# dcy0577/Enhancing-3D-Point-Cloud-Segmentation-Using-Multi-Modal-Fusion-with-2D-Images

Measured on AMD Instinct MI355X. Metric: input points/s through MV-KPConv KPFCNN forward+backward (pyramid + fusion + fwd + bwd + SGD), higher is better.
Workload: dtype f32; 1 GPU; early_fusion_kpfcnn5_sphere19k_x1_per_gpu; views=3, parallelism=dp1, execution=hipGraph[net|chain|enc2d(x2 every 2nd step)+fa], ranks=1, input_lookahead_batches=2, capacity_overflow=False

## Files before the change

### enhancing-3d-point-cloud-segmentation-using-multi-modal-fusion-with-2d-images_amd/_lib.py

```python
import ctypes as C
import os
import re

_HERE = os.path.dirname(os.path.abspath(__file__))
LIB_PATH = os.path.join(_HERE, "libmvkpconv.so")
HEADER_PATH = os.path.join(_HERE, "..", "include", "mvkpconv.h")
SCENE_HEADER_PATH = os.path.join(_HERE, "..", "include", "mvkpconv_scene.h")
TRAIN_HEADER_PATH = os.path.join(_HERE, "..", "include", "mvkpconv_train.h")
SPHERE_HEADER_PATH = os.path.join(_HERE, "..", "include", "mvkpconv_sphere.h")

CTYPES = {"int": C.c_int, "int32_t": C.c_int32, "int64_t": C.c_int64, "float": C.c_float, "double": C.c_double,
          "const char*": C.c_char_p}
_SCALARS = frozenset(t for t in CTYPES if not t.endswith("*"))
_POINTEES = _SCALARS | {"void", "char", "uint8_t", "uint16_t"}
_INTEGER = r"-?(?:0[xX][0-9a-fA-F]+|0|[1-9][0-9]*)"
_DIRECTIVE = re.compile(r"\s*#\s*(?:include\s*<[\w./]+>|ifdef\s+__cplusplus|ifndef\s+\w+_H|endif"
                        r"|define\s+(\w+)(?:\s+(%s))?)\s*" % _INTEGER)
_STRUCT = re.compile(r"typedef\s+struct(?:\s+\w+)?\s*\{([^{}]*)\}\s*(mvk_\w+)\s*;")
_FUNCTION = re.compile(r"([\w\s*]+?)\b(mvk_\w+)\s*\(([^(){};]*)\)\s*;")


def parse_header(text):
    functions, structs, constants = {}, {}, {}

    def fail(pos, what):
        pos += len(text[pos:]) - len(text[pos:].lstrip())
        raise ValueError("mvkpconv.h line %d: %s" % (text.count("\n", 0, pos) + 1, what))

    def canonical(pos, spelling):
        tokens = re.findall(r"\w+|\S", spelling)
        const = tokens[:1] == ["const"]
        base, stars = "".join(tokens[const:const + 1]), tokens[const + 1:]
        if not (stars == [] and not const and base in _SCALARS
                or stars == ["*"] and (base in _POINTEES or base in structs)):
            fail(pos, "unsupported type %r" % " ".join(tokens))
        return "const " * const + base + "*" * len(stars)

    def declarator(pos, spelling):
        m = re.fullmatch(r"(.*[\s*])([A-Za-z_]\w*)\s*", spelling, re.S)
        if not m or m.group(2) == "const" or m.group(2) in _POINTEES:
            fail(pos, "expected '<type> <name>', found %r" % spelling.strip())
        return canonical(pos, m.group(1)), m.group(2)

    text = re.sub(r"/\*.*?\*/|//[^\n]*", lambda m: " " + "\n" * m.group().count("\n"), text, flags=re.S)
    lines = text.split("\n")
    for i, line in enumerate(lines):
        if line.lstrip().startswith("#"):
            m = _DIRECTIVE.fullmatch(line)
            name, value = m.groups() if m else (None, None)
            if not m or (name is not None and (name.startswith("MVK_") != (value is not None) or name in constants)):
                raise ValueError("mvkpconv.h line %d: unsupported preprocessor line %r" % (i + 1, line.strip()))
            if value is not None:
                constants[name] = int(value, 0)
            lines[i] = ""
    text = "\n".join(lines)

    block = re.fullmatch(r'\s*extern\s+"C"\s*\{(.*)\}\s*', text, re.S)
    if not block:
        fail(0, 'expected one extern "C" { ... } block around all declarations')
    pos, end = block.start(1), block.end(1)
    while True:
        pos = re.compile(r"\s*").match(text, pos, end).end()
        if pos == end:
            return functions, structs, constants
        s = _STRUCT.match(text, pos, end)
        f = None if s else _FUNCTION.match(text, pos, end)
        if (s or f) and (s or f).group(2) in functions.keys() | structs.keys():
            fail(pos, "%s is declared twice" % (s or f).group(2))
        if s:
            fields, at = [], s.start(1)
            *statements, tail = s.group(1).split(";")
            if tail.strip() or not statements:
                fail(s.end(1) - len(tail), "struct %s: expected 'type name;' fields" % s.group(2))
            for statement in statements:
                first, *more = statement.split(",")
                ctype, name = declarator(at, first)
                if more and (ctype.endswith("*") or not all(re.fullmatch(r"\s*[A-Za-z_]\w*\s*", n) for n in more)):
                    fail(at, "only scalar fields share a declaration, found %r" % statement.strip())
                fields += [(ctype, n.strip()) for n in [name] + more]
                at += len(statement) + 1
            structs[s.group(2)] = tuple(fields)
        elif f:
            params, at = [], f.start(3)
            for spelling in f.group(3).split(",") if f.group(3).strip() != "void" else ():
                params.append(declarator(at, spelling))
                at += len(spelling) + 1
            functions[f.group(2)] = (canonical(pos, f.group(1)), tuple(params))
        else:
            fail(pos, "neither a function declaration nor a struct typedef: %r" % text[pos:end].split("\n")[0].strip())
        pos = (s or f).end()


def _bind(functions, structs):
    classes = {}

    def ctype(t):
        if t in CTYPES:
            return CTYPES[t]
        assert t.endswith("*"), t
        pointee = t[6 * t.startswith("const "):-1]
        return C.POINTER(classes[pointee]) if pointee in classes else C.c_void_p

    for name, fields in structs.items():
        classes[name] = type("".join(w.capitalize() for w in name.split("_")[1:]), (C.Structure,),
                             {"_fields_": [(n, ctype(t)) for t, n in fields], "__doc__": name + " (include/mvkpconv.h)"})
    return classes, {name: (ctype(ret), [ctype(t) for t, _ in params]) for name, (ret, params) in functions.items()}


def _read_header(path=None, name="mvkpconv.h"):
    path = HEADER_PATH if path is None else path
    if not os.path.exists(path):
        raise RuntimeError(
            "include/%s is not there (%s). The binding reads every prototype of libmvkpconv.so from it -- "
            "run the package from a checkout of the repository; there is no second copy of the C ABI." % (name, path))
    with open(path) as f:
        return f.read()


FUNCTIONS, STRUCTS, CONSTANTS = parse_header(_read_header())
_CLASSES, _PROTOTYPES = _bind(FUNCTIONS, STRUCTS)
EXPORTS = tuple(FUNCTIONS)
ABI_VERSION = CONSTANTS["MVK_ABI_VERSION"]

SCENE_FUNCTIONS, _scene_structs, SCENE_CONSTANTS = parse_header(_read_header(SCENE_HEADER_PATH, "mvkpconv_scene.h"))
if _scene_structs or SCENE_FUNCTIONS.keys() & FUNCTIONS.keys() or SCENE_CONSTANTS.keys() & CONSTANTS.keys():
    raise ValueError("mvkpconv_scene.h: it may declare neither a struct nor a name of mvkpconv.h")
_SCENE_PROTOTYPES = _bind(SCENE_FUNCTIONS, {})[1]

TRAIN_FUNCTIONS, _train_structs, TRAIN_CONSTANTS = parse_header(_read_header(TRAIN_HEADER_PATH, "mvkpconv_train.h"))
if (_train_structs or TRAIN_FUNCTIONS.keys() & (FUNCTIONS.keys() | SCENE_FUNCTIONS.keys())
        or TRAIN_CONSTANTS.keys() & (CONSTANTS.keys() | SCENE_CONSTANTS.keys())):
    raise ValueError("mvkpconv_train.h: it may declare neither a struct nor a name of the other two headers")
_TRAIN_PROTOTYPES = _bind(TRAIN_FUNCTIONS, {})[1]

SPHERE_FUNCTIONS, _sphere_structs, SPHERE_CONSTANTS = parse_header(_read_header(SPHERE_HEADER_PATH, "mvkpconv_sphere.h"))
if (_sphere_structs
        or SPHERE_FUNCTIONS.keys() & (FUNCTIONS.keys() | SCENE_FUNCTIONS.keys() | TRAIN_FUNCTIONS.keys())
        or SPHERE_CONSTANTS.keys() & (CONSTANTS.keys() | SCENE_CONSTANTS.keys() | TRAIN_CONSTANTS.keys())):
    raise ValueError("mvkpconv_sphere.h: it may declare neither a struct nor a name of the other three headers")
_SPHERE_PROTOTYPES = _bind(SPHERE_FUNCTIONS, {})[1]
BnFwdProblem, BnBwdProblem = _CLASSES["mvk_bn_fwd_problem"], _CLASSES["mvk_bn_bwd_problem"]
BnFinish, ATransform = _CLASSES["mvk_bn_finish"], _CLASSES["mvk_a_transform"]
RevList, RegLayer = _CLASSES["mvk_rev_list"], _CLASSES["mvk_reg_layer"]

_lib = None
_owner_pid = None

FORK_MESSAGE = ("the MV-KPConv HIP library was initialised in process %d and is being called from its forked child %d: "
                "a HIP context does not survive fork(). Start DataLoader workers with multiprocessing_context='spawn', "
                "or let the workers emit only stacked points / lengths and build the pyramid "
                "(datasets.common.segmentation_inputs_sphere) in the main process -- see INTEGRATION.md")


def _check_process():
    pid = os.getpid()
    if _owner_pid is not None and pid != _owner_pid:
        raise RuntimeError(FORK_MESSAGE % (_owner_pid, pid))
    try:
        import torch
        if torch.cuda._is_in_bad_fork():
            raise RuntimeError(FORK_MESSAGE % (os.getppid(), pid))
    except (ImportError, AttributeError):
        pass


def lib():
    global _lib, _owner_pid
    _check_process()
    if _lib is None:
        if not os.path.exists(LIB_PATH):
            raise RuntimeError(
                "libmvkpconv.so is not built (%s). Run `python __graft_entry__.py build` -- there is "
                "no CPU fallback for the MV-KPConv hot path." % LIB_PATH)
        l = C.CDLL(LIB_PATH)
        for name, (res, args) in list(_PROTOTYPES.items()) + list(_SCENE_PROTOTYPES.items()) + list(_TRAIN_PROTOTYPES.items()) \
                + list(_SPHERE_PROTOTYPES.items()):
            fn = getattr(l, name)
            fn.restype = res
            fn.argtypes = args
        if l.mvk_abi_version() != ABI_VERSION:
            raise RuntimeError("libmvkpconv.so ABI %d != expected %d; rebuild" % (l.mvk_abi_version(), ABI_VERSION))
        _lib = l
        _owner_pid = os.getpid()
    return _lib


def check(rc):
    if rc != 0:
        raise RuntimeError(lib().mvk_last_error().decode("utf-8", "replace"))
```

### enhancing-3d-point-cloud-segmentation-using-multi-modal-fusion-with-2d-images_amd/build.py

```python
import os
import subprocess
import sys

HERE = os.path.dirname(os.path.abspath(__file__))
CSRC = os.path.join(HERE, "csrc")
OUT = os.path.join(HERE, "libmvkpconv.so")
ARCH = "gfx950"

SOURCES = [
    ("error.cpp", []),
    ("kpconv.hip", []),
    ("gemm.hip", []),
    ("gemm32s.hip", []),
    ("pool.hip", []),
    ("bn.hip", []),
    ("optim.hip", []),
    ("deform.hip", []),
    ("loss.hip", []),
    ("batchpad.hip", []),
    ("revlist.hip", []),
    ("subsample.hip", ["-ffp-contract=off"]),
    ("neighbors.hip", ["-ffp-contract=off"]),
    ("fusion.hip", ["-ffp-contract=off"]),
    ("vote.hip", ["-ffp-contract=off"]),
    ("pn2.hip", ["-ffp-contract=off"]),
    ("chunk.hip", ["-ffp-contract=off"]),
    ("pn2_ordered.hip", ["-ffp-contract=off"]),
    ("pn2_mlp.hip", ["-ffp-contract=off"]),
    ("pn2_rows.hip", ["-ffp-contract=off"]),
    ("scene_inputs.hip", ["-ffp-contract=off"]),
    ("train_inputs.hip", ["-ffp-contract=off"]),
    ("sphere_inputs.hip", ["-ffp-contract=off"]),
]


def _hipcc():
    for c in (os.environ.get("HIPCC"), "/opt/rocm/bin/hipcc", "hipcc"):
        if c and (os.path.isabs(c) and os.path.exists(c) or not os.path.isabs(c)):
            return c
    return "hipcc"


def _stale(target, deps):
    if not os.path.exists(target):
        return True
    t = os.path.getmtime(target)
    return any(os.path.getmtime(d) > t for d in deps if os.path.exists(d))


def build_library(force=False, verbose=False):
    hipcc = _hipcc()
    common = [os.path.join(CSRC, "common.h"), os.path.join(CSRC, "blockscan.h"), os.path.join(CSRC, "compact.h"),
              os.path.join(CSRC, "pn2_rows.h"), os.path.join(CSRC, "unproject.h"), os.path.join(CSRC, "select_frames.h"),
              os.path.join(CSRC, "knn_core.h"), os.path.join(HERE, "..", "include", "mvkpconv_sphere.h"),
              os.path.join(HERE, "..", "include", "mvkpconv.h"), os.path.join(HERE, "..", "include", "mvkpconv_scene.h"),
              os.path.join(HERE, "..", "include", "mvkpconv_train.h"),
              os.path.join(HERE, "..", "include", "mvk_prime_list.h"), os.path.abspath(__file__)]
    objs, jobs = [], []
    for src, extra in SOURCES:
        sp = os.path.join(CSRC, src)
        if not os.path.exists(sp):
            raise FileNotFoundError(sp)
        obj = os.path.join(CSRC, os.path.splitext(src)[0] + ".o")
        if force or _stale(obj, [sp] + common):
            cmd = [hipcc, "--offload-arch=" + ARCH, "-O3", "-std=c++17", "-fPIC", "-c", sp, "-o", obj] + extra
            if src.endswith(".cpp"):
                cmd = [hipcc, "-O2", "-std=c++17", "-fPIC", "-c", sp, "-o", obj]
            jobs.append(cmd)
        objs.append(obj)
    if jobs:
        from concurrent.futures import ThreadPoolExecutor
        n = max(1, min(int(os.environ.get("MVK_BUILD_JOBS", "6")), os.cpu_count() or 1, len(jobs)))

        def run(cmd):
            if verbose:
                print(" ".join(cmd), flush=True)
            subprocess.check_call(cmd)
        with ThreadPoolExecutor(n) as pool:
            list(pool.map(run, jobs))
    if force or _stale(OUT, objs):
        cmd = [hipcc, "--offload-arch=" + ARCH, "-shared", "-fPIC", "-o", OUT] + objs
        if verbose:
            print(" ".join(cmd))
        subprocess.check_call(cmd)
    return OUT


if __name__ == "__main__":
    print(build_library(force="--force" in sys.argv, verbose=True))
```

### enhancing-3d-point-cloud-segmentation-using-multi-modal-fusion-with-2d-images_amd/csrc/gemm.hip

```cpp
#include <stdlib.h>

#include <mutex>
#include <type_traits>

#include "common.h"

namespace {

typedef float f32x4 __attribute__((ext_vector_type(4)));

constexpr int BK = 32;

template <bool CONTIG_K, int ROWS>
struct Tile {
  static constexpr int LD = CONTIG_K ? 40 : ROWS + 4;
  static constexpr int FLOATS = CONTIG_K ? ROWS * 40 : BK * (ROWS + 4);
  static constexpr int NF4 = ROWS * BK / 4;
  static constexpr int NV = (NF4 + 255) / 256;
  static constexpr int IPT = ROWS / 4;
  float4 v[NV];

  __device__ __forceinline__ void transform(const float* __restrict__ xs, int64_t k0, int64_t kbase0, int64_t i0, int64_t imax,
                                            int64_t kmax, int64_t nvalid, float slope, float* __restrict__ out, int64_t ld,
                                            int tid) {
    static_assert(CONTIG_K, "the transform is written for k-contiguous A tiles");
#pragma unroll
    for (int u = 0; u < NV; ++u) {
      const int f = tid + 256 * u;
      if (NF4 % 256 == 0 || f < NF4) {
        const int i = f >> 3, kq = (f & 7) * 4;
        const int64_t gi = i0 + i, gk = k0 + kq;
        const float* t = xs + (gk - kbase0) * 4;
        float e[4] = {v[u].x, v[u].y, v[u].z, v[u].w};
#pragma unroll
        for (int c = 0; c < 4; ++c) {
          const float4 q = *reinterpret_cast<const float4*>(t + 4 * c);
          float z = (e[c] - q.x) * q.y + q.z;
          z = z > 0.f ? z : z * slope;
          e[c] = gi < nvalid ? z : 0.f;
        }
        v[u] = make_float4(e[0], e[1], e[2], e[3]);
        if (out && gi < imax) {
          float* o = out + gi * ld + gk;
          if (gk + 3 < kmax && (ld & 3) == 0)
            *reinterpret_cast<float4*>(o) = v[u];
          else {
#pragma unroll
            for (int c = 0; c < 4; ++c)
              if (gk + c < kmax) o[c] = e[c];
          }
        }
      }
    }
  }

  __device__ __forceinline__ void load(const float* __restrict__ src, int64_t ld, int64_t i0, int64_t imax,
                                       int64_t k0, int64_t kmax, int vec, int tid) {
#pragma unroll
    for (int u = 0; u < NV; ++u) {
      float t[4] = {0.f, 0.f, 0.f, 0.f};
      const int f = tid + 256 * u;
      if (NF4 % 256 == 0 || f < NF4) {
        if (CONTIG_K) {
          const int i = f >> 3, kq = (f & 7) * 4;
          const int64_t gi = i0 + i, gk = k0 + kq;
          if (gi < imax) {
            const float* p = src + gi * ld + gk;
            if (vec == 4 && gk + 3 < kmax) {
              const float4 q = *reinterpret_cast<const float4*>(p);
              t[0] = q.x; t[1] = q.y; t[2] = q.z; t[3] = q.w;
            } else if (vec == 2 && gk + 3 < kmax) {
              const float2 q0 = *reinterpret_cast<const float2*>(p), q1 = *reinterpret_cast<const float2*>(p + 2);
              t[0] = q0.x; t[1] = q0.y; t[2] = q1.x; t[3] = q1.y;
            } else {
#pragma unroll
              for (int e = 0; e < 4; ++e)
                if (gk + e < kmax) t[e] = p[e];
            }
          }
        } else {
          const int k = f / IPT, iq = (f % IPT) * 4;
          const int64_t gk = k0 + k, gi = i0 + iq;
          if (gk < kmax) {
            const float* p = src + gk * ld + gi;
            if (vec == 4 && gi + 3 < imax) {
              const float4 q = *reinterpret_cast<const float4*>(p);
              t[0] = q.x; t[1] = q.y; t[2] = q.z; t[3] = q.w;
            } else if (vec == 2 && gi + 3 < imax) {
              const float2 q0 = *reinterpret_cast<const float2*>(p), q1 = *reinterpret_cast<const float2*>(p + 2);
              t[0] = q0.x; t[1] = q0.y; t[2] = q1.x; t[3] = q1.y;
            } else {
#pragma unroll
              for (int e = 0; e < 4; ++e)
                if (gi + e < imax) t[e] = p[e];
            }
          }
        }
      }
      v[u] = make_float4(t[0], t[1], t[2], t[3]);
    }
  }

  template <int VEC>
  __device__ __forceinline__ void load_fast(const float* __restrict__ src, int64_t ld, int64_t i0, int64_t imax,
                                            int64_t k0, int tid) {
#pragma unroll
    for (int u = 0; u < NV; ++u) {
      int f = tid + 256 * u;
      if (NF4 % 256 != 0) f = f < NF4 ? f : NF4 - 1;
      const float* p;
      if (CONTIG_K) {
        const int i = f >> 3, kq = (f & 7) * 4;
        int64_t gi = i0 + i;
        gi = gi < imax ? gi : imax - 1;
        p = src + gi * ld + (k0 + kq);
      } else {
        const int k = f / IPT, iq = (f % IPT) * 4;
        int64_t gi = i0 + iq;
        gi = gi + 3 < imax ? gi : imax - 4;
        p = src + (k0 + k) * ld + gi;
      }
      if (VEC == 4) {
        const f32x4 q = *reinterpret_cast<const f32x4*>(p);
        v[u] = make_float4(q[0], q[1], q[2], q[3]);
      } else {
        const float2 q0 = *reinterpret_cast<const float2*>(p), q1 = *reinterpret_cast<const float2*>(p + 2);
        v[u] = make_float4(q0.x, q0.y, q1.x, q1.y);
      }
    }
  }

  static __device__ __forceinline__ bool fast_ok(int64_t imax, int vec) {
    return CONTIG_K ? (vec >= 2 && imax >= 1) : (vec == 4 && imax >= 4 && (imax & 3) == 0);
  }

  template <int VEC>
  __device__ __forceinline__ void fetch(const float* __restrict__ src, int64_t ld, int64_t i0, int64_t imax, int64_t k0,
                                        int64_t kmax, int vec, int tid) {
    if (VEC == 0)
      load(src, ld, i0, imax, k0, kmax, vec, tid);
    else
      load_fast<VEC>(src, ld, i0, imax, k0, tid);
  }

  __device__ __forceinline__ void store(float* __restrict__ T, int tid) const {
#pragma unroll
    for (int u = 0; u < NV; ++u) {
      const int f = tid + 256 * u;
      if (NF4 % 256 == 0 || f < NF4) {
        const f32x4 q = {v[u].x, v[u].y, v[u].z, v[u].w};
        if (CONTIG_K) {
          const int i = f >> 3, kq = (f & 7) * 4;
          *reinterpret_cast<f32x4*>(&T[i * LD + kq]) = q;
        } else {
          const int k = f / IPT, iq = (f % IPT) * 4;
          *reinterpret_cast<f32x4*>(&T[k * LD + iq]) = q;
        }
      }
    }
  }

  static __device__ __forceinline__ f32x4 frag(const float* __restrict__ T, int r0, int j, int lane) {
    const int i = lane & 15, g = lane >> 4;
    if (CONTIG_K) {
      return *reinterpret_cast<const f32x4*>(&T[(r0 + i) * LD + 16 * j + 4 * g]);
    } else {
      f32x4 r;
      const float* p = &T[(16 * j + 4 * g) * LD + r0 + i];
      r[0] = p[0];
      r[1] = p[LD];
      r[2] = p[2 * LD];
      r[3] = p[3 * LD];
      return r;
    }
  }
};

struct GemmArgs {
  const float* A;
  const float* B;
  float* C;
  int64_t M, N, Kd, lda, ldb, k_per_split;
  int atomic_out, accumulate, vecA, vecB;
  float* bn_part;
  const int32_t* n_valid;
  const float* bias;
  float act_slope;
  const float* A2;
  const float* B2;
  int64_t Kd2, lda2, ldb2;
  int vecA2, vecB2;
  const void* sc_idx;
  int sc_idx64, sc_c1;
  int64_t sc_stride, sc_ns;
  float* sc_dst;
  float* sc_rest;
  float* det_ws;
  int* det_cnt;
  int det_gx, det_nsplit;
  int seg_shift;
  int64_t seg_extra;
  int* fin_cnt;
  int fin_gy;
  float fin_eps, fin_momentum;
  float* fin_mean;
  float* fin_invstd;
  float* fin_rmean;
  float* fin_rvar;
  long long* fin_nbt;
  const float* ax_mean;
  const float* ax_invstd;
  const float* ax_gamma;
  const float* ax_beta;
  float ax_slope;
  const int32_t* ax_nvalid;
  float* ax_out;
};

constexpr int XF_KMAX = 512;

template <bool TA, bool TB, int PM, int QN, int WM, int WN, bool DUAL = false, bool XF = false>
__device__ __forceinline__ void gemm_body(const GemmArgs& a, const int bx, const int by, const int bz) {
  static_assert(WM * WN == 4, "four waves per workgroup");
  constexpr int TM = 16 * PM * WM, TN = 16 * QN * WN;
  typedef Tile<!TA, TM> TileA;
  typedef Tile<TB, TN> TileB;
  __shared__ __attribute__((aligned(16))) float lds[2 * (TileA::FLOATS + TileB::FLOATS)];
  __shared__ __attribute__((aligned(16))) float xs[XF ? 4 * (XF_KMAX + BK) : 4];
  float* const As = lds;
  float* const Bs = lds + 2 * TileA::FLOATS;
  const int tid = threadIdx.x, lane = tid & 63, wave = tid >> 6;
  const int wm = wave / WN, wn = wave % WN;
  const int64_t m0 = (int64_t)by * TM, n0 = (int64_t)bx * TN;
  const int64_t ktot = DUAL ? a.Kd + a.Kd2 : a.Kd;
  const int64_t kbeg_all = (int64_t)bz * a.k_per_split;
  const int64_t kend_all = kbeg_all + a.k_per_split < ktot ? kbeg_all + a.k_per_split : ktot;

  f32x4 acc[PM][QN];
#pragma unroll
  for (int p = 0; p < PM; ++p)
#pragma unroll
    for (int q = 0; q < QN; ++q) acc[p][q] = (f32x4){0.f, 0.f, 0.f, 0.f};

  int64_t x_nvalid = 0;
  if (XF) {
    for (int k = tid; k < XF_KMAX + BK; k += 256) {
      const int64_t gk = kbeg_all + k;
      float4 q = make_float4(0.f, 0.f, 0.f, 0.f);
      if (gk < a.Kd && k < a.k_per_split + BK) q = make_float4(a.ax_mean[gk], a.ax_invstd[gk] * a.ax_gamma[gk], a.ax_beta[gk], 0.f);
      *reinterpret_cast<float4*>(&xs[4 * k]) = q;
    }
    x_nvalid = a.ax_nvalid ? (int64_t)*a.ax_nvalid : a.M;
    __syncthreads();
  }
  float* const x_out = (XF && bx == 0) ? a.ax_out : nullptr;

  TileA la0, la1;
  TileB lb0, lb1;
  const int ra = wm * 16 * PM, rb = wn * 16 * QN;
  auto compute = [&](const float* __restrict__ Ta, const float* __restrict__ Tb) {
#pragma unroll
    for (int j = 0; j < 2; ++j) {
      f32x4 fa[PM], fb[QN];
#pragma unroll
      for (int p = 0; p < PM; ++p) fa[p] = TileA::frag(Ta, ra + 16 * p, j, lane);
#pragma unroll
      for (int q = 0; q < QN; ++q) fb[q] = TileB::frag(Tb, rb + 16 * q, j, lane);
#pragma unroll
      for (int s = 0; s < 4; ++s)
#pragma unroll
        for (int p = 0; p < PM; ++p)
#pragma unroll
          for (int q = 0; q < QN; ++q)
            acc[p][q] = __builtin_amdgcn_mfma_f32_16x16x4f32(fa[p][s], fb[q][s], acc[p][q], 0, 0, 0);
    }
  };
  float* const A0 = As;
  float* const A1 = As + TileA::FLOATS;
  float* const B0 = Bs;
  float* const B1 = Bs + TileB::FLOATS;
  auto run_range = [&](const float* __restrict__ pA, const int64_t lda, const int vecA, const float* __restrict__ pB,
                       const int64_t ldb, const int vecB, int64_t kbeg, const int64_t kend) {
  auto Bat = [&](const int64_t k) -> const float* {
    return (TB && !DUAL && a.seg_shift >= 0) ? pB + (k >> a.seg_shift) * a.seg_extra : pB;
  };
  auto putA = [&](TileA& la, float* __restrict__ T, const int64_t kt) {
    if constexpr (XF) la.transform(xs, kt, kbeg_all, m0, a.M, a.Kd, x_nvalid, a.ax_slope, x_out, lda, tid);
    la.store(T, tid);
  };
  auto pipeline = [&](auto va, auto vb, const int64_t klim) {
    constexpr int VA = decltype(va)::value, VB = decltype(vb)::value;
    if (kbeg >= klim) return;
    la0.template fetch<VA>(pA, lda, m0, a.M, kbeg, klim, vecA, tid);
    lb0.template fetch<VB>(Bat(kbeg), ldb, n0, a.N, kbeg, klim, vecB, tid);
    if (kbeg + BK < klim) {
      la1.template fetch<VA>(pA, lda, m0, a.M, kbeg + BK, klim, vecA, tid);
      lb1.template fetch<VB>(Bat(kbeg + BK), ldb, n0, a.N, kbeg + BK, klim, vecB, tid);
    }
    putA(la0, A0, kbeg);
    lb0.store(B0, tid);
    __syncthreads();
    for (int64_t k0 = kbeg; k0 < klim; k0 += 2 * BK) {
      if (k0 + 2 * BK < klim) {
        la0.template fetch<VA>(pA, lda, m0, a.M, k0 + 2 * BK, klim, vecA, tid);
        lb0.template fetch<VB>(Bat(k0 + 2 * BK), ldb, n0, a.N, k0 + 2 * BK, klim, vecB, tid);
      }
      compute(A0, B0);
      if (k0 + BK >= klim) break;
      putA(la1, A1, k0 + BK);
      lb1.store(B1, tid);
      __syncthreads();
      if (k0 + 3 * BK < klim) {
        la1.template fetch<VA>(pA, lda, m0, a.M, k0 + 3 * BK, klim, vecA, tid);
        lb1.template fetch<VB>(Bat(k0 + 3 * BK), ldb, n0, a.N, k0 + 3 * BK, klim, vecB, tid);
      }
      compute(A1, B1);
      if (k0 + 2 * BK >= klim) break;
      putA(la0, A0, k0 + 2 * BK);
      lb0.store(B0, tid);
      __syncthreads();
    }
  };
  const bool fastA = TileA::fast_ok(a.M, vecA), fastB = TileB::fast_ok(a.N, vecB);
  const int64_t kfull = kbeg + (kend - kbeg) / BK * BK;
  typedef std::integral_constant<int, 4> I4;
  typedef std::integral_constant<int, 2> I2;
  typedef std::integral_constant<int, 0> I0;
  if (fastA && fastB && vecA == 4 && vecB == 4) {
    pipeline(I4(), I4(), kfull);
  } else if (fastA && fastB && vecA == 2 && vecB == 4) {
    pipeline(I2(), I4(), kfull);
  } else {
    pipeline(I0(), I0(), kend);
    kbeg = kend;
  }
  if (kfull < kend && kbeg < kend) {
    __syncthreads();
    la0.load(pA, lda, m0, a.M, kfull, kend, vecA, tid);
    lb0.load(Bat(kfull), ldb, n0, a.N, kfull, kend, vecB, tid);
    putA(la0, A0, kfull);
    lb0.store(B0, tid);
    __syncthreads();
    compute(A0, B0);
  }
  };
  if (!DUAL) {
    run_range(a.A, a.lda, a.vecA, a.B, a.ldb, a.vecB, kbeg_all, kend_all);
  } else {
    if (kbeg_all < a.Kd) run_range(a.A, a.lda, a.vecA, a.B, a.ldb, a.vecB, kbeg_all, kend_all < a.Kd ? kend_all : a.Kd);
    if (kend_all > a.Kd) {
      if (kbeg_all < a.Kd) __syncthreads();
      run_range(a.A2, a.lda2, a.vecA2, a.B2, a.ldb2, a.vecB2, kbeg_all > a.Kd ? kbeg_all - a.Kd : 0, kend_all - a.Kd);
    }
  }

  if (a.det_ws) {
    constexpr int NB = PM * QN, SLOT = NB * 4 * 256;
    const int64_t tile = (int64_t)by * a.det_gx + bx;
    const __amdgpu_buffer_rsrc_t slots = park_rsrc(a.det_ws + tile * a.det_nsplit * SLOT);
    const uint32_t lane_off = (uint32_t)tid * 16u;
#pragma unroll
    for (int p = 0; p < PM; ++p)
#pragma unroll
      for (int q = 0; q < QN; ++q)
        park_store4(slots, (uint32_t)bz * (SLOT * 4u) + (uint32_t)(p * QN + q) * 4096u + lane_off, acc[p][q]);
    park_wait();
    __syncthreads();
    int* const flag = reinterpret_cast<int*>(lds);
    if (tid == 0) {
      const int old = __hip_atomic_fetch_add(a.det_cnt + tile, 1, __ATOMIC_RELAXED, __HIP_MEMORY_SCOPE_AGENT);
      const int last = old == a.det_nsplit - 1;
      if (last) __hip_atomic_store(a.det_cnt + tile, 0, __ATOMIC_RELAXED, __HIP_MEMORY_SCOPE_AGENT);
      *flag = last;
    }
    __syncthreads();
    const int last = *flag;
    __syncthreads();
    if (!last) return;
#pragma unroll
    for (int p = 0; p < PM; ++p)
#pragma unroll
      for (int q = 0; q < QN; ++q) acc[p][q] = (f32x4){0.f, 0.f, 0.f, 0.f};
    constexpr int ZC = NB >= 8 ? 2 : 4;
    for (int z0 = 0; z0 < a.det_nsplit; z0 += ZC) {
      f32x4 t[ZC][NB];
#pragma unroll
      for (int zz = 0; zz < ZC; ++zz) {
        const int z = z0 + zz < a.det_nsplit ? z0 + zz : a.det_nsplit - 1;
#pragma unroll
        for (int b = 0; b < NB; ++b) t[zz][b] = park_load4(slots, (uint32_t)z * (SLOT * 4u) + (uint32_t)b * 4096u + lane_off);
      }
#pragma unroll
      for (int zz = 0; zz < ZC; ++zz)
        if (z0 + zz < a.det_nsplit) {
#pragma unroll
          for (int p = 0; p < PM; ++p)
#pragma unroll
            for (int q = 0; q < QN; ++q) acc[p][q] += t[zz][p * QN + q];
        }
    }
  }

  const int ci = lane & 15, g4 = (lane >> 4) * 4;
#pragma unroll
  for (int q = 0; q < QN; ++q) {
    const int64_t col = n0 + rb + 16 * q + ci;
    if (col < a.N) {
      const float bq = a.bias ? a.bias[col] : 0.f;
#pragma unroll
      for (int p = 0; p < PM; ++p)
#pragma unroll
        for (int r = 0; r < 4; ++r) {
          const int64_t row = m0 + ra + 16 * p + g4 + r;
          if (row < a.M) {
            if (a.sc_idx) {
              const float v = acc[p][q][r];
              if (col < a.sc_c1) {
                const int j = a.sc_idx64 ? load_idx<true>(a.sc_idx, row * a.sc_stride, a.sc_ns)
                                         : load_idx<false>(a.sc_idx, row * a.sc_stride, a.sc_ns);
                if (j >= 0) atomicAdd(a.sc_dst + (int64_t)j * a.sc_c1 + col, v);
              } else {
                float* c2 = a.sc_rest + row * (a.N - a.sc_c1) + (col - a.sc_c1);
                if (a.atomic_out) atomicAdd(c2, v);
                else *c2 = v;
              }
              continue;
            }
            float* c = a.C + row * a.N + col;
            if (a.atomic_out)
              atomicAdd(c, acc[p][q][r]);
            else if (a.accumulate)
              *c += acc[p][q][r];
            else if (a.bias) {
              const float v = acc[p][q][r] + bq;
              *c = v > 0.f ? v : v * a.act_slope;
            } else
              *c = acc[p][q][r];
          }
        }
    }
  }

  if (a.bn_part) {
    int64_t nv = a.n_valid ? (int64_t)*a.n_valid : a.M;
    nv = nv < a.M ? nv : a.M;
    const int64_t wcnt = nv - (m0 + ra) < 0 ? 0 : (nv - (m0 + ra) > 16 * PM ? 16 * PM : nv - (m0 + ra));
    const int64_t bcnt = nv - m0 < 0 ? 0 : (nv - m0 > TM ? TM : nv - m0);
    const int64_t blk = m0 / TM;
    float* red = lds;
    const __amdgpu_buffer_rsrc_t part_rs = park_rsrc(a.bn_part);
    auto put_part = [&](const int64_t col, const float sum, const float m2) {
      if (a.fin_cnt) {
        park_store1(part_rs, (uint32_t)(((blk * 2) * a.N + col) * 4), sum);
        park_store1(part_rs, (uint32_t)(((blk * 2 + 1) * a.N + col) * 4), m2);
      } else {
        a.bn_part[(blk * 2) * a.N + col] = sum;
        a.bn_part[(blk * 2 + 1) * a.N + col] = m2;
      }
    };
    if (WM > 1) __syncthreads();
    float s[QN], mu[QN];
#pragma unroll
    for (int q = 0; q < QN; ++q) {
      s[q] = 0.f;
#pragma unroll
      for (int p = 0; p < PM; ++p)
#pragma unroll
        for (int r = 0; r < 4; ++r)
          if (16 * p + g4 + r < wcnt) s[q] += acc[p][q][r];
      s[q] += __shfl_xor(s[q], 16);
      s[q] += __shfl_xor(s[q], 32);
      if (WM > 1 && lane < 16) red[wm * TN + rb + 16 * q + ci] = s[q];
    }
    if (WM > 1) {
      __syncthreads();
#pragma unroll
      for (int q = 0; q < QN; ++q) {
        s[q] = 0.f;
#pragma unroll
        for (int w = 0; w < WM; ++w) s[q] += red[w * TN + rb + 16 * q + ci];
      }
    }
#pragma unroll
    for (int q = 0; q < QN; ++q) {
      mu[q] = bcnt > 0 ? s[q] / (float)bcnt : 0.f;
      float m2 = 0.f;
#pragma unroll
      for (int p = 0; p < PM; ++p)
#pragma unroll
        for (int r = 0; r < 4; ++r)
          if (16 * p + g4 + r < wcnt) {
            const float d = acc[p][q][r] - mu[q];
            m2 += d * d;
          }
      m2 += __shfl_xor(m2, 16);
      m2 += __shfl_xor(m2, 32);
      if (WM > 1) {
        if (lane < 16) red[(WM + wm) * TN + rb + 16 * q + ci] = m2;
      } else {
        const int64_t col = n0 + rb + 16 * q + ci;
        if (lane < 16 && col < a.N && m0 < a.M) put_part(col, s[q], m2);
      }
    }
    if (WM > 1) {
      __syncthreads();
      if (wm == 0 && lane < 16) {
#pragma unroll
        for (int q = 0; q < QN; ++q) {
          float m2 = 0.f;
#pragma unroll
          for (int w = 0; w < WM; ++w) m2 += red[(WM + w) * TN + rb + 16 * q + ci];
          const int64_t col = n0 + rb + 16 * q + ci;
          if (col < a.N && m0 < a.M) put_part(col, s[q], m2);
        }
      }
    }
    if (a.fin_cnt) {
      park_wait();
      __syncthreads();
      int* const flag = reinterpret_cast<int*>(lds);
      if (tid == 0) {
        const int old = __hip_atomic_fetch_add(a.fin_cnt + bx, 1, __ATOMIC_RELAXED, __HIP_MEMORY_SCOPE_AGENT);
        const int last = old == a.fin_gy - 1;
        if (last) __hip_atomic_store(a.fin_cnt + bx, 0, __ATOMIC_RELAXED, __HIP_MEMORY_SCOPE_AGENT);
        *flag = last;
      }
      __syncthreads();
      const int last = *flag;
      __syncthreads();
      if (!last) return;
      constexpr int C4 = TN / 4, BL = 256 / C4;
      const int c4 = tid % C4, bl = tid / C4;
      const int64_t col0 = n0 + 4 * c4;
      const int nb = nv > 0 ? (int)((nv + TM - 1) / TM) : 0;
      f32x4 X = {0.f, 0.f, 0.f, 0.f}, Y = {0.f, 0.f, 0.f, 0.f}, ref = {0.f, 0.f, 0.f, 0.f};
      if (col0 < a.N && nb > 0) {
        const float n0f = (float)(nv < TM ? nv : TM);
        ref = park_load4(part_rs, (uint32_t)(col0 * 4));
        ref = ref * (1.f / n0f);
        constexpr int FP = 4;
        for (int i0 = bl; i0 < nb; i0 += FP * BL) {
          f32x4 u[FP], w[FP];
#pragma unroll
          for (int t = 0; t < FP; ++t) {
            const int i = i0 + t * BL < nb ? i0 + t * BL : nb - 1;
            u[t] = park_load4(part_rs, (uint32_t)((((int64_t)i * 2) * a.N + col0) * 4));
            w[t] = park_load4(part_rs, (uint32_t)((((int64_t)i * 2 + 1) * a.N + col0) * 4));
          }
#pragma unroll
          for (int t = 0; t < FP; ++t)
            if (i0 + t * BL < nb) {
              const int64_t left = nv - (int64_t)(i0 + t * BL) * TM;
              const float ni = (float)(left < TM ? left : TM);
              const f32x4 d = u[t] * (1.f / ni) - ref;
              X += u[t];
              Y += w[t] + ni * d * d;
            }
        }
      }
      float* const q1 = lds;
      float* const q2 = lds + 256 * 4;
      *reinterpret_cast<f32x4*>(&q1[bl * TN + 4 * c4]) = X;
      *reinterpret_cast<f32x4*>(&q2[bl * TN + 4 * c4]) = Y;
      float* const qr = lds + 2 * 256 * 4;
      if (bl == 0) *reinterpret_cast<f32x4*>(&qr[4 * c4]) = ref;
      __syncthreads();
      const int64_t col = n0 + tid;
      if (tid < TN && col < a.N) {
        float x = 0.f, y = 0.f;
#pragma unroll 4
        for (int l = 0; l < BL; ++l) {
          x += q1[l * TN + tid];
          y += q2[l * TN + tid];
        }
        float mu = 0.f, var = 0.f, is = 0.f;
        if (nv > 0) {
          mu = x / (float)nv;
          const float dm = mu - qr[tid];
          float M2 = y - (float)nv * dm * dm;
          M2 = M2 > 0.f ? M2 : 0.f;
          var = M2 / (float)nv;
          is = rsqrtf(var + a.fin_eps);
        }
        a.fin_mean[col] = mu;
        a.fin_invstd[col] = is;
        if (a.fin_rmean && nv > 0) {
          const float unbiased = nv > 1 ? var * ((float)nv / (float)(nv - 1)) : var;
          a.fin_rmean[col] = (1.f - a.fin_momentum) * a.fin_rmean[col] + a.fin_momentum * mu;
          a.fin_rvar[col] = (1.f - a.fin_momentum) * a.fin_rvar[col] + a.fin_momentum * unbiased;
        }
      }
      if (a.fin_nbt && bx == 0 && tid == 0) *a.fin_nbt += 1;
    }
  }
}

template <bool TA, bool TB, int PM, int QN, int WM, int WN>
__global__ __launch_bounds__(256) void gemm_f32_mfma(const GemmArgs a) {
  gemm_body<TA, TB, PM, QN, WM, WN>(a, blockIdx.x, blockIdx.y, blockIdx.z);
}

template <bool TB, int PM>
__global__ __launch_bounds__(256) void gemm_f32_mfma_xf(const GemmArgs a) {
  gemm_body<false, TB, PM, 1, 1, 4, false, true>(a, blockIdx.x, blockIdx.y, blockIdx.z);
}

template <bool TA, bool TB, int PM, int QN, int WM, int WN>
__global__ __launch_bounds__(256) void gemm_f32_mfma_pair(const GemmArgs a0, const GemmArgs a1, int gx0, int gz0, int gz1) {
  if ((int)blockIdx.x < gx0) {
    if ((int)blockIdx.z >= gz0) return;
    gemm_body<TA, TB, PM, QN, WM, WN>(a0, blockIdx.x, blockIdx.y, blockIdx.z);
  } else {
    if ((int)blockIdx.z >= gz1) return;
    gemm_body<TA, TB, PM, QN, WM, WN>(a1, blockIdx.x - gx0, blockIdx.y, blockIdx.z);
  }
}

template <bool TA, bool TB, int PM, int QN, int WM, int WN>
__global__ __launch_bounds__(256) void gemm_f32_mfma_dual(const GemmArgs a) {
  gemm_body<TA, TB, PM, QN, WM, WN, true>(a, blockIdx.x, blockIdx.y, blockIdx.z);
}

struct GroupEntry {
  GemmArgs args;
  int gx, gy, gz;
  int wg_begin;
};

template <bool TA, bool TB, int PM, int QN, int WM, int WN>
__global__ __launch_bounds__(256) void gemm_f32_mfma_grouped(const GroupEntry* __restrict__ tab, int n_prob) {
  const int b = blockIdx.x;
  int lo = 0, hi = n_prob - 1;
  while (lo < hi) {
    const int mid = (lo + hi + 1) >> 1;
    if (tab[mid].wg_begin <= b)
      lo = mid;
    else
      hi = mid - 1;
  }
  const GroupEntry& e = tab[lo];
  const int local = b - e.wg_begin;
  const int bx = local % e.gx, by = (local / e.gx) % e.gy, bz = local / (e.gx * e.gy);
  GemmArgs a = e.args;
  a.A = load_global_ptr(&e.args.A);
  a.B = load_global_ptr(&e.args.B);
  a.C = load_global_ptr(&e.args.C);
  a.bn_part = load_global_ptr(&e.args.bn_part);
  a.n_valid = load_global_ptr(&e.args.n_valid);
  a.det_ws = load_global_ptr(&e.args.det_ws);
  a.det_cnt = load_global_ptr(&e.args.det_cnt);
  gemm_body<TA, TB, PM, QN, WM, WN>(a, bx, by, bz);
}


struct Plan {
  int pm, qn, narrow, split;
  int64_t tm() const { return narrow ? 64 * pm : 16 * pm; }
  int64_t tn() const { return narrow ? 16 * qn : 64 * qn; }
};

struct SplitArena {
  float* ws = nullptr;
  int* cnt = nullptr;
  int64_t ws_floats = 0, n_cnt = 0;
  int64_t ws_off = 0, cnt_off = 0;
  int64_t ws_top = 0, cnt_top = 0;
};
SplitArena g_arena;
std::mutex g_arena_mu;

bool ordered_splits() { return g_arena.ws != nullptr; }

int arena_take(hipStream_t st, int64_t tiles, int split, int64_t slot, float** ws, int** cnt) {
  const int64_t need = (tiles * split * slot + 63) / 64 * 64;
  std::lock_guard<std::mutex> lock(g_arena_mu);
  if (need > g_arena.ws_floats || tiles > g_arena.n_cnt) return 1;
  hipStreamCaptureStatus cap = hipStreamCaptureStatusNone;
  if (hipStreamIsCapturing(st, &cap) != hipSuccess) {
    (void)hipGetLastError();
    cap = hipStreamCaptureStatusNone;
  }
  if (cap != hipStreamCaptureStatusNone) {
    if (g_arena.ws_top - need < g_arena.ws_off || g_arena.cnt_top - tiles < g_arena.cnt_off) return 2;
    g_arena.ws_top -= need;
    g_arena.cnt_top -= tiles;
    *ws = g_arena.ws + g_arena.ws_top;
    *cnt = g_arena.cnt + g_arena.cnt_top;
    return 0;
  }
  const int64_t ws_cap = g_arena.ws_top < g_arena.ws_floats / 4 ? g_arena.ws_top : (need > g_arena.ws_floats / 4 ? need : g_arena.ws_floats / 4);
  const int64_t cnt_cap = g_arena.cnt_top < g_arena.n_cnt / 4 ? g_arena.cnt_top : (tiles > g_arena.n_cnt / 4 ? tiles : g_arena.n_cnt / 4);
  if (g_arena.ws_off + need > ws_cap || g_arena.cnt_off + tiles > cnt_cap) {
    if (need > g_arena.ws_top || tiles > g_arena.cnt_top) return 2;
    if (hipDeviceSynchronize() != hipSuccess) return -2;
    g_arena.ws_off = 0;
    g_arena.cnt_off = 0;
  }
  *ws = g_arena.ws + g_arena.ws_off;
  *cnt = g_arena.cnt + g_arena.cnt_off;
  g_arena.ws_off += need;
  g_arena.cnt_off += tiles;
  return 0;
}

const char* arena_error(int rc) {
  return rc == 1 ? "the split-reduction arena is smaller than one product's parking space (MVK_GEMM_ARENA_MB)"
         : rc == 2 ? "the split-reduction arena is used up by the slices captured graphs hold for good: too small for the "
                     "captured steps of this process (MVK_GEMM_ARENA_MB)"
                   : "hipDeviceSynchronize failed while recycling the split-reduction arena";
}

int make_ordered(hipStream_t st, GemmArgs& a, int split, int gx, int64_t gy, int64_t tm, int64_t tn) {
  a.det_ws = nullptr; a.det_cnt = nullptr; a.det_gx = gx; a.det_nsplit = split;
  if (split <= 1 || !ordered_splits()) return 0;
  const int rc = arena_take(st, (int64_t)gx * gy, split, tm * tn, &a.det_ws, &a.det_cnt);
  if (rc != 0) return rc;
  a.atomic_out = 0;
  return 0;
}

#define MVK_ORDERED(call)                                      \
  do {                                                         \
    const int _rc = (call);                                    \
    MVK_REQUIRE(_rc == 0, "gemm: %s", arena_error(_rc));       \
  } while (0)

Plan plan_gemm(int64_t M, int64_t N, int64_t Kd, int split_req, bool want_stats) {
  const int narrow = N <= 32 ? 1 : 0;
  const int pm = narrow ? 1 : (want_stats ? 4 : 2), qn = narrow ? (N <= 16 ? 1 : 2) : 1;
  Plan best{pm, qn, narrow, 1};
  const int64_t tiles = cdiv64(M, best.tm()) * cdiv64(N, best.tn()), ksteps = cdiv64(Kd, BK);
  double best_t = 1e300, t1 = 1e300;
  for (int split = 1; split <= 64; ++split) {
    if (split_req > 0 && split != split_req) continue;
    if (split > 1 && ksteps / split < 4) break;
    const int64_t kt = cdiv64(ksteps, split), wgs = tiles * split;
    double t = (double)cdiv64(wgs, 1280) * (kt * 1500.0 + 3000.0) + (double)wgs * kt * 256.0 * pm * qn / 256.0;
    if (split > 1) t += (double)M * N * split * 4.0 / 2160.0 + 500.0 * split;
    if (split == 1) t1 = t;
    if (t < best_t) {
      best_t = t;
      best.split = split;
    }
  }
  static double bonus = -1.0;
  if (bonus < 0.0) {
    const char* eb = getenv("MVK_GEMM_STATS_BONUS");
    bonus = eb ? atof(eb) : 14000.0;
  }
  if (want_stats && !ordered_splits() && t1 <= best_t + bonus) best.split = 1;
  const char* e = getenv("MVK_GEMM_FORCE");
  if (e) {
    int pm = 0, qn = 0, sp = 0;
    if (sscanf(e, "%d,%d,%d", &pm, &qn, &sp) == 3) {
      if (pm > 0) best.pm = pm;
      if (qn > 0 && !best.narrow) best.qn = qn;
      if (sp > 0 && split_req <= 0) best.split = sp;
    }
  }
  return best;
}

template <bool TA, bool TB, int PM, int QN, int WM, int WN>
void launch_one(dim3 grid, hipStream_t st, const GemmArgs& a) {
  hipLaunchKernelGGL((gemm_f32_mfma<TA, TB, PM, QN, WM, WN>), grid, dim3(256), 0, st, a);
}

template <bool TA, bool TB>
bool launch_cfg(const Plan& p, dim3 grid, hipStream_t st, const GemmArgs& a) {
  if (p.narrow) {
#define NARROW(PMv, QNv) \
  if (p.pm == PMv && p.qn == QNv) return launch_one<TA, TB, PMv, QNv, 4, 1>(grid, st, a), true
    NARROW(1, 1); NARROW(2, 1); NARROW(1, 2); NARROW(2, 2);
#undef NARROW
    return false;
  }
#define WIDE(PMv, QNv) \
  if (p.pm == PMv && p.qn == QNv) return launch_one<TA, TB, PMv, QNv, 1, 4>(grid, st, a), true
  WIDE(1, 1); WIDE(2, 1); WIDE(4, 1); WIDE(5, 1);
  WIDE(1, 2); WIDE(2, 2); WIDE(4, 2);
#undef WIDE
  return false;
}

template <bool TA, bool TB, int PM>
void launch_pair_one(dim3 grid, hipStream_t st, const GemmArgs& a0, const GemmArgs& a1, int gx0, int gz0, int gz1) {
  hipLaunchKernelGGL((gemm_f32_mfma_pair<TA, TB, PM, 1, 1, 4>), grid, dim3(256), 0, st, a0, a1, gx0, gz0, gz1);
}

template <bool TA, bool TB>
bool launch_pair_cfg(const Plan& p, dim3 grid, hipStream_t st, const GemmArgs& a0, const GemmArgs& a1, int gx0, int gz0, int gz1) {
  if (p.qn != 1) return false;
  if (p.pm == 2) return launch_pair_one<TA, TB, 2>(grid, st, a0, a1, gx0, gz0, gz1), true;
  if (p.pm == 4) return launch_pair_one<TA, TB, 4>(grid, st, a0, a1, gx0, gz0, gz1), true;
  return false;
}

void pair_widen(Plan& a, const Plan& b, int64_t Kd) {
  if (a.narrow && !b.narrow && Kd <= 512) {
    a.narrow = 0;
    a.pm = b.pm;
    a.qn = 1;
    a.split = 1;
  }
}

int vec_width(const void* p, int64_t ld) {
  return ((ld % 4 == 0) && ((uintptr_t)p % 16 == 0)) ? 4 : ((ld % 2 == 0) && ((uintptr_t)p % 8 == 0)) ? 2 : 1;
}

struct KSplit { int n; int64_t k_per_split; };
KSplit clamp_split(int64_t Kd, int split) {
  const int64_t ksteps = cdiv64(Kd, BK);
  if (split > ksteps) split = (int)ksteps;
  const int64_t k_per_split = cdiv64(ksteps, split) * BK;
  return {(int)cdiv64(Kd, k_per_split), k_per_split};
}

GemmArgs make_args(const float* A, const float* B, float* C, int64_t M, int64_t N, int64_t Kd, int64_t lda, int64_t ldb,
                   KSplit ks) {
  GemmArgs a{};
  a.A = A; a.B = B; a.C = C; a.M = M; a.N = N; a.Kd = Kd;
  a.lda = lda; a.ldb = ldb; a.vecA = vec_width(A, lda); a.vecB = vec_width(B, ldb);
  a.k_per_split = ks.k_per_split; a.atomic_out = ks.n > 1; a.det_nsplit = ks.n;
  a.act_slope = 1.f; a.ax_slope = 1.f; a.vecA2 = 1; a.vecB2 = 1; a.seg_shift = -1;
  return a;
}

int set_finish(GemmArgs& a, const mvk_bn_finish* fin, int64_t gy) {
  if (!fin) return 0;
  MVK_REQUIRE(a.bn_part != nullptr, "gemm: finished BatchNorm statistics need the statistics epilogue (plan: stat rows 0)");
  MVK_REQUIRE(fin->counters && fin->mean && fin->invstd && a.N % 4 == 0 && (uintptr_t)a.bn_part % 16 == 0,
              "gemm: finished statistics need counters, mean, invstd and a channel count that is a multiple of 4");
  MVK_REQUIRE((fin->running_mean == nullptr) == (fin->running_var == nullptr), "gemm: running_mean and running_var go together");
  a.fin_cnt = fin->counters; a.fin_gy = (int)gy; a.fin_eps = fin->eps; a.fin_momentum = fin->momentum;
  a.fin_mean = fin->mean; a.fin_invstd = fin->invstd; a.fin_rmean = fin->running_mean; a.fin_rvar = fin->running_var;
  a.fin_nbt = (long long*)fin->num_batches_tracked;
  return 0;
}

struct ScatterOut {
  const void* idx;
  int idx64, c1;
  int64_t stride, ns;
  float* dst;
  float* rest;
};

struct GemmOpts {
  int accumulate = 0, split_k = 0;
  float* bn_part = nullptr;
  const int32_t* n_valid = nullptr;
  const float* bias = nullptr;
  float act_slope = 1.f;
  const ScatterOut* scatter = nullptr;
  int seg_shift = -1;
  int64_t seg_extra = 0, ldb = 0, lda = 0;
  const mvk_bn_finish* fin = nullptr;
  const mvk_a_transform* ax = nullptr;
};

int gemm_run(const float* A, const float* B, float* C, int64_t M, int64_t N, int64_t Kd, int transA, int transB,
             const GemmOpts& o, void* stream) {
  MVK_REQUIRE(M >= 0 && N >= 0 && Kd >= 0, "gemm: negative size");
  if (M == 0 || N == 0) return 0;
  hipStream_t st = (hipStream_t)stream;
  MVK_REQUIRE(!(o.bn_part && (o.accumulate || Kd == 0)), "gemm: BatchNorm statistics need a plain store of a non-empty product");
  if (Kd == 0) {
    if (!o.accumulate && o.split_k <= 1) MVK_CHECK_HIP(hipMemsetAsync(C, 0, sizeof(float) * M * N, st));
    return 0;
  }
  MVK_REQUIRE(!(o.bn_part && o.split_k > 1 && !ordered_splits()), "gemm: BatchNorm statistics need an unsplit (or ordered) reduction");
  const Plan p = plan_gemm(M, N, Kd, (o.bn_part && !ordered_splits()) ? 1 : (o.split_k > 0 ? o.split_k : 0), o.bn_part != nullptr);
  const KSplit ks = clamp_split(Kd, p.split);
  const int64_t lda = o.lda > 0 ? o.lda : (transA ? M : Kd);
  if (cdiv64(M, p.tm()) >= 65536) {
    MVK_REQUIRE(!o.bn_part && !o.fin && !o.ax && !o.scatter && o.seg_shift < 0 && ks.n < 65536, "gemm: grid too large");
    constexpr int64_t CHUNK = 15 * 65536;
    GemmOpts oc = o;
    oc.split_k = ks.n;
    oc.lda = lda;
    for (int64_t m0 = 0; m0 < M; m0 += CHUNK) {
      const int64_t mc = M - m0 < CHUNK ? M - m0 : CHUNK;
      if (int e = gemm_run(A + (transA ? m0 : m0 * lda), B, C + m0 * N, mc, N, Kd, transA, transB, oc, stream)) return e;
    }
    return 0;
  }
  GemmArgs a = make_args(A, B, C, M, N, Kd, lda, o.ldb > 0 ? o.ldb : (transB ? Kd : N), ks);
  if (o.seg_shift >= 0) {
    a.ldb = (int64_t)1 << o.seg_shift;
    a.vecB = ((uintptr_t)B % 16 == 0 && o.seg_extra % 4 == 0) ? 4 : 1;
  }
  a.accumulate = o.accumulate; a.bn_part = o.bn_part; a.n_valid = o.n_valid; a.bias = o.bias; a.act_slope = o.act_slope;
  a.seg_shift = o.seg_shift; a.seg_extra = o.seg_extra;
  if (o.scatter) {
    a.sc_idx = o.scatter->idx; a.sc_idx64 = o.scatter->idx64; a.sc_c1 = o.scatter->c1; a.sc_stride = o.scatter->stride;
    a.sc_ns = o.scatter->ns; a.sc_dst = o.scatter->dst; a.sc_rest = o.scatter->rest;
  }
  MVK_REQUIRE(cdiv64(M, p.tm()) < 65536 && ks.n < 65536, "gemm: grid too large");
  dim3 grid((unsigned)cdiv64(N, p.tn()), (unsigned)cdiv64(M, p.tm()), (unsigned)ks.n);
  MVK_ORDERED(make_ordered(st, a, ks.n, (int)grid.x, grid.y, p.tm(), p.tn()));
  MVK_REQUIRE(!(o.bn_part && ks.n > 1 && !a.det_ws), "gemm: BatchNorm statistics of a split product need the ordered reduction");
  if (int e = set_finish(a, o.fin, grid.y)) return e;
  if (const mvk_a_transform* ax = o.ax) {
    MVK_REQUIRE(!transA && transB && !p.narrow && p.qn == 1 && (p.pm == 2 || p.pm == 4) && ks.k_per_split <= XF_KMAX && !o.scatter &&
                    o.seg_shift < 0 && ax->mean && ax->invstd && ax->gamma && ax->beta && ax->slope > 0.f,
                "gemm: the operand transform needs an NT product of more than 32 columns with k-ranges <= %d", XF_KMAX);
    a.ax_mean = ax->mean; a.ax_invstd = ax->invstd; a.ax_gamma = ax->gamma; a.ax_beta = ax->beta; a.ax_slope = ax->slope;
    a.ax_nvalid = ax->n_valid; a.ax_out = ax->out;
    if (p.pm == 2) hipLaunchKernelGGL((gemm_f32_mfma_xf<true, 2>), grid, dim3(256), 0, st, a);
    else hipLaunchKernelGGL((gemm_f32_mfma_xf<true, 4>), grid, dim3(256), 0, st, a);
    MVK_CHECK_HIP(hipGetLastError());
    return 0;
  }
  bool ok;
  if (!transA && !transB) ok = launch_cfg<false, false>(p, grid, st, a);
  else if (!transA && transB) ok = launch_cfg<false, true>(p, grid, st, a);
  else if (transA && !transB) ok = launch_cfg<true, false>(p, grid, st, a);
  else ok = launch_cfg<true, true>(p, grid, st, a);
  MVK_REQUIRE(ok, "gemm: no kernel for plan pm=%d qn=%d narrow=%d", p.pm, p.qn, p.narrow);
  MVK_CHECK_HIP(hipGetLastError());
  return 0;
}

int gemm_pair_run(const float* A, const float* B0, const float* B1, float* C0, float* C1, int64_t M, int64_t N0, int64_t N1,
                  int64_t Kd, int transB, int want_stats, float* bn_part0, float* bn_part1, const int32_t* n_valid,
                  const mvk_bn_finish* fin0, const mvk_bn_finish* fin1, void* stream) {
  MVK_REQUIRE(M > 0 && N0 > 0 && N1 > 0 && Kd > 0, "gemm pair: empty product");
  Plan p0 = plan_gemm(M, N0, Kd, 0, want_stats != 0), p1 = plan_gemm(M, N1, Kd, 0, want_stats != 0);
  pair_widen(p0, p1, Kd);
  MVK_REQUIRE(!p0.narrow && !p1.narrow && p0.pm == p1.pm && p0.qn == 1 && p1.qn == 1 && (p0.pm == 2 || p0.pm == 4),
              "gemm pair: the two products do not share a tile shape (ask mvk_gemm_f32_pair_plan first)");
  hipStream_t st = (hipStream_t)stream;
  const bool ord = ordered_splits();
  const KSplit s0 = clamp_split(Kd, p0.split), s1 = clamp_split(Kd, p1.split);
  GemmArgs a0 = make_args(A, B0, C0, M, N0, Kd, Kd, transB ? Kd : N0, s0);
  GemmArgs a1 = make_args(A, B1, C1, M, N1, Kd, Kd, transB ? Kd : N1, s1);
  a0.bn_part = (want_stats && (p0.split == 1 || ord)) ? bn_part0 : nullptr;
  a1.bn_part = (want_stats && (p1.split == 1 || ord)) ? bn_part1 : nullptr;
  a0.n_valid = a1.n_valid = n_valid;
  const int64_t tm = p0.tm(), tn = p0.tn(), gy = cdiv64(M, tm);
  MVK_REQUIRE(gy < 65536 && s0.n < 65536 && s1.n < 65536, "gemm: grid too large");
  const int gx0 = (int)cdiv64(N0, tn), gx1 = (int)cdiv64(N1, tn);
  MVK_ORDERED(make_ordered(st, a0, s0.n, gx0, gy, tm, tn));
  MVK_ORDERED(make_ordered(st, a1, s1.n, gx1, gy, tm, tn));
  MVK_REQUIRE(ord || ((s0.n == 1 || !a0.bn_part) && (s1.n == 1 || !a1.bn_part)), "gemm pair: statistics of a split product");
  if (int e = set_finish(a0, fin0, gy)) return e;
  if (int e = set_finish(a1, fin1, gy)) return e;
  dim3 grid((unsigned)(gx0 + gx1), (unsigned)gy, (unsigned)(s0.n > s1.n ? s0.n : s1.n));
  const bool ok = transB ? launch_pair_cfg<false, true>(p0, grid, st, a0, a1, gx0, s0.n, s1.n)
                         : launch_pair_cfg<false, false>(p0, grid, st, a0, a1, gx0, s0.n, s1.n);
  MVK_REQUIRE(ok, "gemm pair: no kernel for plan pm=%d", p0.pm);
  MVK_CHECK_HIP(hipGetLastError());
  return 0;
}

}

bool mvk_internal_arena_take(void* stream, int64_t floats, int64_t counters, float** ws, int** cnt) {
  if (!ordered_splits() || floats < 0 || counters < 0) return false;
  return arena_take((hipStream_t)stream, counters > 0 ? counters : 1, 1, cdiv64(floats, counters > 0 ? counters : 1), ws, cnt) == 0;
}

extern "C" int mvk_gemm_split_arena(void* ws, int64_t ws_bytes, void* counters, int64_t n_counters) {
  MVK_REQUIRE((ws == nullptr) == (counters == nullptr) && ws_bytes >= 0 && n_counters >= 0, "gemm arena: bad arguments");
  MVK_REQUIRE(ws == nullptr || (ws_bytes >= (1 << 20) && n_counters >= 4096 && (uintptr_t)ws % 256 == 0),
              "gemm arena: at least 1 MB of 256-byte aligned slots and 4096 counters");
  std::lock_guard<std::mutex> lock(g_arena_mu);
  g_arena.ws = (float*)ws;
  g_arena.cnt = (int*)counters;
  g_arena.ws_floats = ws ? ws_bytes / 4 : 0;
  g_arena.n_cnt = ws ? n_counters : 0;
  g_arena.ws_off = 0;
  g_arena.cnt_off = 0;
  g_arena.ws_top = g_arena.ws_floats;
  g_arena.cnt_top = g_arena.n_cnt;
  return 0;
}

extern "C" int mvk_gemm_split_ordered(void) { return ordered_splits() ? 1 : 0; }

extern "C" int mvk_gemm_f32_dual_plan(int64_t M, int64_t N, int64_t Kd, int64_t Kd2, int* out_split) {
  MVK_REQUIRE(M >= 0 && N >= 0 && Kd >= 0 && Kd2 >= 0 && out_split, "gemm dual plan: bad arguments");
  *out_split = 0;
  if (M == 0 || N == 0 || Kd == 0 || Kd2 == 0 || Kd % BK != 0) return 0;
  const Plan p = plan_gemm(M, N, Kd + Kd2, 0, false);
  if (p.narrow || p.qn != 1 || p.pm != 2) return 0;
  *out_split = clamp_split(Kd + Kd2, p.split).n;
  return 0;
}

extern "C" int mvk_gemm_f32_dual(const float* A, const float* B, const float* A2, const float* B2, float* C, int64_t M,
                                 int64_t N, int64_t Kd, int64_t Kd2, void* stream) {
  MVK_REQUIRE(M > 0 && N > 0 && Kd > 0 && Kd2 > 0 && Kd % BK == 0, "gemm dual: unsupported shape (ask mvk_gemm_f32_dual_plan)");
  const Plan p = plan_gemm(M, N, Kd + Kd2, 0, false);
  MVK_REQUIRE(!p.narrow && p.qn == 1 && p.pm == 2, "gemm dual: unsupported shape (ask mvk_gemm_f32_dual_plan)");
  hipStream_t st = (hipStream_t)stream;
  const KSplit ks = clamp_split(Kd + Kd2, p.split);
  GemmArgs a = make_args(A, B, C, M, N, Kd, Kd, N, ks);
  a.A2 = A2; a.B2 = B2; a.Kd2 = Kd2; a.lda2 = Kd2; a.ldb2 = N;
  a.vecA2 = vec_width(A2, a.lda2);
  a.vecB2 = vec_width(B2, a.ldb2);
  MVK_REQUIRE(cdiv64(M, 32) < 65536 && ks.n < 65536, "gemm: grid too large");
  dim3 grid((unsigned)cdiv64(N, 64), (unsigned)cdiv64(M, 32), (unsigned)ks.n);
  MVK_ORDERED(make_ordered(st, a, ks.n, (int)grid.x, grid.y, 32, 64));
  hipLaunchKernelGGL((gemm_f32_mfma_dual<false, false, 2, 1, 1, 4>), grid, dim3(256), 0, st, a);
  MVK_CHECK_HIP(hipGetLastError());
  return 0;
}

extern "C" int mvk_gemm_f32_pair_plan(int64_t M, int64_t N0, int64_t N1, int64_t Kd, int want_stats, int* out ) {
  MVK_REQUIRE(M >= 0 && N0 >= 0 && N1 >= 0 && Kd >= 0 && out, "gemm pair plan: bad arguments");
  for (int i = 0; i < 5; ++i) out[i] = 0;
  if (M == 0 || N0 == 0 || N1 == 0 || Kd == 0) return 0;
  Plan p0 = plan_gemm(M, N0, Kd, 0, want_stats != 0), p1 = plan_gemm(M, N1, Kd, 0, want_stats != 0);
  pair_widen(p0, p1, Kd);
  if (p0.narrow || p1.narrow || p0.pm != p1.pm || p0.qn != 1 || p1.qn != 1 || (p0.pm != 2 && p0.pm != 4)) return 0;
  out[0] = 1;
  out[1] = p0.split;
  out[2] = p1.split;
  out[3] = (want_stats && (p0.split == 1 || ordered_splits())) ? (int)p0.tm() : 0;
  out[4] = (want_stats && (p1.split == 1 || ordered_splits())) ? (int)p1.tm() : 0;
  return 0;
}

extern "C" int mvk_gemm_f32_pair(const float* A, const float* B0, const float* B1, float* C0, float* C1, int64_t M,
                                 int64_t N0, int64_t N1, int64_t Kd, int transB, int want_stats, float* bn_part0,
                                 float* bn_part1, const int32_t* n_valid, void* stream) {
  return gemm_pair_run(A, B0, B1, C0, C1, M, N0, N1, Kd, transB, want_stats, bn_part0, bn_part1, n_valid, nullptr, nullptr, stream);
}
extern "C" int mvk_gemm_f32_pair_bn(const float* A, const float* B0, const float* B1, float* C0, float* C1, int64_t M,
                                    int64_t N0, int64_t N1, int64_t Kd, int transB, float* bn_part0, float* bn_part1,
                                    const int32_t* n_valid, const mvk_bn_finish* fin0, const mvk_bn_finish* fin1, void* stream) {
  return gemm_pair_run(A, B0, B1, C0, C1, M, N0, N1, Kd, transB, 1, bn_part0, bn_part1, n_valid, fin0, fin1, stream);
}

extern "C" int mvk_gemm_f32_plan(int64_t M, int64_t N, int64_t Kd, int split_k, int want_stats, int* out_split,
                                 int* out_stat_rows) {
  MVK_REQUIRE(M >= 0 && N >= 0 && Kd >= 0 && out_split && out_stat_rows, "gemm plan: bad arguments");
  if (M == 0 || N == 0 || Kd == 0) {
    *out_split = 1;
    *out_stat_rows = 0;
    return 0;
  }
  const Plan p = plan_gemm(M, N, Kd, split_k > 0 ? split_k : 0, want_stats != 0);
  *out_split = p.split;
  *out_stat_rows = (want_stats && (p.split == 1 || ordered_splits())) ? (int)p.tm() : 0;
  return 0;
}

extern "C" int mvk_gemm_f32_ex(const float* A, const float* B, float* C, int64_t M, int64_t N, int64_t Kd,
                               int transA, int transB, int accumulate, int split_k, float* bn_part,
                               const int32_t* n_valid, void* stream) {
  GemmOpts o; o.accumulate = accumulate; o.split_k = split_k; o.bn_part = bn_part; o.n_valid = n_valid;
  return gemm_run(A, B, C, M, N, Kd, transA, transB, o, stream);
}

extern "C" int mvk_gemm_f32_bn(const float* A, const float* B, float* C, int64_t M, int64_t N, int64_t Kd, int transB,
                               float* bn_part, const int32_t* n_valid, const mvk_bn_finish* fin, const mvk_a_transform* ax,
                               void* stream) {
  MVK_REQUIRE(M > 0 && N > 0 && Kd > 0, "gemm bn: empty product");
  GemmOpts o; o.bn_part = bn_part; o.n_valid = n_valid; o.fin = fin; o.ax = ax;
  return gemm_run(A, B, C, M, N, Kd, 0, transB, o, stream);
}

extern "C" int mvk_gemm_f32_bias_act(const float* A, const float* B, float* C, int64_t M, int64_t N, int64_t Kd, int transB,
                                     const float* bias, float slope, void* stream) {
  MVK_REQUIRE(bias != nullptr && slope > 0.f && Kd > 0, "gemm bias_act: bias, a positive slope and a non-empty product");
  GemmOpts o; o.split_k = 1; o.bias = bias; o.act_slope = slope;
  return gemm_run(A, B, C, M, N, Kd, 0, transB, o, stream);
}

extern "C" int mvk_gemm_f32_kp_transposed(const float* A, const float* W, float* dx, int64_t M, int K, int Cin, int Cout,
                                          void* stream) {
  MVK_REQUIRE(K >= 1 && Cin >= 1 && Cout >= BK && (Cout & (Cout - 1)) == 0, "gemm kp_transposed: Cout must be a power of two >= 32");
  int shift = 0;
  while ((1 << shift) < Cout) ++shift;
  GemmOpts o; o.seg_shift = shift; o.seg_extra = (int64_t)Cin * Cout - Cout;
  return gemm_run(A, W, dx, M, Cin, (int64_t)K * Cout, 0, 1, o, stream);
}

extern "C" int mvk_gemm_f32_ldb(const float* A, const float* B, float* C, int64_t M, int64_t N, int64_t Kd, int64_t ldb,
                                void* stream) {
  MVK_REQUIRE(ldb >= N, "gemm ldb: ldb < N");
  GemmOpts o; o.ldb = ldb;
  return gemm_run(A, B, C, M, N, Kd, 0, 0, o, stream);
}

extern "C" int mvk_gemm_f32_scatter_cat(const float* A, const float* B, int64_t M, int64_t N, int64_t Kd, const void* idx,
                                        int idx64, int64_t idx_stride, int64_t Ns, int c1, float* d_x, float* d_skip,
                                        void* stream) {
  MVK_REQUIRE(idx && d_x && d_skip && c1 > 0 && c1 < N && Kd > 0 && Ns >= 0 && idx_stride >= 1, "gemm scatter_cat: bad arguments");
  const ScatterOut sc{idx, idx64, c1, idx_stride, Ns, d_x, d_skip};
  GemmOpts o; o.scatter = &sc;
  return gemm_run(A, B, d_skip , M, N, Kd, 0, 0, o, stream);
}

struct MvkGemmProblem {
  const float* A;
  const float* B;
  float* C;
  int64_t M, N, Kd;
};

extern "C" int64_t mvk_gemm_group_entry_bytes(void) { return (int64_t)sizeof(GroupEntry); }

constexpr int GROUP_KTILES_MIN = 16, GROUP_KTILES_MAX = 96;

int group_wide_pm() {
  static const int v = getenv("MVK_DW_WIDE_PM") ? atoi(getenv("MVK_DW_WIDE_PM")) : 4;
  return v == 2 || v == 8 ? v : 4;
}

int group_ktiles_env() {
  static const int v = getenv("MVK_DW_GROUP_KTILES") ? atoi(getenv("MVK_DW_GROUP_KTILES")) : -1;
  return v;
}

int grouped_split_at(int64_t M, int64_t N, int64_t Kd, int ktiles) {
  if (ktiles <= 0) return plan_gemm(M, N, Kd, 0, false).split;
  int64_t split = cdiv64(cdiv64(Kd, BK), ktiles);
  return (int)(split > 64 ? 64 : (split < 1 ? 1 : split));
}

extern "C" int mvk_gemm_f32_tn_grouped_split(int64_t M, int64_t N, int64_t Kd) {
  const int e = group_ktiles_env();
  return grouped_split_at(M, N, Kd, e >= 0 ? e : GROUP_KTILES_MIN);
}

extern "C" int mvk_gemm_f32_tn_grouped_plan(const void* problems, int n, void* table_host, int* n_narrow,
                                            int64_t* wgs_narrow, int64_t* wgs_wide, int32_t* splits ,
                                            void* stream ) {
  MVK_REQUIRE(n >= 0 && problems && table_host && n_narrow && wgs_narrow && wgs_wide && splits, "grouped gemm: bad arguments");
  const MvkGemmProblem* pr = (const MvkGemmProblem*)problems;
  GroupEntry* tab = (GroupEntry*)table_host;
  int nn = 0;
  for (int i = 0; i < n; ++i) nn += pr[i].N <= 32 ? 1 : 0;
  int64_t wn = 0, ww = 0;
  int in = 0, iw = nn;
  int ktiles = group_ktiles_env();
  if (ktiles < 0) {
    double units = 0.0;
    for (int i = 0; i < n; ++i)
      units += (double)cdiv64(pr[i].M, pr[i].N <= 32 ? 64 : 16 * group_wide_pm()) * cdiv64(pr[i].N, pr[i].N <= 32 ? 32 : 64) * cdiv64(pr[i].Kd, BK);
    const double t = units / 8000.0;
    ktiles = t < GROUP_KTILES_MIN ? GROUP_KTILES_MIN : (t > GROUP_KTILES_MAX ? GROUP_KTILES_MAX : (int)t);
  }
  for (int i = 0; i < n; ++i) {
    const MvkGemmProblem& q = pr[i];
    MVK_REQUIRE(q.M > 0 && q.N > 0 && q.Kd > 0 && q.A && q.B && q.C, "grouped gemm: empty problem %d", i);
    const bool narrow = q.N <= 32;
    MVK_REQUIRE(!narrow || q.N > 16, "grouped gemm: outputs of <= 16 columns are not grouped");
    const KSplit ks = clamp_split(q.Kd, grouped_split_at(q.M, q.N, q.Kd, ktiles));
    const int split = ks.n;
    GroupEntry e{};
    e.args = make_args(q.A, q.B, q.C, q.M, q.N, q.Kd, q.M, q.N, ks);
    const int64_t tm = narrow ? 64 : 16 * group_wide_pm(), tn = narrow ? 32 : 64;
    e.gx = (int)cdiv64(q.N, tn);
    e.gy = (int)cdiv64(q.M, tm);
    e.gz = split;
    MVK_ORDERED(make_ordered((hipStream_t)stream, e.args, split, e.gx, e.gy, tm, tn));
    const int64_t wgs = (int64_t)e.gx * e.gy * e.gz;
    if (narrow) {
      e.wg_begin = (int)wn;
      wn += wgs;
      tab[in++] = e;
    } else {
      e.wg_begin = (int)ww;
      ww += wgs;
      tab[iw++] = e;
    }
    splits[i] = split;
  }
  MVK_REQUIRE(wn < (1ll << 31) && ww < (1ll << 31), "grouped gemm: grid too large");
  *n_narrow = nn;
  *wgs_narrow = wn;
  *wgs_wide = ww;
  return 0;
}

extern "C" int mvk_gemm_f32_tn_grouped(const void* table_dev, int n, int n_narrow, int64_t wgs_narrow, int64_t wgs_wide,
                                       void* stream) {
  MVK_REQUIRE(n >= 0 && n_narrow >= 0 && n_narrow <= n, "grouped gemm: bad counts");
  hipStream_t st = (hipStream_t)stream;
  const GroupEntry* tab = (const GroupEntry*)table_dev;
  if (n_narrow > 0 && wgs_narrow > 0)
    hipLaunchKernelGGL((gemm_f32_mfma_grouped<true, false, 1, 2, 4, 1>), dim3((unsigned)wgs_narrow), dim3(256), 0, st, tab,
                       n_narrow);
  if (n - n_narrow > 0 && wgs_wide > 0) {
    if (group_wide_pm() == 4)
      hipLaunchKernelGGL((gemm_f32_mfma_grouped<true, false, 4, 1, 1, 4>), dim3((unsigned)wgs_wide), dim3(256), 0, st,
                         tab + n_narrow, n - n_narrow);
    else if (group_wide_pm() == 8)
      hipLaunchKernelGGL((gemm_f32_mfma_grouped<true, false, 8, 1, 1, 4>), dim3((unsigned)wgs_wide), dim3(256), 0, st,
                         tab + n_narrow, n - n_narrow);
    else
      hipLaunchKernelGGL((gemm_f32_mfma_grouped<true, false, 2, 1, 1, 4>), dim3((unsigned)wgs_wide), dim3(256), 0, st,
                         tab + n_narrow, n - n_narrow);
  }
  MVK_CHECK_HIP(hipGetLastError());
  return 0;
}

extern "C" int mvk_gemm_f32(const float* A, const float* B, float* C, int64_t M, int64_t N, int64_t Kd, int transA,
                            int transB, int accumulate, int split_k, void* stream) {
  return mvk_gemm_f32_ex(A, B, C, M, N, Kd, transA, transB, accumulate, split_k, nullptr, nullptr, stream);
}
```

### enhancing-3d-point-cloud-segmentation-using-multi-modal-fusion-with-2d-images_amd/ops.py

```python
import collections
import os
import ctypes as C

import weakref

import torch

from ._lib import lib, check, CONSTANTS, SCENE_CONSTANTS, TRAIN_CONSTANTS, SPHERE_CONSTANTS

INFLUENCE = {k[len("MVK_INFL_"):].lower(): v for k, v in CONSTANTS.items() if k.startswith("MVK_INFL_")}
AGGREGATION = {k[len("MVK_AGG_"):].lower(): v for k, v in CONSTANTS.items() if k.startswith("MVK_AGG_")}


def _p(t):
    return C.c_void_p(t.data_ptr()) if t is not None else None


def _stream():
    return C.c_void_p(torch.cuda.current_stream().cuda_stream)


def _dev(*ts):
    for t in ts:
        if t is not None and not t.is_cuda:
# ... 138 lines not shown
    e = getattr(t, "_mvk_bn_stats", None)
    return e if e is None or isinstance(e, BnStats) else BnStats(*e)


def bn_finished(t):
    return getattr(bn_stats_of(t), "finished", None) is not None


def _finishable(bn):
    return BN_FOLD and bn is not None and bn.training and _SYNC_BN["group"] is None and bn.num_features % 4 == 0


def _fin_counters(bn, device):
    c = getattr(bn, "_mvk_fin_counters", None)
    if c is None or c.device != device:
        if torch.cuda.is_current_stream_capturing():
            raise RuntimeError("ops: the finish counters of a BatchNorm do not exist yet and cannot be created inside a "
                               "graph capture; run one eager step first")
        c = torch.zeros(128, dtype=torch.int32, device=device)
        torch.cuda.current_stream(device).synchronize()
        bn._mvk_fin_counters = c
    return c


def _fin_struct(bn, N, device):
    from ._lib import BnFinish
    if bn.num_features != N:
        raise RuntimeError("ops: the BatchNorm handed to a product has %d channels, the product %d columns" % (bn.num_features, N))
    mean = torch.empty(N, device=device, dtype=torch.float32)
    invstd = torch.empty(N, device=device, dtype=torch.float32)
    track = bn.track_running_stats and bn.running_mean is not None
    fin = BnFinish(_p(_fin_counters(bn, device)), float(bn.eps), float(bn.momentum if bn.momentum is not None else 0.0),
                   _p(mean), _p(invstd), _p(bn.running_mean) if track else None, _p(bn.running_var) if track else None,
                   _p(bn.num_batches_tracked) if track else None)
    return fin, (mean, invstd)


def gemm(A, B, transA=False, transB=False, out=None, accumulate=False, split_k=None, keep=False, stats_n_valid=None):
    out, st = _product(A, B, transA=transA, transB=transB, out=out, accumulate=accumulate, split_k=split_k, keep=keep,
                       stats_n_valid=stats_n_valid)
    if stats_n_valid is None:
        return out
    return out, (st[:2] if st is not None else None)


def _product(A, B, *, transA=False, transB=False, out=None, accumulate=False, split_k=None, keep=False,
             stats_n_valid=None, finish=None, a_transform=None):
    _dev(A, B)
    A, B = _f32c(A), _f32c(B)
    M, Kd = (A.shape[1], A.shape[0]) if transA else (A.shape[0], A.shape[1])
    N = B.shape[0] if transB else B.shape[1]
    assert (B.shape[1] if transB else B.shape[0]) == Kd, "gemm: inner dimensions differ"
    ax = a_transform
    if ax is not None and (ax["lazy"].data_ptr() != A.data_ptr() or transA or not transB or out is not None or accumulate
                           or M == 0):
        raise RuntimeError("ops: a product with an operand transform takes the lazy tensor as A, W as transposed B and "
                           "an output of its own")
    if M == 0 or N == 0 or Kd == 0:
        return (out.zero_() if out is not None else torch.zeros((M, N), device=A.device, dtype=torch.float32)), None
    split_arena_prepare(A.device)
    stats_ok = stats_n_valid is not None and out is None and not accumulate and M <= _STATS_EPILOGUE_ROWS
    if finish is None and ax is None:
        stats_ok = stats_ok and M > bn_single_launch_rows(N)
    split, rows = gemm_plan(M, N, Kd, split_k, stats_ok)
    if out is None:
        out = _split_out((M, N), A.device, split, keep)
    elif split > 1 and not accumulate and A.device.index not in _SPLIT_ARENA:
        out.zero_()
    part =torch.empty(((M + rows - 1) // rows, 2, N), device=A.device, dtype=torch.float32) if rows > 0 else None
    fin = done = None
    if finish is not None and part is not None and not transA and split_k is None:
        fin, done = _fin_struct(finish, N, A.device)
    if fin is not None or ax is not None:
        xf = None
        if ax is not None:
            from ._lib import ATransform
            xf = ATransform(_p(ax["mean"]), _p(ax["invstd"]), _p(ax["gamma"]), _p(ax["beta"]), float(ax["slope"]),
                            _p(ax["n_valid"]), _p(ax["lazy"]))
            A = ax["raw"]
        check(lib().mvk_gemm_f32_bn(_p(A), _p(B), _p(out), M, N, Kd, int(transB), _p(part),
                                    _p(stats_n_valid) if part is not None else None,
                                    C.byref(fin) if fin is not None else None, C.byref(xf) if xf is not None else None,
                                    _stream()))
    else:
        check(lib().mvk_gemm_f32_ex(_p(A), _p(B), _p(out), M, N, Kd, int(transA), int(transB), int(accumulate),
                                    int(split), _p(part), _p(stats_n_valid) if part is not None else None, _stream()))
    return out, (BnStats(part, rows, done) if part is not None else None)


def gemm_f32_stream_plan(M, N, Kd):
    out = (C.c_int64 * 4)()
    check(lib().mvk_gemm_f32_stream_plan(int(M), int(N), int(Kd), out))
    return bool(out[0]), int(out[1]), int(out[2]), int(out[3])


def _slack_floats(t):
    return t.untyped_storage().nbytes() // 4 - t.storage_offset() - t.numel()


def gemm_f32_stream(A, B, stats_n_valid=None):
    _dev(A, B, stats_n_valid)
    A, B = _f32c(A), _f32c(B)
    M, Kd = A.shape
    N = B.shape[1]
    ok, tiles, wgs, need = gemm_f32_stream_plan(M, N, Kd)
    if not ok or B.shape[0] != Kd:
        raise RuntimeError("gemm_f32_stream: unsupported shape %d x %d x %d" % (M, N, Kd))
    y = torch.empty((M, N), device=A.device, dtype=torch.float32)
    part = torch.empty((wgs, 2, N), device=A.device, dtype=torch.float32) if stats_n_valid is not None else None
    check(lib().mvk_gemm_f32_stream(_p(A), _slack_floats(A), _p(B), _p(y), M, N, Kd, _p(stats_n_valid), _p(part), _stream()))
    return y, ((part, 16 * tiles) if part is not None else None)


_PROF = {"on": False, "rec": [], "gemm": []}


def profile_reset(enabled):
    _PROF["on"] = bool(enabled)
    _PROF["rec"] = []
    _PROF["gemm"] = []
    _PROF["h_eff"] = {}


def _timing_events():
    torch.cuda._sleep(200000)
    e0, e1 = torch.cuda.Event(enable_timing=True), torch.cuda.Event(enable_timing=True)
    e0.record()
    return e0, e1


def profile_collect_contraction():
    torch.cuda.synchronize()
    out = {}
    for key, e0, e1 in _PROF["gemm"]:
        r = out.setdefault(key, {"launches": 0, "total_ms": 0.0, "flops_per_launch": 2.0 * key[0] * key[1] * key[2]})
        r["launches"] += 1
        r["total_ms"] += e0.elapsed_time(e1)
    return out


def _gather_kernel_label(Nq, Ns, H, Cin, deform, fast=True):
    p = kpconv_gather_plan(Nq, Ns, H, Cin, 4, deform)
    if fast and p["mfma"]:
        return "kpconv_gather_mfma<T=%d>(1 point per wave)" % p["rows_per_batch"]
    return "kpconv_lane_channel<fwd,deform>" if deform else "kpconv_lane_channel<fwd>"


def profile_collect(h_eff=None):
    torch.cuda.synchronize()
    out = {}
    for key, e0, e1 in _PROF["rec"]:
        r = out.setdefault(key, {"launches": 0, "total_ms": 0.0, "each_ms": []})
        r["launches"] += 1
        t = e0.elapsed_time(e1)
        r["total_ms"] += t
        r["each_ms"].append(t)
    for key, r in out.items():
        name, Nq, Ns, H, Cin, K = key
        he = _PROF.get("h_eff", {}).get((Nq, Ns, H)) if name.endswith("[dx]") else None
        if he is None:
            he = (h_eff or {}).get((Nq, Ns, H), H)
        sx = 4
        r["bytes_per_launch"] = Nq * he * (Cin * sx + 12 + 4) + Nq * 12 + Nq * K * Cin * sx
        r["kernel"] = name
        r["shape"] = {"Nq": Nq, "Ns": Ns, "H": H, "H_eff": he, "Cin": Cin, "K": K}
    return out


def kpconv_gather(q, s, idx, x, kp, extent, influence="linear", aggregation="sum", offsets=None,
                  want_min_d2=False, order=None, tag=None):
    _dev(q, s, idx, x, kp, offsets, order)
    if order is not None and (order.dtype != torch.int32 or order.shape != (q.shape[0],) or not order.is_contiguous()):
        raise RuntimeError("kpconv_gather: order must be a contiguous int32 tensor of Nq entries")
    q, s, x, kp = _f32c(q), _f32c(s), _f32c(x), _f32c(kp)
    idx, i64 = _idx(idx)
    Nq, Ns, H, Cin, K = q.shape[0], s.shape[0], idx.shape[1] if idx.dim() == 2 else 0, x.shape[1], kp.shape[0]
    if x.shape[0] != Ns:
        raise RuntimeError("kpconv: features and support points differ in length")
    A = torch.empty(Nq * K * Cin + 64, device=q.device, dtype=torch.float32)[:Nq * K * Cin].view(Nq, K, Cin)
    min_d2 = min_arg = None
    if offsets is not None:
        offsets = _f32c(offsets)
        if want_min_d2:
            min_d2 = torch.empty((Nq, K), device=q.device, dtype=torch.float32)
            min_arg = torch.empty((Nq, K), device=q.device, dtype=torch.int32)
    if _PROF["on"]:
        e0, e1 = _timing_events()
    check(lib().mvk_kpconv_gather_fwd_ordered(_p(q), Nq, _p(s), Ns, _p(idx), i64, H, _p(x), Cin, _p(kp), K,
                                              float(extent), INFLUENCE[influence], AGGREGATION[aggregation],
                                              _p(offsets), _p(min_d2), _p(min_arg), _p(A), _p(order), _stream()))
    if _PROF["on"]:
        e1.record()
        name = _gather_kernel_label(Nq, Ns, H, Cin, offsets is not None, (influence, aggregation) == ("linear", "sum"))
        if tag:
            name += tag
            _PROF.setdefault("h_eff", {})[(Nq, Ns, H)] = float((idx < Ns).sum().item()) / max(Nq, 1)
        _PROF["rec"].append(((name, Nq, Ns, H, Cin, K), e0, e1))
    if min_d2 is not None:
        min_d2._mvk_min_arg = min_arg
    return A, min_d2


def kpconv_scatter(q, s, idx, dA, kp, extent, influence="linear", aggregation="sum", x=None,
                   offsets=None, g_min_d2=None, min_arg=None):
    _dev(q, s, idx, dA, kp)
    q, s, dA, kp = _f32c(q), _f32c(s), _f32c(dA), _f32c(kp)
    idx, i64 = _idx(idx)
    Nq, Ns, H, K, Cin = q.shape[0], s.shape[0], idx.shape[1], kp.shape[0], dA.shape[2]
    dx = _zeros((Ns, Cin), q.device)
    d_off = None
    if offsets is not None:
        offsets, x = _f32c(offsets), _f32c(x)
        d_off = (torch.zeros if (Nq == 0 or H == 0) else torch.empty)((Nq, K, 3), device=q.device, dtype=torch.float32)
        if g_min_d2 is not None:
            g_min_d2 = _f32c(g_min_d2)
            if min_arg is None:
                raise RuntimeError("kpconv_scatter: the min_d2 gradient needs the forward's arg-min columns")
    check(lib().mvk_kpconv_scatter_bwd(_p(q), Nq, _p(s), Ns, _p(idx), i64, H, Cin, _p(kp), K, float(extent),
                                       INFLUENCE[influence], AGGREGATION[aggregation], _p(dA), _p(dx),
                                       _p(x), _p(offsets), _p(g_min_d2), _p(min_arg), _p(d_off), _stream()))
    return dx, d_off


def kpconv_deform_doff(q, s, idx, x, kp, extent, offsets, dA, g_min_d2=None, min_arg=None):
    _dev(q, s, idx, x, kp, offsets, dA, g_min_d2, min_arg)
    q, s, x, kp, offsets, dA = _f32c(q), _f32c(s), _f32c(x), _f32c(kp), _f32c(offsets), _f32c(dA)
    idx, i64 = _idx(idx)
    Nq, Ns, H, K, Cin = q.shape[0], s.shape[0], idx.shape[1], kp.shape[0], dA.shape[2]
    if Nq == 0 or H == 0:
        return torch.zeros((Nq, K, 3), device=q.device, dtype=torch.float32)
    d_off = torch.empty((Nq, K, 3), device=q.device, dtype=torch.float32)
    if g_min_d2 is not None:
        g_min_d2 = _f32c(g_min_d2)
        if min_arg is None:
            raise RuntimeError("kpconv_deform_doff: the min_d2 gradient needs the forward's arg-min columns")
    check(lib().mvk_kpconv_deform_doff(_p(q), Nq, _p(s), Ns, _p(idx), i64, H, _p(x), Cin, _p(kp), K, float(extent),
                                       INFLUENCE["linear"], _p(offsets), _p(dA), _p(g_min_d2), _p(min_arg), _p(d_off),
                                       _stream()))
    return d_off


def kpconv_gather_rev_deform(s, q, rev, g, kp, extent, offsets, modulations=None, order=None):
    _dev(s, q, rev, g, kp, offsets, modulations, order)
    s, q, g, kp, offsets = _f32c(s), _f32c(q), _f32c(g), _f32c(kp), _f32c(offsets)
    if modulations is not None:
        modulations = _f32c(modulations)
    rev, r64 = _idx(rev)
    Ns, Nq, Hr, Cc, K = s.shape[0], q.shape[0], rev.shape[1], g.shape[1], kp.shape[0]
    if rev.shape[0] != Ns or g.shape[0] != Nq or offsets.shape != (Nq, K, 3):
        raise RuntimeError("kpconv_gather_rev_deform: rev [Ns,Hr], g [Nq,C] and offsets [Nq,K,3] expected")
    A2 = torch.empty(Ns * K * Cc + 64, device=s.device, dtype=torch.float32)[:Ns * K * Cc].view(Ns, K, Cc)
    check(lib().mvk_kpconv_gather_rev_deform(_p(s), Ns, _p(q), Nq, _p(rev), r64, Hr, _p(g), Cc, _p(kp), K, float(extent),
                                             _p(offsets), _p(modulations), _p(A2), _p(order), _stream()))
    return A2


_DEFER = {"on": False, "items": [], "leaves": set(), "slots": None, "eager": 0}
_DW_MAX = 512


def _defer_slots(device):
    if _DEFER["slots"] is None:
        nb = _DW_MAX * int(lib().mvk_gemm_group_entry_bytes())
        _DEFER["slots"] = [{"host": torch.empty(nb, dtype=torch.uint8).pin_memory(),
                            "dev": torch.empty(nb, dtype=torch.uint8, device=device), "event": None} for _ in range(34)]
    return _DEFER["slots"]


def capture_table_slots_left(device):
    return max(0, len(_defer_slots(device)) - 2)


class defer_weight_grads:

    def __init__(self, flush=True):
        self.flush = bool(flush)
        self.items = []

    def __enter__(self):
        _DEFER.update(on=True, items=[], leaves=set())
        return self

    def __exit__(self, *exc):
        try:
            if exc[0] is None:
                if self.flush:
                    _flush_deferred()
                else:
                    self.items = _DEFER["items"]
        finally:
            _DEFER.update(on=False, items=[], leaves=set())
        return False

    def take(self):
        items, self.items = self.items, []
        return items


def flush_deferred(items, stream=None):
    if not items:
        return
    if stream is None or stream == torch.cuda.current_stream():
        return _flush_deferred(items)
    for (A, B, _, _, _) in items:
        A.record_stream(stream)
        B.record_stream(stream)
    with torch.cuda.stream(stream):
        _flush_deferred(items)


_HAS_USE_COUNT = hasattr(torch._C, "_storage_Use_Count")


def _storage_use_count(storage):
    return torch._C._storage_Use_Count(storage._cdata)


def _flush_deferred(items=None):
    if items is None:
        items = _DEFER["items"]
    if not items:
        return
    import numpy as np
    dev = items[0][0].device
    n = len(items)
    prob = np.zeros(n, dtype=np.dtype([("A", "<u8"), ("B", "<u8"), ("C", "<u8"), ("M", "<i8"), ("N", "<i8"), ("Kd", "<i8")]))
    for i, (A, B, out_ptr, _, storage) in enumerate(items):
        if _storage_use_count(storage) < 2:
            raise RuntimeError("defer_weight_grads: a deferred weight-gradient result (%d x %d) was consumed before the "
                               "grouped launch computed it; was the backward run on parameters that already hold a "
                               ".grad, or with hooks that copy gradients? Run it without the scope (MVK_DEFER_DW=0)"
                               % (A.shape[1], B.shape[1]))
        prob[i] = (A.data_ptr(), B.data_ptr(), out_ptr, A.shape[1], B.shape[1], A.shape[0])
    slots = _defer_slots(dev)
    if torch.cuda.is_current_stream_capturing():
        if len(slots) <= 2:
            raise RuntimeError("defer_weight_grads: out of pre-pinned table slots for graph captures")
        slot = slots.pop()
        _DEFER.setdefault("captured", []).append(slot)
    else:
        slot = slots[_DEFER["eager"] % 2]
        _DEFER["eager"] += 1
        if slot["event"] is not None:
            slot["event"].synchronize()
    nn, wn, ww = C.c_int(0), C.c_int64(0), C.c_int64(0)
    splits = np.zeros(n, np.int32)
    check(lib().mvk_gemm_f32_tn_grouped_plan(prob.ctypes.data_as(C.c_void_p), n, C.c_void_p(slot["host"].data_ptr()),
                                             C.byref(nn), C.byref(wn), C.byref(ww), splits.ctypes.data_as(C.c_void_p),
                                             _stream()))
    for i, item in enumerate(items):
        if splits[i] > 1 and not item[3] and not lib().mvk_gemm_split_ordered():
            raise RuntimeError("defer_weight_grads: the grouped plan splits a product whose output was not zero-initialised")
    nb = n * int(lib().mvk_gemm_group_entry_bytes())
    slot["dev"][:nb].copy_(slot["host"][:nb], non_blocking=True)
    check(lib().mvk_gemm_f32_tn_grouped(C.c_void_p(slot["dev"].data_ptr()), n, nn.value, wn.value, ww.value, _stream()))
    if not torch.cuda.is_current_stream_capturing():
        ev = torch.cuda.Event()
        ev.record()
        slot["event"] = ev


def _accumulate_in_place_ok(t):
    if _DEFER["on"] and _DEFER["items"]:
        st = t.untyped_storage().data_ptr()
        for it in _DEFER["items"]:
            if it[0].untyped_storage().data_ptr() == st or it[1].untyped_storage().data_ptr() == st:
                return False
    return True


def _dw_gemm(A, B, transB=False, target=None):
    leaf = target if (target is not None and target.is_leaf) else None
    if _DEFER["on"] and leaf is not None:
        if id(leaf) in _DEFER["leaves"]:
            raise RuntimeError("defer_weight_grads: the same parameter receives two weight gradients inside one scope "
                               "(shared weights): run this backward without the scope (MVK_DEFER_DW=0)")
        if leaf.grad is not None:
            return gemm(A, B, transA=True, transB=transB)
    if _DEFER["on"] and _HAS_USE_COUNT and not transB and A.is_cuda and B.shape[1] > 16 and len(_DEFER["items"]) < _DW_MAX \
            and A.shape[0] > 0 and A.shape[1] > 0:
        A, B = _f32c(A), _f32c(B)
        split_arena_prepare(A.device)
        zeroed = lib().mvk_gemm_f32_tn_grouped_split(A.shape[1], B.shape[1], A.shape[0]) > 1 \
            and not lib().mvk_gemm_split_ordered()
        out = (_zeros((A.shape[1], B.shape[1]), A.device) if zeroed
               else torch.empty((A.shape[1], B.shape[1]), device=A.device, dtype=torch.float32))
        _DEFER["items"].append((A, B, out.data_ptr(), zeroed, out.untyped_storage()))
        if leaf is not None:
            _DEFER["leaves"].add(id(leaf))
        return out
    return gemm(A, B, transA=True, transB=transB)



class _KPConvFn(torch.autograd.Function):

    @staticmethod
    def forward(ctx, q, s, idx, x, kp, W, offsets, modulations, extent, influence, aggregation, stats_n_valid=None,
                order=None, rev=None, rev_order=None, finish=None):
        K, Cin, Cout = W.shape
        deform = offsets is not None
        A, min_d2 = kpconv_gather(q, s, idx, x, kp, extent, influence, aggregation, offsets, want_min_d2=deform,
                                  order=order)
        ctx.rev = (rev, rev_order)
        Am = A * modulations.unsqueeze(2) if modulations is not None else A
        if _PROF["on"]:
            e0, e1 = _timing_events()
        st = None
        if _contraction_streams(Am, q.shape[0], K * Cin, Cout):
            y, st = gemm_f32_stream(Am.view(-1, K * Cin), W.reshape(K * Cin, Cout), stats_n_valid)
            st = BnStats(*st) if st is not None else None
        else:
            y, st = _product(Am.view(-1, K * Cin), W.reshape(K * Cin, Cout), stats_n_valid=stats_n_valid, finish=finish)
        if _PROF["on"]:
            e1.record()
            _PROF["gemm"].append(((q.shape[0], K * Cin, Cout), e0, e1))
        ctx.save_for_backward(q, s, idx, x, kp, W, A, offsets, modulations)
        ctx.min_arg = getattr(min_d2, "_mvk_min_arg", None)
        ctx.cfg = (extent, influence, aggregation)
        if st is not None:
            ctx.mark_non_differentiable(st.partials)
        ctx.set_materialize_grads(False)
        return y, min_d2, st

    @staticmethod
    def backward(ctx, gy, g_min_d2, g_st=None):
        q, s, idx, x, kp, W, A, offsets, modulations = ctx.saved_tensors
        extent, influence, aggregation = ctx.cfg
        K, Cin, Cout = W.shape
        Nq = q.shape[0]
        if gy is None:
            gy = torch.zeros((Nq, Cout), device=q.device, dtype=torch.float32)
        gy = _f32c(gy)
        Am = A * modulations.unsqueeze(2) if modulations is not None else A
        dW = dx = d_off = d_mod = None
        if ctx.needs_input_grad[5]:
            dW = _dw_gemm(Am.view(Nq, K * Cin), gy, target=W).view(K, Cin, Cout)
        need_dA = ctx.needs_input_grad[3] or (offsets is not None)
        rev, rev_order = ctx.rev
        gather_form = (need_dA and rev is not None and REVERSE_DX and rev.shape[0] >= s.shape[0] and Cout >= 5
                       and influence == "linear" and aggregation == "sum")
        if gather_form and rev.shape[0] != s.shape[0]:
            rev = rev[:s.shape[0]]
        if gather_form and offsets is None and modulations is None:
            A2, _ = kpconv_gather(s, q, rev, gy, _neg_kernel_points(kp), extent, influence, aggregation, order=rev_order,
                                  tag="[dx]")
            dx = kp_transposed_contraction(A2, W)
        elif need_dA:
            dAm = gemm(gy, W.reshape(K * Cin, Cout), transB=True).view(Nq, K, Cin)
            if modulations is not None:
                if ctx.needs_input_grad[7]:
                    d_mod = (dAm * A).sum(dim=2)
                dA = dAm * modulations.unsqueeze(2)
            else:
                dA = dAm
            if gather_form and offsets is not None:
                d_off = kpconv_deform_doff(q, s, idx, x, kp, extent, offsets, dA, g_min_d2, ctx.min_arg)
                if ctx.needs_input_grad[3]:
                    A2 = kpconv_gather_rev_deform(s, q, rev, gy, kp, extent, offsets, modulations, order=rev_order)
                    dx = kp_transposed_contraction(A2, W)
            else:
                dx, d_off = kpconv_scatter(q, s, idx, dA, kp, extent, influence, aggregation, x=x,
                                           offsets=offsets,
                                           g_min_d2=g_min_d2 if offsets is not None else None, min_arg=ctx.min_arg)
        return None, None, None, dx, None, dW, d_off, d_mod, None, None, None, None, None, None, None, None


def _contraction_streams(A, M, Kd, N):
    if M <= 0:
        return False
    ok, _, _, need = gemm_f32_stream_plan(M, N, Kd)
    return ok and A.is_contiguous() and _slack_floats(A) >= need


def kpconv(q, s, idx, x, kp, W, extent, influence="linear", aggregation="sum", offsets=None, modulations=None,
           stats_n_valid=None, order=None, rev=None, rev_order=None, bn=None):
    if rev is not None and (rev.dtype != torch.int32 or rev.dim() != 2 or not rev.is_contiguous()):
        raise RuntimeError("kpconv: rev must be a contiguous int32 [Ns, Hr] matrix (ops.reverse_neighbors)")
    if influence not in INFLUENCE:
        raise ValueError("Unknown influence function type (config.KP_influence)")
    if aggregation not in AGGREGATION:
        raise ValueError("Unknown convolution mode. Should be 'closest' or 'sum'")
    y, min_d2, st = _KPConvFn.apply(q, s, idx, x, kp, W, offsets, modulations, float(extent), influence, aggregation,
                                    stats_n_valid, order, rev, rev_order,
                                    bn if stats_n_valid is not None and _finishable(bn) else None)
    if st is not None:
        y._mvk_bn_stats = st
    return y, min_d2



class _DeformRegFn(torch.autograd.Function):

    @staticmethod
    def forward(ctx, min_d2, deformed_kp, n_valid, extent, repulse_extent, power):
        _dev(min_d2, deformed_kp, n_valid)
        min_d2, dkp = _f32c(min_d2), _f32c(deformed_kp)
        N, K = min_d2.shape
        loss = _zeros((1,), min_d2.device)
        d_min = torch.empty_like(min_d2)
        d_dkp = torch.empty_like(dkp)
        check(lib().mvk_deform_regularizer(_p(min_d2), _p(dkp), _p(n_valid), N, K, float(extent), float(repulse_extent),
                                           float(power), _p(loss), _p(d_min), _p(d_dkp), _stream()))
        ctx.save_for_backward(d_min, d_dkp)
        return loss.reshape(())

    @staticmethod
    def backward(ctx, g):
        d_min, d_dkp = ctx.saved_tensors
        return d_min * g, d_dkp * g, None, None, None, None


class _DeformOperandsFn(torch.autograd.Function):

    @staticmethod
    def forward(ctx, raw, bias, kernel_points, extent, modulated):
        _dev(raw, bias, kernel_points)
        raw, bias, kp = _f32c(raw), _f32c(bias), _f32c(kernel_points)
        N, D = raw.shape
        K = kp.shape[0]
        if D != (4 if modulated else 3) * K or bias.numel() != D:
            raise RuntimeError("deform operands: the inner convolution must deliver %d columns" % ((4 if modulated else 3) * K))
        feat = torch.empty_like(raw)
        offsets = torch.empty((N, K, 3), device=raw.device, dtype=torch.float32)
        dkp = torch.empty_like(offsets)
        mod = torch.empty((N, K), device=raw.device, dtype=torch.float32) if modulated else None
        check(lib().mvk_deform_operands_fwd(_p(raw), _p(bias), _p(kp), N, K, int(bool(modulated)), float(extent), _p(feat),
                                            _p(offsets), _p(dkp), _p(mod), _stream()))
        ctx.save_for_backward(mod)
        ctx.cfg = (N, K, D, float(extent), bool(modulated))
        ctx.set_materialize_grads(False)
        return feat, offsets, dkp, mod

    @staticmethod
    def backward(ctx, g_feat, g_off, g_dkp, g_mod):
        (mod,) = ctx.saved_tensors
        N, K, D, extent, modulated = ctx.cfg
        dev = (mod if mod is not None else next(g for g in (g_feat, g_off, g_dkp, g_mod) if g is not None)).device
        gs = [None if g is None else _f32c(g) for g in (g_off, g_dkp, g_mod, g_feat)]
        d_raw = torch.empty((N, D), device=dev, dtype=torch.float32)
        d_bias = _zeros((D,), dev)
        check(lib().mvk_deform_operands_bwd(_p(gs[0]), _p(gs[1]), _p(gs[2]), _p(mod), _p(gs[3]), N, K, int(modulated), extent,
                                            _p(d_raw), _p(d_bias), _stream()))
        return d_raw, d_bias, None, None, None


def deform_operands(raw, bias, kernel_points, extent, modulated=False):
    return _DeformOperandsFn.apply(raw, bias, kernel_points, extent, modulated)


def _reg_many(cfgs, ts, grads, loss, gscale):
    from ._lib import RegLayer
    by_k = {}
    for i, (extent, repulse, power, nv) in enumerate(cfgs):
        m, d = ts[2 * i], ts[2 * i + 1]
        L = RegLayer(_p(m), _p(d), _p(nv), _p(grads[2 * i]) if grads else None, _p(grads[2 * i + 1]) if grads else None,
                     m.shape[0], float(extent), float(repulse), float(power))
        by_k.setdefault(int(m.shape[1]), []).append(L)
    for K, layers in by_k.items():
        for b in range(0, len(layers), REG_MANY):
            part = layers[b:b + REG_MANY]
            arr = (RegLayer * len(part))(*part)
            check(lib().mvk_deform_regularizer_many(arr, len(part), K, _p(loss), _p(gscale), _stream()))


class _DeformRegAllFn(torch.autograd.Function):

    @staticmethod
    def forward(ctx, cfgs, *tensors):
        ts = [_f32c(t) for t in tensors]
        _dev(*ts)
        loss = _zeros((1,), ts[0].device)
        _reg_many(cfgs, ts, None, loss, None)
        ctx.save_for_backward(*ts)
        ctx.cfgs = cfgs
        return loss.reshape(())

    @staticmethod
    def backward(ctx, g):
        ts = ctx.saved_tensors
        g = _f32c(g).reshape(1)
        grads = [torch.empty_like(t) for t in ts]
        _reg_many(ctx.cfgs, ts, grads, None, g)
        return (None, *grads)


def deform_regularizer_all(layers):
    layers = [l for l in layers if l[0].shape[0] > 0]
    if not layers:
        return None
    cfgs = [(l[2], l[3], l[4], l[5]) for l in layers]
    flat = []
    for l in layers:
        flat += [l[0], l[1]]
    return _DeformRegAllFn.apply(cfgs, *flat)


def deform_regularizer(min_d2, deformed_kp, extent, repulse_extent, power=1.0, n_valid=None):
    return _DeformRegFn.apply(min_d2, deformed_kp, n_valid, extent, repulse_extent, power)



_ROW_COUNTS = {}


def set_row_counts(mapping):
    _ROW_COUNTS.clear()
    if mapping:
        _ROW_COUNTS.update(mapping)


def row_count_for(rows):
    return _ROW_COUNTS.get(int(rows))


_COUNT_TABLE = {}
_COUNT_TABLE_ROWS = 1 << 22
_BIG_COUNTS = {}


def full_count(rows, device):
    rows = int(rows)
    t = _COUNT_TABLE.get(device.index)
    if t is None:
        if torch.cuda.is_current_stream_capturing():
            raise RuntimeError("ops.full_count: the constant row-count table does not exist yet and cannot be created "
                               "inside a graph capture; run one eager step first or call ops.full_count_prepare(device)")
        t = torch.arange(_COUNT_TABLE_ROWS, dtype=torch.int32, device=device)
        torch.cuda.current_stream(device).synchronize()
        _COUNT_TABLE[device.index] = t
    if 0 <= rows < _COUNT_TABLE_ROWS:
        return t[rows:rows + 1]
    key = (rows, device.index)
    w = _BIG_COUNTS.get(key)
    if w is None:
        if torch.cuda.is_current_stream_capturing():
            raise RuntimeError("ops.full_count: %d rows lie beyond the constant table; request this count once outside "
                               "the capture" % rows)
        w = torch.full((1,), rows, dtype=torch.int32, device=device)
        torch.cuda.current_stream(device).synchronize()
        _BIG_COUNTS[key] = w
    return w


def full_count_prepare(device):
    full_count(0, torch.device(device))


def _bn_fwd_problem(who, x, n_valid, gamma, beta, running_mean, running_var, cfg, nbt, addend, ext):
    R, D = x.shape
    y = torch.empty_like(x)
    ext_part, ext_rows, fin = ext if ext is not None else (None, 0, None)
    if ext_part is not None and (ext_part.shape[2] != D or ext_part.shape[0] != (R + ext_rows - 1) // ext_rows):
        raise RuntimeError("%s: the statistics partials do not belong to this tensor" % who)
    scratch = None
    if fin is not None:
        mean, invstd = fin
        running_mean = running_var = nbt = ext_part = None
        ext_rows = -1
    else:
        mean = torch.empty(D, device=x.device, dtype=torch.float32)
        invstd = torch.empty(D, device=x.device, dtype=torch.float32)
        if ext_part is None:
            scratch = torch.empty(((R + 63) // 64) * 2 * D, device=x.device, dtype=torch.float32)
    eps, momentum, slope = cfg
    args = (_p(x), _p(n_valid), R, D, _p(gamma), _p(beta), float(eps), float(momentum), float(slope), _p(running_mean),
            _p(running_var), _p(mean), _p(invstd), _p(scratch), _p(y), _p(nbt), _p(addend), _p(ext_part), int(ext_rows))
    return args, y, mean, invstd, scratch


def _bn_bwd_problem(x, g, n_valid, gamma, beta, mean, invstd, slope, yout):
    g = _f32c(g)
    R, D = x.shape
    dgb = torch.empty(2 * D, device=x.device, dtype=torch.float32)
    scratch = torch.empty(((R + 63) // 64) * 2 * D, device=x.device, dtype=torch.float32)
    dx = torch.empty_like(x)
    d_add = torch.empty_like(x) if yout is not None else None
    args = (_p(x), _p(g), _p(n_valid), R, D, _p(gamma), _p(beta), _p(mean), _p(invstd), float(slope), _p(scratch), _p(dgb),
            _p(dx), _p(yout), _p(d_add))
    return args, dgb, dx, d_add, (g, scratch)


class _BNLReLUFn(torch.autograd.Function):
    @staticmethod
    def forward(ctx, x, n_valid, gamma, beta, running_mean, running_var, eps, momentum, slope, training, nbt=None,
                addend=None, ext=None):
        _dev(x, n_valid, gamma, beta, addend)
        x = _f32c(x)
        if addend is not None:
            addend = _f32c(addend)
            if addend.shape != x.shape:
                raise RuntimeError("bn_lrelu: the residual addend must have the shape of the input")
        if not training:
            raise RuntimeError("masked BatchNorm is a training-mode op; use nn.BatchNorm1d in eval mode")
# ... 56 lines not shown
    nbt = bn.num_batches_tracked if (bn.training and bn.track_running_stats) else None
    return _BNLReLUFn.apply(x, n_valid, bn.weight, bn.bias, bn.running_mean, bn.running_var, bn.eps,
                            bn.momentum if bn.momentum is not None else 0.0, slope, bn.training, nbt, addend,
                            bn_stats_of(x))


class _BNLazyFn(torch.autograd.Function):

    @staticmethod
    def forward(ctx, x, n_valid, gamma, beta, mean, invstd, slope):
        y = torch.empty_like(x)
        ctx.save_for_backward(x, n_valid, gamma, beta, mean, invstd)
        ctx.slope = float(slope)
        return y

    @staticmethod
    def backward(ctx, g):
        x, n_valid, gamma, beta, mean, invstd = ctx.saved_tensors
        args, dgb, dx, _, _keep = _bn_bwd_problem(x, g, n_valid, gamma, beta, mean, invstd, ctx.slope, None)
        check(lib().mvk_bn_lrelu_bwd(*args, _stream()))
        D = x.shape[1]
        return dx, None, dgb[D:], dgb[:D], None, None, None


XF_KMAX = 512


def bn_lrelu_linear(x, n_valid, bn, slope, W, stats_n_valid=None, bn_out=None):
    fin = getattr(bn_stats_of(x), "finished", None)
    R, Kd = x.shape
    if (fin is None or not BN_FOLD or _SYNC_BN["group"] is not None or not x.is_cuda or x.dtype != torch.float32
            or not x.is_contiguous() or W.dtype != torch.float32 or not W.is_contiguous() or W.shape[1] != Kd
            or W.shape[0] <= 32 or Kd > XF_KMAX or Kd % 4 != 0 or R == 0 or not slope > 0):
        return None
    mean, invstd = fin
    lazy = _BNLazyFn.apply(x, n_valid, bn.weight, bn.bias, mean, invstd, float(slope))
    xf = {"raw": x.detach(), "mean": mean, "invstd": invstd, "gamma": bn.weight.detach(), "beta": bn.bias.detach(),
          "slope": float(slope), "n_valid": n_valid, "lazy": lazy}
    return linear(lazy, W, stats_n_valid=stats_n_valid, bn=bn_out, _a_transform=xf), lazy


class _BNLReLUPairFn(torch.autograd.Function):

    @staticmethod
    def forward(ctx, xa, xb, n_valid, ga, ba, rma, rva, gb, bb, rmb, rvb, cfg_a, cfg_b, nbt_a, nbt_b, ext_a, ext_b):
        from ._lib import BnFwdProblem
        _dev(xa, xb, n_valid, ga, ba, gb, bb)
        xa, xb = _f32c(xa), _f32c(xb)
        if xa.shape[0] != xb.shape[0]:
            raise RuntimeError("bn_lrelu_pair: the two inputs differ in rows")
        (args_a, ya, mean_a, is_a, _ka), (args_b, yb, mean_b, is_b, _kb) = [
            _bn_fwd_problem("bn_lrelu_pair", x, n_valid, g, b, rm, rv, cfg, nbt, None, ext)
            for x, g, b, rm, rv, cfg, nbt, ext in ((xa, ga, ba, rma, rva, cfg_a, nbt_a, ext_a),
                                                   (xb, gb, bb, rmb, rvb, cfg_b, nbt_b, ext_b))]
        check(lib().mvk_bn_lrelu_fwd_pair(C.byref(BnFwdProblem(*args_a)), C.byref(BnFwdProblem(*args_b)), _stream()))
        ctx.save_for_backward(xa, xb, n_valid, ga, ba, gb, bb, mean_a, is_a, mean_b, is_b)
        ctx.slopes = (float(cfg_a[2]), float(cfg_b[2]))
        ctx.set_materialize_grads(False)
        return ya, yb

    @staticmethod
    def backward(ctx, g_a, g_b):
        from ._lib import BnBwdProblem
        xa, xb, n_valid, ga, ba, gb, bb, mean_a, is_a, mean_b, is_b = ctx.saved_tensors
        (args_a, dgb_a, dx_a, _, _ka), (args_b, dgb_b, dx_b, _, _kb) = [
            _bn_bwd_problem(x, g if g is not None else torch.zeros_like(x), n_valid, gam, bet, mean, istd, slope, None)
            for x, g, gam, bet, mean, istd, slope in ((xa, g_a, ga, ba, mean_a, is_a, ctx.slopes[0]),
                                                      (xb, g_b, gb, bb, mean_b, is_b, ctx.slopes[1]))]
        check(lib().mvk_bn_lrelu_bwd_pair(C.byref(BnBwdProblem(*args_a)), C.byref(BnBwdProblem(*args_b)), _stream()))
        Da, Db = xa.shape[1], xb.shape[1]
        return (dx_a, dx_b, None, dgb_a[Da:], dgb_a[:Da], None, None, dgb_b[Db:], dgb_b[:Db], None, None, None, None, None,
                None, None, None)


def bn_lrelu_pair(xa, bn_a, slope_a, xb, bn_b, slope_b, n_valid):
    def unpack(bn):
        nbt = bn.num_batches_tracked if (bn.training and bn.track_running_stats) else None
        return nbt, (bn.eps, bn.momentum if bn.momentum is not None else 0.0)
    if not (bn_a.training and bn_b.training):
        raise RuntimeError("masked BatchNorm is a training-mode op; use nn.BatchNorm1d in eval mode")
    if _SYNC_BN["group"] is not None:
        return _sync_bn_lrelu(xa, n_valid, bn_a, slope_a, None), _sync_bn_lrelu(xb, n_valid, bn_b, slope_b, None)
    nbt_a, (eps_a, mom_a) = unpack(bn_a)
    nbt_b, (eps_b, mom_b) = unpack(bn_b)
    return _BNLReLUPairFn.apply(xa, xb, n_valid, bn_a.weight, bn_a.bias, bn_a.running_mean, bn_a.running_var,
                                bn_b.weight, bn_b.bias, bn_b.running_mean, bn_b.running_var,
                                (eps_a, mom_a, slope_a), (eps_b, mom_b, slope_b), nbt_a, nbt_b,
                                bn_stats_of(xa), bn_stats_of(xb))


class _AddLReLUFn(torch.autograd.Function):
    @staticmethod
    def forward(ctx, a, b, slope):
        _dev(a, b)
        a, b = _f32c(a), _f32c(b)
        y = torch.empty_like(a)
        check(lib().mvk_add_lrelu_fwd(_p(a), _p(b), a.numel(), float(slope), _p(y), _stream()))
        ctx.save_for_backward(y)
        ctx.slope = float(slope)
        return y

    @staticmethod
    def backward(ctx, g):
        (y,) = ctx.saved_tensors
        g = _f32c(g)
        d = torch.empty_like(y)
        check(lib().mvk_add_lrelu_bwd(_p(y), _p(g), y.numel(), ctx.slope, _p(d), _stream()))
        return d, d.clone(), None


def _bias_grad(y):
    split_arena_prepare(y.device)
    if lib().mvk_gemm_split_ordered():
        return torch.empty((y.shape[1],), device=y.device, dtype=torch.float32)
    return torch.zeros((y.shape[1],), device=y.device, dtype=torch.float32)


class _BiasLReLUFn(torch.autograd.Function):
    @staticmethod
    def forward(ctx, x, bias, slope):
        _dev(x, bias)
        x, bias = _f32c(x), _f32c(bias)
        y = torch.empty_like(x)
        check(lib().mvk_bias_lrelu_fwd(_p(x), _p(bias), x.shape[0], x.shape[1], float(slope), _p(y), _stream()))
        ctx.save_for_backward(y)
        ctx.slope = float(slope)
        return y

    @staticmethod
    def backward(ctx, g):
        (y,) = ctx.saved_tensors
        g = _f32c(g)
        dx = torch.empty_like(y)
        db = _bias_grad(y)
        check(lib().mvk_bias_lrelu_bwd(_p(y), _p(g), y.shape[0], y.shape[1], ctx.slope, _p(dx), _p(db), _stream()))
        return dx, db, None


def bias_lrelu(x, bias, slope=0.1):
    if x.dim() != 2 or bias.dim() != 1 or bias.shape[0] != x.shape[1]:
        raise RuntimeError("bias_lrelu: x [R,C] and bias [C] expected")
    if not slope > 0:
        raise ValueError("bias_lrelu: slope must be positive")
    return _BiasLReLUFn.apply(x, bias, slope)


class _LinearBiasActFn(torch.autograd.Function):

    @staticmethod
    def forward(ctx, x, W, bias, slope):
        _dev(x, W, bias)
        x, W, bias = _f32c(x), _f32c(W), _f32c(bias)
        y = torch.empty((x.shape[0], W.shape[0]), device=x.device, dtype=torch.float32)
        if x.shape[0] > 0:
            check(lib().mvk_gemm_f32_bias_act(_p(x), _p(W), _p(y), x.shape[0], W.shape[0], x.shape[1], 1, _p(bias),
                                              float(slope), _stream()))
        ctx.save_for_backward(x, W, y)
        ctx.slope = float(slope)
        return y

    @staticmethod
    def backward(ctx, g):
        x, W, y = ctx.saved_tensors
        g = _f32c(g)
        d = torch.empty_like(y)
        db = _bias_grad(y)
        check(lib().mvk_bias_lrelu_bwd(_p(y), _p(g), y.shape[0], y.shape[1], ctx.slope, _p(d), _p(db), _stream()))
        dx = gemm(d, W) if ctx.needs_input_grad[0] else None
        dW = _dw_gemm(d, x, target=W) if ctx.needs_input_grad[1] else None
        return dx, dW, db, None


def linear_bias_lrelu(x, W, bias, slope=0.1):
    if x.dim() != 2 or bias.dim() != 1 or bias.shape[0] != W.shape[0] or W.shape[1] != x.shape[1]:
        raise RuntimeError("linear_bias_lrelu: x [R,K], W [C,K] and bias [C] expected")
    if not slope > 0:
        raise ValueError("linear_bias_lrelu: slope must be positive")
    return _LinearBiasActFn.apply(x, W, bias, slope)


def add_lrelu(a, b, slope=0.1):
    if a.shape != b.shape:
        raise RuntimeError("add_lrelu: shapes differ")
    return _AddLReLUFn.apply(a, b, slope)



class _MaxPoolFn(torch.autograd.Function):

    @staticmethod
    def forward(ctx, x, inds, passthrough=False):
        _dev(x, inds)
        x = _f32c(x)
        ctx.rev = reverse_for(inds) if is_deterministic() else None
        inds, i64 = _idx(inds)
        Nq, H = inds.shape
        out = torch.empty((Nq, x.shape[1]), device=x.device, dtype=torch.float32)
        arg = torch.empty((Nq, x.shape[1]), device=x.device, dtype=torch.int32)
        check(lib().mvk_max_pool_fwd(_p(x), x.shape[0], x.shape[1], _p(inds), i64, Nq, H, _p(out), _p(arg), _stream()))
        ctx.save_for_backward(inds, arg)
        ctx.ns, ctx.c = x.shape[0], x.shape[1]
        ctx.set_materialize_grads(False)
        return out, (x.view_as(x) if passthrough else None)

    @staticmethod
    def backward(ctx, g, g_alias=None):
        inds, arg = ctx.saved_tensors
        if g is None:
            return g_alias, None, None
        g = _f32c(g)
        if is_deterministic():
            rev = ctx.rev
            if rev is not None and rev.shape[0] >= ctx.ns:
                base = g_alias if (g_alias is not None and g_alias.shape == (ctx.ns, ctx.c)) else None
                dx = torch.empty((ctx.ns, ctx.c), device=g.device, dtype=torch.float32)
                check(lib().mvk_max_pool_bwd_gather(_p(g), _p(arg), _p(inds), int(inds.dtype == torch.int64), inds.shape[1],
                                                    inds.shape[0], _p(rev), rev.shape[1], ctx.ns, ctx.c,
                                                    _p(_f32c(base)) if base is not None else None, _p(dx), _stream()))
                if g_alias is not None and base is None:
                    dx = dx + g_alias
                return dx, None, None
            _no_reverse_list("a max_pool matrix")
        if (g_alias is not None and g_alias.dtype == torch.float32 and g_alias.is_contiguous()
                and g_alias.shape == (ctx.ns, ctx.c) and _accumulate_in_place_ok(g_alias)):
            dx = g_alias
        else:
            dx = _zeros((ctx.ns, ctx.c), g.device)
        check(lib().mvk_max_pool_bwd(_p(g), _p(arg), _p(inds), int(inds.dtype == torch.int64), inds.shape[0],
                                     inds.shape[1], ctx.ns, g.shape[1], _p(dx), _stream()))
        if g_alias is not None and dx is not g_alias:
            dx = dx + g_alias
        return dx, None, None


class _GatherRowsFn(torch.autograd.Function):
    @staticmethod
    def forward(ctx, x, inds2d):
        _dev(x, inds2d)
        x = _f32c(x)
        ctx.rev = reverse_for(inds2d, first_column=True) if is_deterministic() else None
        inds2d, i64 = _idx(inds2d)
        Nq = inds2d.shape[0]
        stride = inds2d.shape[1] if inds2d.dim() == 2 else 1
        out = torch.empty((Nq, x.shape[1]), device=x.device, dtype=torch.float32)
        check(lib().mvk_gather_rows_fwd(_p(x), x.shape[0], x.shape[1], _p(inds2d), i64, Nq, stride, _p(out), _stream()))
        ctx.save_for_backward(inds2d)
        ctx.ns, ctx.stride = x.shape[0], stride
        return out

    @staticmethod
    def backward(ctx, g):
        (inds2d,) = ctx.saved_tensors
        if not (g.dtype == torch.float32 and g.dim() == 2 and g.stride(1) == 1 and g.stride(0) >= g.shape[1]):
            g = _f32c(g)
        if is_deterministic():
            rev = ctx.rev
            if rev is not None and rev.shape[0] >= ctx.ns:
                return gather_sum_rows(g, rev[:ctx.ns]), None
            _no_reverse_list("a closest_pool / upsampling matrix")
        dx = _zeros((ctx.ns, g.shape[1]), g.device)
        check(lib().mvk_gather_rows_bwd_ld(_p(g), g.stride(0), _p(inds2d), int(inds2d.dtype == torch.int64),
                                           inds2d.shape[0], ctx.stride, ctx.ns, g.shape[1], _p(dx), _stream()))
        return dx, None


class _UpsampleCatFn(torch.autograd.Function):

    @staticmethod
    def forward(ctx, x, inds2d, skip):
        _dev(x, inds2d, skip)
        x, skip = _f32c(x), _f32c(skip)
        ctx.rev = reverse_for(inds2d, first_column=True) if is_deterministic() else None
        inds2d, i64 = _idx(inds2d)
        Nq = inds2d.shape[0]
        if skip.shape[0] != Nq:
            raise RuntimeError("upsample_cat: the skip features and the upsampling indices differ in length")
        stride = inds2d.shape[1] if inds2d.dim() == 2 else 1
        C1, C2 = x.shape[1], skip.shape[1]
        out = torch.empty((Nq, C1 + C2), device=x.device, dtype=torch.float32)
        check(lib().mvk_gather_rows_cat_fwd(_p(x), x.shape[0], C1, _p(inds2d), i64, Nq, stride, _p(skip), C2, _p(out),
                                            _stream()))
        ctx.save_for_backward(inds2d)
        ctx.ns, ctx.stride, ctx.c1 = x.shape[0], stride, C1
        return out

    @staticmethod
    def backward(ctx, g):
        (inds2d,) = ctx.saved_tensors
        g = _f32c(g)
        c2 = g.shape[1] - ctx.c1
        if is_deterministic():
            rev = ctx.rev
            if rev is not None and rev.shape[0] >= ctx.ns:
                dx = gather_sum_rows(g[:, :ctx.c1], rev[:ctx.ns]) if ctx.needs_input_grad[0] else None
                return dx, None, (g[:, ctx.c1:].contiguous() if ctx.needs_input_grad[2] else None)
            _no_reverse_list("a closest_pool / upsampling matrix")
        dx = _zeros((ctx.ns, ctx.c1), g.device) if ctx.needs_input_grad[0] else None
        d_skip = torch.empty((g.shape[0], c2), device=g.device, dtype=torch.float32) if ctx.needs_input_grad[2] else None
        check(lib().mvk_gather_rows_cat_bwd(_p(g), _p(inds2d), int(inds2d.dtype == torch.int64), inds2d.shape[0],
                                            ctx.stride, ctx.ns, ctx.c1, c2, _p(dx), _p(d_skip), _stream()))
        return dx, None, d_skip


class _UpsampleCatLinearFn(torch.autograd.Function):

    @staticmethod
    def forward(ctx, x, inds2d, skip, W, stats_n_valid, finish=None):
        _dev(x, inds2d, skip, W)
        x, skip = _f32c(x), _f32c(skip)
        ctx.rev = reverse_for(inds2d, first_column=True) if is_deterministic() else None
        inds2d, i64 = _idx(inds2d)
        Nq = inds2d.shape[0]
        if skip.shape[0] != Nq:
            raise RuntimeError("upsample_cat_linear: the skip features and the upsampling indices differ in length")
        stride = inds2d.shape[1] if inds2d.dim() == 2 else 1
        C1, C2 = x.shape[1], skip.shape[1]
        cat = torch.empty((Nq, C1 + C2), device=x.device, dtype=torch.float32)
        check(lib().mvk_gather_rows_cat_fwd(_p(x), x.shape[0], C1, _p(inds2d), i64, Nq, stride, _p(skip), C2, _p(cat),
                                            _stream()))
        ctx.set_materialize_grads(False)
        ctx.save_for_backward(cat, W, inds2d)
        ctx.dims = (x.shape[0], C1, C2, stride, i64)
        y, st = _product(cat, W, transB=True, stats_n_valid=stats_n_valid, finish=finish)
        if st is not None:
            ctx.mark_non_differentiable(st.partials)
        return y, st

    @staticmethod
    def backward(ctx, g, g_st=None):
        cat, W, inds2d = ctx.saved_tensors
        ns, C1, C2, stride, i64 = ctx.dims
        g = _f32c(g)
        M, N, Kd = cat.shape[0], C1 + C2, W.shape[0]
        split_arena_prepare(g.device)
        if is_deterministic() and M > 0:
            rev = ctx.rev
            if rev is not None and rev.shape[0] >= ns:
                dx = gemm_ldb(gather_sum_rows(g, rev[:ns]), W, 0, C1, N) if ctx.needs_input_grad[0] else None
                d_skip = gemm_ldb(g, W, C1, C2, N) if ctx.needs_input_grad[2] else None
                dW = _dw_gemm(g, cat, target=W) if ctx.needs_input_grad[3] else None
                return dx, None, d_skip, dW, None, None
            _no_reverse_list("a closest_pool / upsampling matrix")
        dx = _zeros((ns, C1), g.device)
        split = gemm_plan(M, N, Kd, None, False)[0] if M > 0 else 1
        d_skip = _split_out((M, C2), g.device, split)
        if M > 0:
            check(lib().mvk_gemm_f32_scatter_cat(_p(g), _p(W), M, N, Kd, _p(inds2d), i64, stride, ns, C1, _p(dx),
                                                 _p(d_skip), _stream()))
        dW = _dw_gemm(g, cat, target=W) if ctx.needs_input_grad[3] else None
        return (dx if ctx.needs_input_grad[0] else None), None, (d_skip if ctx.needs_input_grad[2] else None), dW, None, None


def upsample_cat_linear(x, inds, skip, W, stats_n_valid=None, bn=None):
    y, st = _UpsampleCatLinearFn.apply(x, inds, skip, W, stats_n_valid,
                                       bn if stats_n_valid is not None and _finishable(bn) else None)
    if st is not None:
        y._mvk_bn_stats = st
    return y


def upsample_cat(x, inds, skip):
    return _UpsampleCatFn.apply(x, inds, skip)


def max_pool(x, inds, passthrough=False):
    out, alias = _MaxPoolFn.apply(x, inds, passthrough)
    return (out, alias) if passthrough else out


def closest_pool(x, inds):
    return _GatherRowsFn.apply(x, inds)



import numpy as _np

_WS = {}


def _workspace(tag, nbytes, device):
    key = (tag, device.index)
    buf = _WS.get(key)
    if buf is None or buf.numel() < nbytes:
        buf = torch.empty(int(nbytes * 1.25) + 1024, dtype=torch.uint8, device=device)
        _WS[key] = buf
    return buf


def _lens_host(lens):
    if isinstance(lens, torch.Tensor):
        lens = lens.detach().cpu().numpy()
    return _np.ascontiguousarray(lens, dtype=_np.int32)


def grid_subsample_batch(points, lens, features=None, labels=None, dl=0.1, max_p=0, rotations=None):
    _dev(points, features, labels)
    points = _f32c(points)
    lens_h = _lens_host(lens)
    N, B = points.shape[0], int(lens_h.shape[0])
    fdim = ldim = 0
    if features is not None:
        features = _f32c(features)
        fdim = features.shape[1]
    if labels is not None:
        labels = labels.to(torch.int32).contiguous()
        if labels.dim() == 1:
            labels = labels.unsqueeze(1)
        ldim = labels.shape[1]
    ws = _workspace("sub", lib().mvk_grid_subsample_workspace(N, B, fdim, ldim), points.device)
    out_pts = torch.empty((max(N, 1), 3), device=points.device, dtype=torch.float32)
    out_f = torch.empty((max(N, 1), fdim), device=points.device, dtype=torch.float32) if fdim else None
    out_l = torch.empty((max(N, 1), ldim), device=points.device, dtype=torch.int32) if ldim else None
    out_lens = torch.empty((B,), device=points.device, dtype=torch.int32)
    out_lens_h = _np.empty((B,), _np.int32)
    tail = (_p(features), fdim, _p(labels), ldim, float(dl), int(max_p), _p(out_pts), _p(out_f), _p(out_l),
            _p(out_lens), out_lens_h.ctypes.data_as(C.c_void_p), _p(ws), ws.numel(), _stream())
    if rotations is None:
        check(lib().mvk_grid_subsample_batch(_p(points), N, lens_h.ctypes.data_as(C.c_void_p), B, *tail))
    else:
        rot = _np.ascontiguousarray(rotations, dtype=_np.float32)
        if rot.shape != (B, 3, 3):
            raise RuntimeError("grid_subsample_batch: rotations must be [B,3,3]")
        check(lib().mvk_grid_subsample_batch_oriented(_p(points), N, lens_h.ctypes.data_as(C.c_void_p), B,
                                                      rot.ctypes.data_as(C.c_void_p), *tail))
    M = int(out_lens_h.sum())
    res = [out_pts[:M], out_lens_h]
    if fdim:
        res.append(out_f[:M])
    if ldim:
        res.append(out_l[:M])
    return tuple(res)


_NB_GRID = {}


def radius_neighbors_batch(queries, supports, q_lens, s_lens, radius, limit=None, status=None, reuse_grid=False):
    _dev(queries, supports)
    q, s = _f32c(queries), _f32c(supports)
    ql, sl = _lens_host(q_lens), _lens_host(s_lens)
    if ql.shape[0] != sl.shape[0]:
        raise RuntimeError("Wrong number of batch elements: different for queries and supports ")
    Nq, Ns, B = q.shape[0], s.shape[0], int(ql.shape[0])
    ws = _workspace("nb", lib().mvk_radius_neighbors_workspace(Nq, Ns, B), q.device)
    args = (_p(q), Nq, _p(s), Ns, ql.ctypes.data_as(C.c_void_p), sl.ctypes.data_as(C.c_void_p), B, float(radius))
    if status is not None:
        if limit is None:
            raise RuntimeError("radius_neighbors_batch: the enqueue-only mode needs a column limit")
        _dev(status)
        width = int(limit)
        out = torch.empty((Nq, width), device=q.device, dtype=torch.int32)
        reuse = bool(reuse_grid) and _NB_GRID.get(q.device.index) == ws.data_ptr()
        if width > 0 and Nq > 0:
            check(lib().mvk_radius_neighbors_enqueue(*args, _p(out), width, _p(status), int(reuse), _p(ws),
                                                     ws.numel(), _stream()))
            _NB_GRID[q.device.index] = ws.data_ptr()
        return out
    _NB_GRID.pop(q.device.index, None)
    if limit is None:
        w = C.c_int(0)
        check(lib().mvk_radius_neighbors_batch(*args, None, 0, C.byref(w), _p(ws), ws.numel(), _stream()))
        width = int(w.value)
    else:
        width = int(limit)
    out = torch.empty((Nq, width), device=q.device, dtype=torch.int32)
    if width > 0 and Nq > 0:
        w = C.c_int(0)
        check(lib().mvk_radius_neighbors_batch(*args, _p(out), width, C.byref(w), _p(ws), ws.numel(), _stream()))
        if int(w.value) < width:
            out = out[:, :int(w.value)].contiguous()
    return out


def grid_subsample_dev(points, lens_dev, dl, out_points, out_lens_dev, status, rotations_dev=None,
                       total_out=None, pad_value=1e6):
    _dev(points, lens_dev, out_points, out_lens_dev, status, rotations_dev, total_out)
    points = _f32c(points)
    cap_in, B = points.shape[0], int(lens_dev.shape[0])
    if not out_points.is_contiguous() or out_points.dtype != torch.float32:
        raise RuntimeError("grid_subsample_dev: out_points must be a contiguous float32 [cap,3] tensor")
    ws = _workspace("sub", lib().mvk_grid_subsample_workspace(cap_in, B, 0, 0), points.device)
    check(lib().mvk_grid_subsample_batch_dev(_p(points), cap_in, _p(lens_dev), B, _p(rotations_dev), float(dl),
                                             _p(out_points), out_points.shape[0], float(pad_value),
                                             _p(out_lens_dev), _p(total_out), _p(status), _p(ws), ws.numel(), _stream()))


def radius_neighbors_dev(queries, supports, q_lens_dev, s_lens_dev, radius, out, shadow, status, reuse_grid=False,
                         rev=None, rev_counts=None, rev_status=None):
    _dev(queries, supports, q_lens_dev, s_lens_dev, out, status, rev, rev_counts, rev_status)
    q, s = _f32c(queries), _f32c(supports)
    if out.dtype != torch.int32 or not out.is_contiguous() or out.shape[0] != q.shape[0]:
        raise RuntimeError("radius_neighbors_dev: out must be a contiguous int32 [Nq_cap, width] tensor")
    B = int(q_lens_dev.shape[0])
    ws = _workspace("nb", lib().mvk_radius_neighbors_workspace(q.shape[0], s.shape[0], B), q.device)
    if rev is not None:
        if (rev.dtype != torch.int32 or not rev.is_contiguous() or rev.dim() != 2 or rev.shape[0] < s.shape[0]
                or rev_counts is None or rev_counts.dtype != torch.int32 or rev_counts.numel() < s.shape[0] or rev_status is None):
            raise RuntimeError("radius_neighbors_dev: rev must be a contiguous int32 [>= Ns_cap, Hr] matrix with int32 "
                               "counters [>= Ns_cap] and a status word")
        check(lib().mvk_radius_neighbors_dev_rev(_p(q), q.shape[0], _p(s), s.shape[0], _p(q_lens_dev), _p(s_lens_dev), B,
                                                 float(radius), _p(out), out.shape[1], int(shadow), _p(status),
                                                 int(bool(reuse_grid)), _p(ws), ws.numel(), _p(rev), rev.shape[1],
                                                 _p(rev_counts), _p(rev_status), _stream()))
    else:
        check(lib().mvk_radius_neighbors_dev(_p(q), q.shape[0], _p(s), s.shape[0], _p(q_lens_dev), _p(s_lens_dev), B,
                                             float(radius), _p(out), out.shape[1], int(shadow), _p(status),
                                             int(bool(reuse_grid)), _p(ws), ws.numel(), _stream()))
    _NB_GRID.pop(q.device.index, None)


REG_MANY = CONSTANTS["MVK_REG_MANY"]
REV_MANY = CONSTANTS["MVK_REV_MANY"]


def reverse_finish_many(lists, status=None):
    from ._lib import RevList
    for i0 in range(0, len(lists), REV_MANY):
        chunk = lists[i0:i0 + REV_MANY]
        arr = (RevList * len(chunk))()
        for k, (rev, counts, rows, shadow) in enumerate(chunk):
            _dev(rev, counts, status)
            arr[k] = RevList(_p(rev), _p(counts), _p(status), int(rows), int(rev.shape[1]), int(shadow))
        check(lib().mvk_reverse_finish_many(arr, len(chunk), _stream()))


def neighbors_cell_order(Nq, Ns, B, out=None, s_lens_dev=None, device=None):
    dev = out.device if out is not None else (s_lens_dev.device if s_lens_dev is not None else device)
    if out is None:
        out = torch.empty((Ns,), device=dev, dtype=torch.int32)
    _dev(out, s_lens_dev)
    if out.dtype != torch.int32 or not out.is_contiguous() or out.dim() != 1 or out.shape[0] < Ns:
        raise RuntimeError("neighbors_cell_order: out must be a contiguous int32 vector of at least Ns entries")
    ws = _workspace("nb", lib().mvk_radius_neighbors_workspace(Nq, Ns, B), dev)
    check(lib().mvk_neighbors_cell_order(Ns, B, _p(s_lens_dev), _p(out), out.shape[0], _p(ws), ws.numel(), _stream()))
    return out


_REV_COUNTS = {}
_REV_COUNTS_RETIRED = []
REVERSE_DX = os.environ.get("MVK_REVERSE_DX", "1") == "1"


def _rev_counts(n, device):
    key = device.index
    buf = _REV_COUNTS.get(key)
    if buf is None or buf.numel() < n:
        if torch.cuda.is_current_stream_capturing():
            raise RuntimeError("ops.reverse_neighbors: the counter buffer of this device does not exist yet (or is too "
                               "small) and cannot be created inside a graph capture; build one batch eagerly first")
        if buf is not None:
            _REV_COUNTS_RETIRED.append(buf)
        buf = torch.zeros(max(int(n), 1 << 16), dtype=torch.int32, device=device)
        torch.cuda.current_stream(device).synchronize()
        _REV_COUNTS[key] = buf
    return buf


REV_MAX_WIDTH = CONSTANTS["MVK_REV_MAX_WIDTH"]


def reverse_width_cap(sort=None):
    return REV_MAX_WIDTH


def reverse_neighbors(idx, Ns, width=None, out=None, status=None, shadow=None, sort=None, first_column=False):
    _dev(idx, out, status)
    idx, i64 = _idx(idx)
    Nq, H = idx.shape[0], idx.shape[1] if idx.dim() == 2 else 0
    stride = H
    if first_column:
        H = min(H, 1)
    Ns = int(Ns)
    shadow = Nq if shadow is None else int(shadow)
    dev = idx.device
    counts = _rev_counts(Ns, dev)
    do_sort = int(is_deterministic() if sort is None else bool(sort))

    def run(dst, w, st):
        check(lib().mvk_reverse_neighbors(_p(idx), i64, Nq, H, max(stride, H), Ns, _p(dst), int(w), shadow, do_sort,
                                          _p(counts), _p(st), _stream()))

    if out is not None:
        if out.dtype != torch.int32 or not out.is_contiguous() or out.dim() != 2 or out.shape[0] < Ns:
            raise RuntimeError("reverse_neighbors: out must be a contiguous int32 [>= Ns, width] matrix")
        run(out, out.shape[1], status)
        return out
    if width is not None:
        rev = torch.empty((Ns, max(int(width), 1)), device=dev, dtype=torch.int32)
        run(rev, rev.shape[1], status)
        return rev
    st = torch.zeros(2, dtype=torch.int32, device=dev)
    cap = reverse_width_cap(do_sort)
    w = max(8, min(cap, 2 * H + 8))
    rev = torch.empty((Ns, w), device=dev, dtype=torch.int32)
    run(rev, w, st)
    longest, ovf = (int(v) for v in st.cpu())
    if ovf:
        if longest > cap:
            raise RuntimeError("reverse_neighbors: a support has %d reverse neighbours (> %d)" % (longest, cap))
        rev = torch.empty((Ns, longest), device=dev, dtype=torch.int32)
        run(rev, longest, None)
        return rev
    return rev[:, :max(longest, 1)].contiguous()


_REVERSES = collections.OrderedDict()
_REVERSES_KEPT = 256


def _rev_key(inds, first):
    return (inds.device.index, inds.data_ptr(), tuple(inds.shape), inds.dtype, bool(first))


def remember_reverse(inds, rev, first_column=False):
    key = _rev_key(inds, first_column)
    if len(_REVERSES) >= 16:
        for k in [k for k, e in _REVERSES.items() if e[0]() is None]:
            del _REVERSES[k]
    _REVERSES[key] = (weakref.ref(inds), rev)
    _REVERSES.move_to_end(key)
    while len(_REVERSES) > _REVERSES_KEPT:
        _REVERSES.popitem(last=False)


def reverse_for(inds, first_column=False):
    if not (torch.is_tensor(inds) and inds.is_cuda):
        return None
    e = _REVERSES.get(_rev_key(inds, first_column))
    return e[1] if (e is not None and e[0]() is inds) else None


_DET_WARNED = set()


def _no_reverse_list(what):
    if what not in _DET_WARNED:
        _DET_WARNED.add(what)
        import warnings
        warnings.warn("deterministic mode: no reverse list for %s; its backward uses float atomics (not bit-reproducible)" % what)


def gather_sum_rows(g, rev, base=None):
    _dev(g, rev, base)
    if not (g.dtype == torch.float32 and g.dim() == 2 and g.stride(1) == 1 and g.stride(0) >= g.shape[1]):
        g = _f32c(g)
    Ns, Hr = rev.shape
    out = torch.empty((Ns, g.shape[1]), device=g.device, dtype=torch.float32)
    if base is not None:
        base = _f32c(base)
    check(lib().mvk_gather_sum_rows(_p(g), g.stride(0), g.shape[0], _p(rev), Hr, Ns, g.shape[1], _p(base), _p(out), _stream()))
    return out

# ... 1652 lines not shown
```

Before: 5.541 million points/s.

## Fuse decoder upsample gather and concat into row-indexed GEMM loads

```diff
diff --git a/enhancing-3d-point-cloud-segmentation-using-multi-modal-fusion-with-2d-images_amd/_lib.py b/enhancing-3d-point-cloud-segmentation-using-multi-modal-fusion-with-2d-images_amd/_lib.py
--- a/enhancing-3d-point-cloud-segmentation-using-multi-modal-fusion-with-2d-images_amd/_lib.py
+++ b/enhancing-3d-point-cloud-segmentation-using-multi-modal-fusion-with-2d-images_amd/_lib.py
@@ -8,6 +8,7 @@
 SCENE_HEADER_PATH = os.path.join(_HERE, "..", "include", "mvkpconv_scene.h")
 TRAIN_HEADER_PATH = os.path.join(_HERE, "..", "include", "mvkpconv_train.h")
 SPHERE_HEADER_PATH = os.path.join(_HERE, "..", "include", "mvkpconv_sphere.h")
+DECODER_HEADER_PATH = os.path.join(_HERE, "..", "include", "mvkpconv_decoder.h")
 
 CTYPES = {"int": C.c_int, "int32_t": C.c_int32, "int64_t": C.c_int64, "float": C.c_float, "double": C.c_double,
           "const char*": C.c_char_p}
@@ -139,6 +140,12 @@
         or SPHERE_CONSTANTS.keys() & (CONSTANTS.keys() | SCENE_CONSTANTS.keys() | TRAIN_CONSTANTS.keys())):
     raise ValueError("mvkpconv_sphere.h: it may declare neither a struct nor a name of the other three headers")
 _SPHERE_PROTOTYPES = _bind(SPHERE_FUNCTIONS, {})[1]
+
+DECODER_FUNCTIONS, _decoder_structs, DECODER_CONSTANTS = parse_header(_read_header(DECODER_HEADER_PATH, "mvkpconv_decoder.h"))
+if (_decoder_structs or DECODER_CONSTANTS
+        or DECODER_FUNCTIONS.keys() & (FUNCTIONS.keys() | SCENE_FUNCTIONS.keys() | TRAIN_FUNCTIONS.keys() | SPHERE_FUNCTIONS.keys())):
+    raise ValueError("mvkpconv_decoder.h: it may declare neither a struct, a constant nor a name of the other four headers")
+_DECODER_PROTOTYPES = _bind(DECODER_FUNCTIONS, {})[1]
 BnFwdProblem, BnBwdProblem = _CLASSES["mvk_bn_fwd_problem"], _CLASSES["mvk_bn_bwd_problem"]
 BnFinish, ATransform = _CLASSES["mvk_bn_finish"], _CLASSES["mvk_a_transform"]
 RevList, RegLayer = _CLASSES["mvk_rev_list"], _CLASSES["mvk_reg_layer"]
@@ -174,7 +181,7 @@
                 "no CPU fallback for the MV-KPConv hot path." % LIB_PATH)
         l = C.CDLL(LIB_PATH)
         for name, (res, args) in list(_PROTOTYPES.items()) + list(_SCENE_PROTOTYPES.items()) + list(_TRAIN_PROTOTYPES.items()) \
-                + list(_SPHERE_PROTOTYPES.items()):
+                + list(_SPHERE_PROTOTYPES.items()) + list(_DECODER_PROTOTYPES.items()):
             fn = getattr(l, name)
             fn.restype = res
             fn.argtypes = args
diff --git a/enhancing-3d-point-cloud-segmentation-using-multi-modal-fusion-with-2d-images_amd/build.py b/enhancing-3d-point-cloud-segmentation-using-multi-modal-fusion-with-2d-images_amd/build.py
--- a/enhancing-3d-point-cloud-segmentation-using-multi-modal-fusion-with-2d-images_amd/build.py
+++ b/enhancing-3d-point-cloud-segmentation-using-multi-modal-fusion-with-2d-images_amd/build.py
@@ -54,7 +54,7 @@
               os.path.join(CSRC, "pn2_rows.h"), os.path.join(CSRC, "unproject.h"), os.path.join(CSRC, "select_frames.h"),
               os.path.join(CSRC, "knn_core.h"), os.path.join(HERE, "..", "include", "mvkpconv_sphere.h"),
               os.path.join(HERE, "..", "include", "mvkpconv.h"), os.path.join(HERE, "..", "include", "mvkpconv_scene.h"),
-              os.path.join(HERE, "..", "include", "mvkpconv_train.h"),
+              os.path.join(HERE, "..", "include", "mvkpconv_train.h"), os.path.join(HERE, "..", "include", "mvkpconv_decoder.h"),
               os.path.join(HERE, "..", "include", "mvk_prime_list.h"), os.path.abspath(__file__)]
     objs, jobs = [], []
     for src, extra in SOURCES:
diff --git a/enhancing-3d-point-cloud-segmentation-using-multi-modal-fusion-with-2d-images_amd/csrc/gemm.hip b/enhancing-3d-point-cloud-segmentation-using-multi-modal-fusion-with-2d-images_amd/csrc/gemm.hip
--- a/enhancing-3d-point-cloud-segmentation-using-multi-modal-fusion-with-2d-images_amd/csrc/gemm.hip
+++ b/enhancing-3d-point-cloud-segmentation-using-multi-modal-fusion-with-2d-images_amd/csrc/gemm.hip
@@ -2,6 +2,7 @@
 
 #include <mutex>
 #include <type_traits>
+#include <vector>
 
 #include "common.h"
 
@@ -141,6 +142,115 @@
       load(src, ld, i0, imax, k0, kmax, vec, tid);
     else
       load_fast<VEC>(src, ld, i0, imax, k0, tid);
+  }
+
+  template <int VEC>
+  __device__ __forceinline__ void fetch_rows(const float* __restrict__ src, int64_t ld, const int* row, int64_t k0,
+                                             int64_t kmax, int vec, int tid) {
+    static_assert(CONTIG_K && NF4 % 256 == 0, "row-indexed A: k-contiguous tiles of whole float4 rounds");
+#pragma unroll
+    for (int u = 0; u < NV; ++u) {
+      const int kq = ((tid + 256 * u) & 7) * 4;
+      const int64_t gk = k0 + kq;
+      if (VEC == 0) {
+        float t[4] = {0.f, 0.f, 0.f, 0.f};
+        if (row[u] >= 0) {
+          const float* p = src + (int64_t)row[u] * ld + gk;
+          if (vec == 4 && gk + 3 < kmax) {
+            const float4 q = *reinterpret_cast<const float4*>(p);
+            t[0] = q.x; t[1] = q.y; t[2] = q.z; t[3] = q.w;
+          } else if (vec == 2 && gk + 3 < kmax) {
+            const float2 q0 = *reinterpret_cast<const float2*>(p), q1 = *reinterpret_cast<const float2*>(p + 2);
+            t[0] = q0.x; t[1] = q0.y; t[2] = q1.x; t[3] = q1.y;
+          } else {
+#pragma unroll
+            for (int e = 0; e < 4; ++e)
+              if (gk + e < kmax) t[e] = p[e];
+          }
+        }
+        v[u] = make_float4(t[0], t[1], t[2], t[3]);
+      } else {
+        const float* p = src + (int64_t)(row[u] < 0 ? 0 : row[u]) * ld + gk;
+        if (VEC == 4) {
+          const f32x4 q = *reinterpret_cast<const f32x4*>(p);
+          v[u] = make_float4(q[0], q[1], q[2], q[3]);
+        } else {
+          const float2 q0 = *reinterpret_cast<const float2*>(p), q1 = *reinterpret_cast<const float2*>(p + 2);
+          v[u] = make_float4(q0.x, q0.y, q1.x, q1.y);
+        }
+      }
+    }
+  }
+
+  __device__ __forceinline__ void prime_krows(const void* idx, int idx64, int64_t stride, int64_t ns, int* row, int64_t k0,
+                                              int64_t kcount, int tid) {
+#pragma unroll
+    for (int u = 0; u < NV; ++u) {
+      int f = tid + 256 * u;
+      if (NF4 % 256 != 0) f = f < NF4 ? f : NF4 - 1;
+      int64_t gk = k0 + f / IPT;
+      gk = gk < kcount ? gk : kcount - 1;
+      row[u] = 0;
+      row[NV + u] = idx64 ? load_idx<true>(idx, gk * stride, ns) : load_idx<false>(idx, gk * stride, ns);
+    }
+  }
+
+  template <int VEC>
+  __device__ __forceinline__ void fetch_krows(const float* __restrict__ src, int64_t ld, const void* idx, int idx64,
+                                              int64_t stride, int64_t ns, int* row, int64_t i0, int64_t imax, int64_t k0,
+                                              int64_t kmax, int64_t kcount, int vec, int tid) {
+    static_assert(!CONTIG_K, "k-indexed B: row-contiguous tiles");
+#pragma unroll
+    for (int u = 0; u < NV; ++u) {
+      int f = tid + 256 * u;
+      const bool mine = NF4 % 256 == 0 || f < NF4;
+      if (!mine) f = NF4 - 1;
+      const int k = f / IPT, iq = (f % IPT) * 4;
+      const int64_t gk = k0 + k;
+      int64_t gi = i0 + iq;
+      int64_t r = gk;
+      row[u] = 0;
+      if (VEC == 0) {
+        float t[4] = {0.f, 0.f, 0.f, 0.f};
+        if (mine && gk < kmax) {
+          if (idx) r = idx64 ? load_idx<true>(idx, gk * stride, ns) : load_idx<false>(idx, gk * stride, ns);
+          if (r >= 0) {
+            const float* p = src + r * ld + gi;
+            if (vec == 4 && gi + 3 < imax) {
+              const float4 q = *reinterpret_cast<const float4*>(p);
+              t[0] = q.x; t[1] = q.y; t[2] = q.z; t[3] = q.w;
+            } else if (vec == 2 && gi + 3 < imax) {
+              const float2 q0 = *reinterpret_cast<const float2*>(p), q1 = *reinterpret_cast<const float2*>(p + 2);
+              t[0] = q0.x; t[1] = q0.y; t[2] = q1.x; t[3] = q1.y;
+            } else {
+#pragma unroll
+              for (int e = 0; e < 4; ++e)
+                if (gi + e < imax) t[e] = p[e];
+            }
+          }
+        }
+        v[u] = make_float4(t[0], t[1], t[2], t[3]);
+      } else {
+        static_assert(VEC == 0 || VEC == 4, "row-contiguous tiles load whole float4");
+        if (idx) {
+          const int j = row[NV + u];
+          row[u] = j;
+          r = j < 0 ? 0 : j;
+          int64_t gn = gk + 2 * BK;
+          gn = gn < kcount ? gn : kcount - 1;
+          row[NV + u] = idx64 ? load_idx<true>(idx, gn * stride, ns) : load_idx<false>(idx, gn * stride, ns);
+        }
+        gi = gi + 3 < imax ? gi : imax - 4;
+        const f32x4 q = *reinterpret_cast<const f32x4*>(src + r * ld + gi);
+        v[u] = make_float4(q[0], q[1], q[2], q[3]);
+      }
+    }
+  }
+
+  __device__ __forceinline__ void zero_rows(const int* row) {
+#pragma unroll
+    for (int u = 0; u < NV; ++u)
+      if (row[u] < 0) v[u] = make_float4(0.f, 0.f, 0.f, 0.f);
   }
 
   __device__ __forceinline__ void store(float* __restrict__ T, int tid) const {
@@ -215,13 +325,17 @@
   float ax_slope;
   const int32_t* ax_nvalid;
   float* ax_out;
+  const void* ri_idx;
+  int ri_idx64;
+  int64_t ri_stride, ri_ns, ldc;
 };
 
 constexpr int XF_KMAX = 512;
 
-template <bool TA, bool TB, int PM, int QN, int WM, int WN, bool DUAL = false, bool XF = false>
+template <bool TA, bool TB, int PM, int QN, int WM, int WN, bool DUAL = false, bool XF = false, int RI = 0>
 __device__ __forceinline__ void gemm_body(const GemmArgs& a, const int bx, const int by, const int bz) {
   static_assert(WM * WN == 4, "four waves per workgroup");
+  static_assert(RI == 0 || (RI == 1 && !TA && DUAL && !XF) || (RI == 2 && TA && !TB && !DUAL && !XF), "row-indexed forms");
   constexpr int TM = 16 * PM * WM, TN = 16 * QN * WN;
   typedef Tile<!TA, TM> TileA;
   typedef Tile<TB, TN> TileB;
@@ -232,7 +346,8 @@
   const int tid = threadIdx.x, lane = tid & 63, wave = tid >> 6;
   const int wm = wave / WN, wn = wave % WN;
   const int64_t m0 = (int64_t)by * TM, n0 = (int64_t)bx * TN;
-  const int64_t ktot = DUAL ? a.Kd + a.Kd2 : a.Kd;
+  const int64_t kseam = RI == 1 ? (a.Kd + BK - 1) / BK * BK : a.Kd;
+  const int64_t ktot = DUAL ? kseam + a.Kd2 : a.Kd;
   const int64_t kbeg_all = (int64_t)bz * a.k_per_split;
   const int64_t kend_all = kbeg_all + a.k_per_split < ktot ? kbeg_all + a.k_per_split : ktot;
 
@@ -257,6 +372,16 @@
 
   TileA la0, la1;
   TileB lb0, lb1;
+  int arow[RI == 1 ? TileA::NV : 1], br0[RI == 2 ? 2 * TileB::NV : 1], br1[RI == 2 ? 2 * TileB::NV : 1];
+  if constexpr (RI == 1) {
+#pragma unroll
+    for (int u = 0; u < TileA::NV; ++u) {
+      const int64_t gi = m0 + ((tid + 256 * u) >> 3);
+      arow[u] = -1;
+      if (gi < a.M)
+        arow[u] = a.ri_idx64 ? load_idx<true>(a.ri_idx, gi * a.ri_stride, a.ri_ns) : load_idx<false>(a.ri_idx, gi * a.ri_stride, a.ri_ns);
+    }
+  }
   const int ra = wm * 16 * PM, rb = wn * 16 * QN;
   auto compute = [&](const float* __restrict__ Ta, const float* __restrict__ Tb) {
 #pragma unroll
@@ -279,49 +404,73 @@
   float* const A1 = As + TileA::FLOATS;
   float* const B0 = Bs;
   float* const B1 = Bs + TileB::FLOATS;
-  auto run_range = [&](const float* __restrict__ pA, const int64_t lda, const int vecA, const float* __restrict__ pB,
-                       const int64_t ldb, const int vecB, int64_t kbeg, const int64_t kend) {
+  auto run_range = [&](auto ri, const float* __restrict__ pA, const int64_t lda, const int vecA,
+                       const float* __restrict__ pB, const int64_t ldb, const int vecB, int64_t kbeg, const int64_t kend) {
+  constexpr int R = decltype(ri)::value;
   auto Bat = [&](const int64_t k) -> const float* {
     return (TB && !DUAL && a.seg_shift >= 0) ? pB + (k >> a.seg_shift) * a.seg_extra : pB;
   };
+  auto getA = [&](auto va, TileA& la, const int64_t kt, const int64_t klim) {
+    constexpr int VA = decltype(va)::value;
+    if constexpr (R == 1) la.template fetch_rows<VA>(pA, lda, arow, kt, klim, vecA, tid);
+    else la.template fetch<VA>(pA, lda, m0, a.M, kt, klim, vecA, tid);
+  };
+  auto getB = [&](auto vb, TileB& lb, int* brow, const int64_t kt, const int64_t klim) {
+    constexpr int VB = decltype(vb)::value;
+    if constexpr (R == 2)
+      lb.template fetch_krows<VB>(pB, ldb, a.ri_idx, a.ri_idx64, a.ri_stride, a.ri_ns, brow, n0, a.N, kt, klim, a.Kd, vecB, tid);
+    else lb.template fetch<VB>(Bat(kt), ldb, n0, a.N, kt, klim, vecB, tid);
+  };
   auto putA = [&](TileA& la, float* __restrict__ T, const int64_t kt) {
     if constexpr (XF) la.transform(xs, kt, kbeg_all, m0, a.M, a.Kd, x_nvalid, a.ax_slope, x_out, lda, tid);
+    if constexpr (R == 1) la.zero_rows(arow);
     la.store(T, tid);
+  };
+  auto putB = [&](TileB& lb, const int* brow, float* __restrict__ T) {
+    if constexpr (R == 2) lb.zero_rows(brow);
+    lb.store(T, tid);
   };
   auto pipeline = [&](auto va, auto vb, const int64_t klim) {
     constexpr int VA = decltype(va)::value, VB = decltype(vb)::value;
     if (kbeg >= klim) return;
-    la0.template fetch<VA>(pA, lda, m0, a.M, kbeg, klim, vecA, tid);
-    lb0.template fetch<VB>(Bat(kbeg), ldb, n0, a.N, kbeg, klim, vecB, tid);
+    if constexpr (R == 2 && VB != 0) {
+      if (a.ri_idx) {
+        lb0.prime_krows(a.ri_idx, a.ri_idx64, a.ri_stride, a.ri_ns, br0, kbeg, a.Kd, tid);
+        lb1.prime_krows(a.ri_idx, a.ri_idx64, a.ri_stride, a.ri_ns, br1, kbeg + BK, a.Kd, tid);
+      }
+    }
+    getA(va, la0, kbeg, klim);
+    getB(vb, lb0, br0, kbeg, klim);
     if (kbeg + BK < klim) {
-      la1.template fetch<VA>(pA, lda, m0, a.M, kbeg + BK, klim, vecA, tid);
-      lb1.template fetch<VB>(Bat(kbeg + BK), ldb, n0, a.N, kbeg + BK, klim, vecB, tid);
+      getA(va, la1, kbeg + BK, klim);
+      getB(vb, lb1, br1, kbeg + BK, klim);
     }
     putA(la0, A0, kbeg);
-    lb0.store(B0, tid);
+    putB(lb0, br0, B0);
     __syncthreads();
     for (int64_t k0 = kbeg; k0 < klim; k0 += 2 * BK) {
       if (k0 + 2 * BK < klim) {
-        la0.template fetch<VA>(pA, lda, m0, a.M, k0 + 2 * BK, klim, vecA, tid);
-        lb0.template fetch<VB>(Bat(k0 + 2 * BK), ldb, n0, a.N, k0 + 2 * BK, klim, vecB, tid);
+        getA(va, la0, k0 + 2 * BK, klim);
+        getB(vb, lb0, br0, k0 + 2 * BK, klim);
       }
       compute(A0, B0);
       if (k0 + BK >= klim) break;
       putA(la1, A1, k0 + BK);
-      lb1.store(B1, tid);
+      putB(lb1, br1, B1);
       __syncthreads();
       if (k0 + 3 * BK < klim) {
-        la1.template fetch<VA>(pA, lda, m0, a.M, k0 + 3 * BK, klim, vecA, tid);
-        lb1.template fetch<VB>(Bat(k0 + 3 * BK), ldb, n0, a.N, k0 + 3 * BK, klim, vecB, tid);
+        getA(va, la1, k0 + 3 * BK, klim);
+        getB(vb, lb1, br1, k0 + 3 * BK, klim);
       }
       compute(A1, B1);
       if (k0 + 2 * BK >= klim) break;
       putA(la0, A0, k0 + 2 * BK);
-      lb0.store(B0, tid);
+      putB(lb0, br0, B0);
       __syncthreads();
     }
   };
-  const bool fastA = TileA::fast_ok(a.M, vecA), fastB = TileB::fast_ok(a.N, vecB);
+  const bool fastA = R == 1 ? (vecA >= 2 && a.ri_ns >= 1) : TileA::fast_ok(a.M, vecA);
+  const bool fastB = TileB::fast_ok(a.N, vecB) && (R != 2 || a.ri_idx == nullptr || a.ri_ns >= 1);
   const int64_t kfull = kbeg + (kend - kbeg) / BK * BK;
   typedef std::integral_constant<int, 4> I4;
   typedef std::integral_constant<int, 2> I2;
@@ -336,21 +485,23 @@
   }
   if (kfull < kend && kbeg < kend) {
     __syncthreads();
-    la0.load(pA, lda, m0, a.M, kfull, kend, vecA, tid);
-    lb0.load(Bat(kfull), ldb, n0, a.N, kfull, kend, vecB, tid);
+    getA(I0(), la0, kfull, kend);
+    getB(I0(), lb0, br0, kfull, kend);
     putA(la0, A0, kfull);
-    lb0.store(B0, tid);
+    putB(lb0, br0, B0);
     __syncthreads();
     compute(A0, B0);
   }
   };
+  typedef std::integral_constant<int, RI> RIc;
+  typedef std::integral_constant<int, 0> RI0;
   if (!DUAL) {
-    run_range(a.A, a.lda, a.vecA, a.B, a.ldb, a.vecB, kbeg_all, kend_all);
+    run_range(RIc(), a.A, a.lda, a.vecA, a.B, a.ldb, a.vecB, kbeg_all, kend_all);
   } else {
-    if (kbeg_all < a.Kd) run_range(a.A, a.lda, a.vecA, a.B, a.ldb, a.vecB, kbeg_all, kend_all < a.Kd ? kend_all : a.Kd);
-    if (kend_all > a.Kd) {
+    if (kbeg_all < a.Kd) run_range(RIc(), a.A, a.lda, a.vecA, a.B, a.ldb, a.vecB, kbeg_all, kend_all < a.Kd ? kend_all : a.Kd);
+    if (kend_all > kseam) {
       if (kbeg_all < a.Kd) __syncthreads();
-      run_range(a.A2, a.lda2, a.vecA2, a.B2, a.ldb2, a.vecB2, kbeg_all > a.Kd ? kbeg_all - a.Kd : 0, kend_all - a.Kd);
+      run_range(RI0(), a.A2, a.lda2, a.vecA2, a.B2, a.ldb2, a.vecB2, kbeg_all > kseam ? kbeg_all - kseam : 0, kend_all - kseam);
     }
   }
 
@@ -426,7 +577,7 @@
               }
               continue;
             }
-            float* c = a.C + row * a.N + col;
+            float* c = a.C + row * (RI == 2 ? a.ldc : a.N) + col;
             if (a.atomic_out)
               atomicAdd(c, acc[p][q][r]);
             else if (a.accumulate)
@@ -621,14 +772,27 @@
   gemm_body<TA, TB, PM, QN, WM, WN, true>(a, blockIdx.x, blockIdx.y, blockIdx.z);
 }
 
+template <int PM, int QN, int WM, int WN>
+__global__ __launch_bounds__(256) __attribute__((amdgpu_waves_per_eu(4))) void gemm_f32_mfma_rows_dual(const GemmArgs a) {
+  gemm_body<false, true, PM, QN, WM, WN, true, false, 1>(a, blockIdx.x, blockIdx.y, blockIdx.z);
+}
+__global__ __launch_bounds__(256) void gemm_f32_mfma_rows_dual_tall(const GemmArgs a) {
+  gemm_body<false, true, 4, 1, 1, 4, true, false, 1>(a, blockIdx.x, blockIdx.y, blockIdx.z);
+}
+
+template <int PM, int QN, int WM, int WN>
+__global__ __launch_bounds__(256) void gemm_f32_mfma_krows(const GemmArgs a) {
+  gemm_body<true, false, PM, QN, WM, WN, false, false, 2>(a, blockIdx.x, blockIdx.y, blockIdx.z);
+}
+
 struct GroupEntry {
   GemmArgs args;
   int gx, gy, gz;
   int wg_begin;
 };
 
-template <bool TA, bool TB, int PM, int QN, int WM, int WN>
-__global__ __launch_bounds__(256) void gemm_f32_mfma_grouped(const GroupEntry* __restrict__ tab, int n_prob) {
+template <bool TA, bool TB, int PM, int QN, int WM, int WN, int RI>
+__device__ __forceinline__ void grouped_body(const GroupEntry* __restrict__ tab, int n_prob) {
   const int b = blockIdx.x;
   int lo = 0, hi = n_prob - 1;
   while (lo < hi) {
@@ -649,7 +813,18 @@
   a.n_valid = load_global_ptr(&e.args.n_valid);
   a.det_ws = load_global_ptr(&e.args.det_ws);
   a.det_cnt = load_global_ptr(&e.args.det_cnt);
-  gemm_body<TA, TB, PM, QN, WM, WN>(a, bx, by, bz);
+  if constexpr (RI != 0) a.ri_idx = load_global_ptr(&e.args.ri_idx);
+  gemm_body<TA, TB, PM, QN, WM, WN, false, false, RI>(a, bx, by, bz);
+}
+
+template <bool TA, bool TB, int PM, int QN, int WM, int WN>
+__global__ __launch_bounds__(256) void gemm_f32_mfma_grouped(const GroupEntry* __restrict__ tab, int n_prob) {
+  grouped_body<TA, TB, PM, QN, WM, WN, 0>(tab, n_prob);
+}
+
+template <int PM, int QN, int WM, int WN>
+__global__ __launch_bounds__(256) __attribute__((amdgpu_waves_per_eu(4))) void gemm_f32_mfma_grouped_krows(const GroupEntry* __restrict__ tab, int n_prob) {
+  grouped_body<true, false, PM, QN, WM, WN, 2>(tab, n_prob);
 }
 
 
@@ -823,7 +998,7 @@
   a.A = A; a.B = B; a.C = C; a.M = M; a.N = N; a.Kd = Kd;
   a.lda = lda; a.ldb = ldb; a.vecA = vec_width(A, lda); a.vecB = vec_width(B, ldb);
   a.k_per_split = ks.k_per_split; a.atomic_out = ks.n > 1; a.det_nsplit = ks.n;
-  a.act_slope = 1.f; a.ax_slope = 1.f; a.vecA2 = 1; a.vecB2 = 1; a.seg_shift = -1;
+  a.act_slope = 1.f; a.ax_slope = 1.f; a.vecA2 = 1; a.vecB2 = 1; a.seg_shift = -1; a.ldc = N;
   return a;
 }
 
@@ -838,6 +1013,12 @@
   a.fin_nbt = (long long*)fin->num_batches_tracked;
   return 0;
 }
+
+struct RowIndex {
+  const void* idx;
+  int idx64;
+  int64_t stride, ns;
+};
 
 struct ScatterOut {
   const void* idx;
@@ -858,7 +1039,12 @@
   int64_t seg_extra = 0, ldb = 0, lda = 0;
   const mvk_bn_finish* fin = nullptr;
   const mvk_a_transform* ax = nullptr;
+  const RowIndex* krows = nullptr;
+  int64_t ldc = 0;
 };
+
+bool rows_dual_has(const Plan& p) { return p.narrow ? (p.pm == 1 && (p.qn == 1 || p.qn == 2)) : (p.qn == 1 && (p.pm == 2 || p.pm == 4)); }
+bool krows_has(const Plan& p) { return p.narrow ? (p.pm == 1 && (p.qn == 1 || p.qn == 2)) : (p.qn == 1 && p.pm == 2); }
 
 int gemm_run(const float* A, const float* B, float* C, int64_t M, int64_t N, int64_t Kd, int transA, int transB,
              const GemmOpts& o, void* stream) {
@@ -875,7 +1061,7 @@
   const KSplit ks = clamp_split(Kd, p.split);
   const int64_t lda = o.lda > 0 ? o.lda : (transA ? M : Kd);
   if (cdiv64(M, p.tm()) >= 65536) {
-    MVK_REQUIRE(!o.bn_part && !o.fin && !o.ax && !o.scatter && o.seg_shift < 0 && ks.n < 65536, "gemm: grid too large");
+    MVK_REQUIRE(!o.bn_part && !o.fin && !o.ax && !o.scatter && o.seg_shift < 0 && o.ldc == 0 && ks.n < 65536, "gemm: grid too large");
     constexpr int64_t CHUNK = 15 * 65536;
     GemmOpts oc = o;
     oc.split_k = ks.n;
@@ -910,6 +1096,17 @@
     a.ax_nvalid = ax->n_valid; a.ax_out = ax->out;
     if (p.pm == 2) hipLaunchKernelGGL((gemm_f32_mfma_xf<true, 2>), grid, dim3(256), 0, st, a);
     else hipLaunchKernelGGL((gemm_f32_mfma_xf<true, 4>), grid, dim3(256), 0, st, a);
+    MVK_CHECK_HIP(hipGetLastError());
+    return 0;
+  }
+  if (o.ldc > 0) {
+    MVK_REQUIRE(transA && !transB && o.ldc >= N && !o.accumulate && !o.bn_part && !o.bias && !o.scatter && o.seg_shift < 0 && krows_has(p),
+                "gemm: the row-indexed TN product has no kernel for this call (plan pm=%d qn=%d narrow=%d)", p.pm, p.qn, p.narrow);
+    a.ldc = o.ldc;
+    if (o.krows) { a.ri_idx = o.krows->idx; a.ri_idx64 = o.krows->idx64; a.ri_stride = o.krows->stride; a.ri_ns = o.krows->ns; }
+    if (!p.narrow) hipLaunchKernelGGL((gemm_f32_mfma_krows<2, 1, 1, 4>), grid, dim3(256), 0, st, a);
+    else if (p.qn == 1) hipLaunchKernelGGL((gemm_f32_mfma_krows<1, 1, 4, 1>), grid, dim3(256), 0, st, a);
+    else hipLaunchKernelGGL((gemm_f32_mfma_krows<1, 2, 4, 1>), grid, dim3(256), 0, st, a);
     MVK_CHECK_HIP(hipGetLastError());
     return 0;
   }
@@ -1128,78 +1325,196 @@
   return grouped_split_at(M, N, Kd, e >= 0 ? e : GROUP_KTILES_MIN);
 }
 
+struct MvkGemmProblemRows {
+  MvkGemmProblem p;
+  int64_t ldc;
+  const void* idx;
+  int64_t idx_stride, ns, idx64;
+};
+
+static int grouped_plan(const MvkGemmProblemRows* pr, int n, void* table_host, int* counts , int64_t* wgs_out ,
+                        int32_t* splits, bool rows_ok, void* stream) {
+  GroupEntry* tab = (GroupEntry*)table_host;
+  static const bool merge = !getenv("MVK_DW_ROWS_MERGE") || atoi(getenv("MVK_DW_ROWS_MERGE")) != 0;
+  auto needs = [](const MvkGemmProblemRows& r) { return r.idx != nullptr || r.ldc != r.p.N; };
+  bool any[2] = {false, false};
+  for (int i = 0; i < n; ++i)
+    if (needs(pr[i])) any[pr[i].p.N <= 32 ? 0 : 1] = true;
+  auto cls = [&](const MvkGemmProblemRows& r) {
+    const int w = r.p.N <= 32 ? 0 : 1;
+    return 2 * w + ((needs(r) || (merge && rows_ok && any[w] && (w == 0 || group_wide_pm() == 4))) ? 1 : 0);
+  };
+  int pos[4] = {0, 0, 0, 0};
+  int64_t wg[4] = {0, 0, 0, 0};
+  for (int c = 0; c < 4; ++c) counts[c] = 0;
+  for (int i = 0; i < n; ++i) counts[cls(pr[i])] += 1;
+  for (int c = 1; c < 4; ++c) pos[c] = pos[c - 1] + counts[c - 1];
+  int ktiles = group_ktiles_env();
+  if (ktiles < 0) {
+    double units = 0.0;
+    for (int i = 0; i < n; ++i) {
+      const MvkGemmProblem& q = pr[i].p;
+      units += (double)cdiv64(q.M, q.N <= 32 ? 64 : 16 * group_wide_pm()) * cdiv64(q.N, q.N <= 32 ? 32 : 64) * cdiv64(q.Kd, BK);
+    }
+    const double t = units / 8000.0;
+    ktiles = t < GROUP_KTILES_MIN ? GROUP_KTILES_MIN : (t > GROUP_KTILES_MAX ? GROUP_KTILES_MAX : (int)t);
+  }
+  for (int i = 0; i < n; ++i) {
+    const MvkGemmProblem& q = pr[i].p;
+    MVK_REQUIRE(q.M > 0 && q.N > 0 && q.Kd > 0 && q.A && q.B && q.C, "grouped gemm: empty problem %d", i);
+    const bool narrow = q.N <= 32;
+    const int c = cls(pr[i]);
+    MVK_REQUIRE(!narrow || q.N > 16, "grouped gemm: outputs of <= 16 columns are not grouped");
+    const KSplit ks = clamp_split(q.Kd, grouped_split_at(q.M, q.N, q.Kd, ktiles));
+    const int split = ks.n;
+    GroupEntry e{};
+    e.args = make_args(q.A, q.B, q.C, q.M, q.N, q.Kd, q.M, q.N, ks);
+    if (c & 1) {
+      MVK_REQUIRE(rows_ok && pr[i].ldc >= q.N && (!pr[i].idx || (pr[i].idx_stride >= 1 && pr[i].ns >= 0)) &&
+                      (narrow || group_wide_pm() == 4),
+                  "grouped gemm: problem %d asks for a row index or a column block this launch cannot give it", i);
+      e.args.ldc = pr[i].ldc;
+      e.args.ri_idx = pr[i].idx; e.args.ri_idx64 = pr[i].idx64 != 0; e.args.ri_stride = pr[i].idx_stride; e.args.ri_ns = pr[i].ns;
+    }
+    const int64_t tm = narrow ? 64 : 16 * group_wide_pm(), tn = narrow ? 32 : 64;
+    e.gx = (int)cdiv64(q.N, tn);
+    e.gy = (int)cdiv64(q.M, tm);
+    e.gz = split;
+    MVK_ORDERED(make_ordered((hipStream_t)stream, e.args, split, e.gx, e.gy, tm, tn));
+    e.wg_begin = (int)wg[c];
+    wg[c] += (int64_t)e.gx * e.gy * e.gz;
+    tab[pos[c]++] = e;
+    splits[i] = split;
+  }
+  for (int c = 0; c < 4; ++c) {
+    MVK_REQUIRE(wg[c] < (1ll << 31), "grouped gemm: grid too large");
+    wgs_out[c] = wg[c];
+  }
+  return 0;
+}
+
 extern "C" int mvk_gemm_f32_tn_grouped_plan(const void* problems, int n, void* table_host, int* n_narrow,
                                             int64_t* wgs_narrow, int64_t* wgs_wide, int32_t* splits ,
                                             void* stream ) {
   MVK_REQUIRE(n >= 0 && problems && table_host && n_narrow && wgs_narrow && wgs_wide && splits, "grouped gemm: bad arguments");
   const MvkGemmProblem* pr = (const MvkGemmProblem*)problems;
-  GroupEntry* tab = (GroupEntry*)table_host;
-  int nn = 0;
-  for (int i = 0; i < n; ++i) nn += pr[i].N <= 32 ? 1 : 0;
-  int64_t wn = 0, ww = 0;
-  int in = 0, iw = nn;
-  int ktiles = group_ktiles_env();
-  if (ktiles < 0) {
-    double units = 0.0;
-    for (int i = 0; i < n; ++i)
-      units += (double)cdiv64(pr[i].M, pr[i].N <= 32 ? 64 : 16 * group_wide_pm()) * cdiv64(pr[i].N, pr[i].N <= 32 ? 32 : 64) * cdiv64(pr[i].Kd, BK);
-    const double t = units / 8000.0;
-    ktiles = t < GROUP_KTILES_MIN ? GROUP_KTILES_MIN : (t > GROUP_KTILES_MAX ? GROUP_KTILES_MAX : (int)t);
-  }
-  for (int i = 0; i < n; ++i) {
-    const MvkGemmProblem& q = pr[i];
-    MVK_REQUIRE(q.M > 0 && q.N > 0 && q.Kd > 0 && q.A && q.B && q.C, "grouped gemm: empty problem %d", i);
-    const bool narrow = q.N <= 32;
-    MVK_REQUIRE(!narrow || q.N > 16, "grouped gemm: outputs of <= 16 columns are not grouped");
-    const KSplit ks = clamp_split(q.Kd, grouped_split_at(q.M, q.N, q.Kd, ktiles));
-    const int split = ks.n;
-    GroupEntry e{};
-    e.args = make_args(q.A, q.B, q.C, q.M, q.N, q.Kd, q.M, q.N, ks);
-    const int64_t tm = narrow ? 64 : 16 * group_wide_pm(), tn = narrow ? 32 : 64;
-    e.gx = (int)cdiv64(q.N, tn);
-    e.gy = (int)cdiv64(q.M, tm);
-    e.gz = split;
-    MVK_ORDERED(make_ordered((hipStream_t)stream, e.args, split, e.gx, e.gy, tm, tn));
-    const int64_t wgs = (int64_t)e.gx * e.gy * e.gz;
-    if (narrow) {
-      e.wg_begin = (int)wn;
-      wn += wgs;
-      tab[in++] = e;
-    } else {
-      e.wg_begin = (int)ww;
-      ww += wgs;
-      tab[iw++] = e;
-    }
-    splits[i] = split;
-  }
-  MVK_REQUIRE(wn < (1ll << 31) && ww < (1ll << 31), "grouped gemm: grid too large");
-  *n_narrow = nn;
-  *wgs_narrow = wn;
-  *wgs_wide = ww;
+  std::vector<MvkGemmProblemRows> rows((size_t)n);
+  for (int i = 0; i < n; ++i) rows[i] = MvkGemmProblemRows{pr[i], pr[i].N, nullptr, 1, 0, 0};
+  int counts[4];
+  int64_t wgs[4];
+  if (int e = grouped_plan(rows.data(), n, table_host, counts, wgs, splits, false, stream)) return e;
+  *n_narrow = counts[0];
+  *wgs_narrow = wgs[0];
+  *wgs_wide = wgs[2];
+  return 0;
+}
+
+extern "C" int mvk_gemm_f32_tn_grouped_plan_rows(const void* problems, int n, void* table_host, int* counts, int64_t* wgs,
+                                                 int32_t* splits, void* stream) {
+  MVK_REQUIRE(n >= 0 && problems && table_host && counts && wgs && splits, "grouped gemm: bad arguments");
+  return grouped_plan((const MvkGemmProblemRows*)problems, n, table_host, counts, wgs, splits, true, stream);
+}
+
+extern "C" int mvk_gemm_f32_tn_grouped_rows_ok(int64_t N) { return N > 16 && (N <= 32 || group_wide_pm() == 4) ? 1 : 0; }
+
+static int grouped_launch(const void* table_dev, const int* counts, const int64_t* wgs, void* stream) {
+  hipStream_t st = (hipStream_t)stream;
+  const GroupEntry* tab = (const GroupEntry*)table_dev;
+  for (int c = 0; c < 4; ++c) {
+    MVK_REQUIRE(counts[c] >= 0 && wgs[c] >= 0 && wgs[c] < (1ll << 31), "grouped gemm: bad counts");
+    const dim3 grid((unsigned)wgs[c]);
+    if (counts[c] > 0 && wgs[c] > 0) {
+      if (c == 0)
+        hipLaunchKernelGGL((gemm_f32_mfma_grouped<true, false, 1, 2, 4, 1>), grid, dim3(256), 0, st, tab, counts[c]);
+      else if (c == 1)
+        hipLaunchKernelGGL((gemm_f32_mfma_grouped_krows<1, 2, 4, 1>), grid, dim3(256), 0, st, tab, counts[c]);
+      else if (c == 3) {
+        MVK_REQUIRE(group_wide_pm() == 4, "grouped gemm: the row-indexed wide kernel has 64-row tiles only");
+        hipLaunchKernelGGL((gemm_f32_mfma_grouped_krows<4, 1, 1, 4>), grid, dim3(256), 0, st, tab, counts[c]);
+      } else if (group_wide_pm() == 4)
+        hipLaunchKernelGGL((gemm_f32_mfma_grouped<true, false, 4, 1, 1, 4>), grid, dim3(256), 0, st, tab, counts[c]);
+      else if (group_wide_pm() == 8)
+        hipLaunchKernelGGL((gemm_f32_mfma_grouped<true, false, 8, 1, 1, 4>), grid, dim3(256), 0, st, tab, counts[c]);
+      else
+        hipLaunchKernelGGL((gemm_f32_mfma_grouped<true, false, 2, 1, 1, 4>), grid, dim3(256), 0, st, tab, counts[c]);
+    }
+    tab += counts[c];
+  }
+  MVK_CHECK_HIP(hipGetLastError());
   return 0;
 }
 
 extern "C" int mvk_gemm_f32_tn_grouped(const void* table_dev, int n, int n_narrow, int64_t wgs_narrow, int64_t wgs_wide,
                                        void* stream) {
   MVK_REQUIRE(n >= 0 && n_narrow >= 0 && n_narrow <= n, "grouped gemm: bad counts");
+  const int counts[4] = {n_narrow, 0, n - n_narrow, 0};
+  const int64_t wgs[4] = {wgs_narrow, 0, wgs_wide, 0};
+  return grouped_launch(table_dev, counts, wgs, stream);
+}
+
+extern "C" int mvk_gemm_f32_tn_grouped_rows(const void* table_dev, const int* counts, const int64_t* wgs, void* stream) {
+  MVK_REQUIRE(table_dev && counts && wgs, "grouped gemm: bad arguments");
+  return grouped_launch(table_dev, counts, wgs, stream);
+}
+
+
+extern "C" int mvk_gemm_f32_rows_dual_plan(int64_t M, int64_t N, int64_t C1, int64_t C2, int want_stats, int* out_split,
+                                           int* out_stat_rows) {
+  MVK_REQUIRE(M >= 0 && N >= 0 && C1 >= 0 && C2 >= 0 && out_split && out_stat_rows, "gemm rows_dual plan: bad arguments");
+  *out_split = 0;
+  *out_stat_rows = 0;
+  if (M == 0 || N == 0 || C1 == 0 || C2 == 0) return 0;
+  const Plan p = plan_gemm(M, N, C1 + C2, 0, want_stats != 0);
+  if (!rows_dual_has(p) || cdiv64(M, p.tm()) >= 65536) return 0;
+  *out_split = clamp_split(cdiv64(C1, BK) * BK + C2, p.split).n;
+  *out_stat_rows = (want_stats && (*out_split == 1 || ordered_splits())) ? (int)p.tm() : 0;
+  return 0;
+}
+
+extern "C" int mvk_gemm_f32_rows_dual(const float* x, const void* idx, int idx64, int64_t idx_stride, int64_t Ns,
+                                      const float* skip, const float* W, float* C, int64_t M, int64_t N, int64_t C1,
+                                      int64_t C2, int split_k, float* bn_part, const int32_t* n_valid, void* stream) {
+  MVK_REQUIRE(x && idx && skip && W && C && M > 0 && N > 0 && C1 > 0 && C2 > 0 && Ns >= 0 && idx_stride >= 1 && split_k >= 1,
+              "gemm rows_dual: bad arguments");
   hipStream_t st = (hipStream_t)stream;
-  const GroupEntry* tab = (const GroupEntry*)table_dev;
-  if (n_narrow > 0 && wgs_narrow > 0)
-    hipLaunchKernelGGL((gemm_f32_mfma_grouped<true, false, 1, 2, 4, 1>), dim3((unsigned)wgs_narrow), dim3(256), 0, st, tab,
-                       n_narrow);
-  if (n - n_narrow > 0 && wgs_wide > 0) {
-    if (group_wide_pm() == 4)
-      hipLaunchKernelGGL((gemm_f32_mfma_grouped<true, false, 4, 1, 1, 4>), dim3((unsigned)wgs_wide), dim3(256), 0, st,
-                         tab + n_narrow, n - n_narrow);
-    else if (group_wide_pm() == 8)
-      hipLaunchKernelGGL((gemm_f32_mfma_grouped<true, false, 8, 1, 1, 4>), dim3((unsigned)wgs_wide), dim3(256), 0, st,
-                         tab + n_narrow, n - n_narrow);
-    else
-      hipLaunchKernelGGL((gemm_f32_mfma_grouped<true, false, 2, 1, 1, 4>), dim3((unsigned)wgs_wide), dim3(256), 0, st,
-                         tab + n_narrow, n - n_narrow);
-  }
+  Plan p = plan_gemm(M, N, C1 + C2, 0, bn_part != nullptr);
+  p.split = split_k;
+  MVK_REQUIRE(rows_dual_has(p) && cdiv64(M, p.tm()) < 65536, "gemm rows_dual: no kernel for this shape (ask mvk_gemm_f32_rows_dual_plan)");
+  const int64_t ld = C1 + C2;
+  const KSplit ks = clamp_split(cdiv64(C1, BK) * BK + C2, p.split);
+  GemmArgs a = make_args(x, W, C, M, N, C1, C1, ld, ks);
+  a.A2 = skip; a.B2 = W + C1; a.Kd2 = C2; a.lda2 = C2; a.ldb2 = ld;
+  a.vecA2 = vec_width(a.A2, a.lda2);
+  a.vecB2 = vec_width(a.B2, a.ldb2);
+  a.ri_idx = idx; a.ri_idx64 = idx64 != 0; a.ri_stride = idx_stride; a.ri_ns = Ns;
+  a.bn_part = bn_part; a.n_valid = n_valid;
+  dim3 grid((unsigned)cdiv64(N, p.tn()), (unsigned)cdiv64(M, p.tm()), (unsigned)ks.n);
+  MVK_ORDERED(make_ordered(st, a, ks.n, (int)grid.x, grid.y, p.tm(), p.tn()));
+  MVK_REQUIRE(!(bn_part && ks.n > 1 && !a.det_ws), "gemm rows_dual: BatchNorm statistics need an unsplit (or ordered) reduction");
+  if (p.narrow && p.qn == 1) hipLaunchKernelGGL((gemm_f32_mfma_rows_dual<1, 1, 4, 1>), grid, dim3(256), 0, st, a);
+  else if (p.narrow) hipLaunchKernelGGL((gemm_f32_mfma_rows_dual<1, 2, 4, 1>), grid, dim3(256), 0, st, a);
+  else if (p.pm == 2) hipLaunchKernelGGL((gemm_f32_mfma_rows_dual<2, 1, 1, 4>), grid, dim3(256), 0, st, a);
+  else hipLaunchKernelGGL(gemm_f32_mfma_rows_dual_tall, grid, dim3(256), 0, st, a);
   MVK_CHECK_HIP(hipGetLastError());
   return 0;
+}
+
+extern "C" int mvk_gemm_f32_tn_rows_plan(int64_t M, int64_t N, int64_t Kd, int* out_split) {
+  MVK_REQUIRE(M >= 0 && N >= 0 && Kd >= 0 && out_split, "gemm tn_rows plan: bad arguments");
+  *out_split = 0;
+  if (M == 0 || N == 0 || Kd == 0) return 0;
+  const Plan p = plan_gemm(M, N, Kd, 0, false);
+  if (!krows_has(p) || cdiv64(M, p.tm()) >= 65536) return 0;
+  *out_split = p.split;
+  return 0;
+}
+
+extern "C" int mvk_gemm_f32_tn_rows(const float* A, const float* B, float* C, int64_t M, int64_t N, int64_t Kd, int64_t ldc,
+                                    const void* idx, int idx64, int64_t idx_stride, int64_t Ns, void* stream) {
+  MVK_REQUIRE(A && B && C && M > 0 && N > 0 && Kd > 0 && ldc >= N && (!idx || (idx_stride >= 1 && Ns >= 0)), "gemm tn_rows: bad arguments");
+  const RowIndex ri{idx, idx64 != 0, idx_stride, Ns};
+  GemmOpts o; o.ldc = ldc; o.krows = idx ? &ri : nullptr;
+  return gemm_run(A, B, C, M, N, Kd, 1, 0, o, stream);
 }
 
 extern "C" int mvk_gemm_f32(const float* A, const float* B, float* C, int64_t M, int64_t N, int64_t Kd, int transA,
diff --git a/enhancing-3d-point-cloud-segmentation-using-multi-modal-fusion-with-2d-images_amd/ops.py b/enhancing-3d-point-cloud-segmentation-using-multi-modal-fusion-with-2d-images_amd/ops.py
--- a/enhancing-3d-point-cloud-segmentation-using-multi-modal-fusion-with-2d-images_amd/ops.py
+++ b/enhancing-3d-point-cloud-segmentation-using-multi-modal-fusion-with-2d-images_amd/ops.py
@@ -464,9 +464,12 @@
         return
     if stream is None or stream == torch.cuda.current_stream():
         return _flush_deferred(items)
-    for (A, B, _, _, _) in items:
-        A.record_stream(stream)
-        B.record_stream(stream)
+    for it in items:
+        it[0].record_stream(stream)
+        it[1].record_stream(stream)
+        rows = getattr(it, "rows", None)
+        if rows is not None and rows[1] is not None:
+            rows[1].record_stream(stream)
     with torch.cuda.stream(stream):
         _flush_deferred(items)
 
@@ -486,14 +489,22 @@
     import numpy as np
     dev = items[0][0].device
     n = len(items)
-    prob = np.zeros(n, dtype=np.dtype([("A", "<u8"), ("B", "<u8"), ("C", "<u8"), ("M", "<i8"), ("N", "<i8"), ("Kd", "<i8")]))
+    fields = [("A", "<u8"), ("B", "<u8"), ("C", "<u8"), ("M", "<i8"), ("N", "<i8"), ("Kd", "<i8")]
+    with_rows = any(getattr(it, "rows", None) is not None for it in items)
+    if with_rows:
+        fields += [("ldc", "<i8"), ("idx", "<u8"), ("stride", "<i8"), ("ns", "<i8"), ("idx64", "<i8")]
+    prob = np.zeros(n, dtype=np.dtype(fields))
     for i, (A, B, out_ptr, _, storage) in enumerate(items):
-        if _storage_use_count(storage) < 2:
+        if storage is not None and _storage_use_count(storage) < 2:
             raise RuntimeError("defer_weight_grads: a deferred weight-gradient result (%d x %d) was consumed before the "
                                "grouped launch computed it; was the backward run on parameters that already hold a "
                                ".grad, or with hooks that copy gradients? Run it without the scope (MVK_DEFER_DW=0)"
                                % (A.shape[1], B.shape[1]))
-        prob[i] = (A.data_ptr(), B.data_ptr(), out_ptr, A.shape[1], B.shape[1], A.shape[0])
+        rec = (A.data_ptr(), B.data_ptr(), out_ptr, A.shape[1], B.shape[1], A.shape[0])
+        if with_rows:
+            ldc, inds, i64, stride, ns = getattr(items[i], "rows", None) or (B.shape[1], None, 0, 1, 0)
+            rec += (ldc, inds.data_ptr() if inds is not None else 0, stride, ns, i64)
+        prob[i] = rec
     slots = _defer_slots(dev)
     if torch.cuda.is_current_stream_capturing():
         if len(slots) <= 2:
@@ -506,16 +517,26 @@
         if slot["event"] is not None:
             slot["event"].synchronize()
     nn, wn, ww = C.c_int(0), C.c_int64(0), C.c_int64(0)
+    counts, wgs = np.zeros(4, np.int32), np.zeros(4, np.int64)
     splits = np.zeros(n, np.int32)
-    check(lib().mvk_gemm_f32_tn_grouped_plan(prob.ctypes.data_as(C.c_void_p), n, C.c_void_p(slot["host"].data_ptr()),
-                                             C.byref(nn), C.byref(wn), C.byref(ww), splits.ctypes.data_as(C.c_void_p),
-                                             _stream()))
+    if with_rows:
+        check(lib().mvk_gemm_f32_tn_grouped_plan_rows(prob.ctypes.data_as(C.c_void_p), n, C.c_void_p(slot["host"].data_ptr()),
+                                                      counts.ctypes.data_as(C.c_void_p), wgs.ctypes.data_as(C.c_void_p),
+                                                      splits.ctypes.data_as(C.c_void_p), _stream()))
+    else:
+        check(lib().mvk_gemm_f32_tn_grouped_plan(prob.ctypes.data_as(C.c_void_p), n, C.c_void_p(slot["host"].data_ptr()),
+                                                 C.byref(nn), C.byref(wn), C.byref(ww), splits.ctypes.data_as(C.c_void_p),
+                                                 _stream()))
     for i, item in enumerate(items):
         if splits[i] > 1 and not item[3] and not lib().mvk_gemm_split_ordered():
             raise RuntimeError("defer_weight_grads: the grouped plan splits a product whose output was not zero-initialised")
     nb = n * int(lib().mvk_gemm_group_entry_bytes())
     slot["dev"][:nb].copy_(slot["host"][:nb], non_blocking=True)
-    check(lib().mvk_gemm_f32_tn_grouped(C.c_void_p(slot["dev"].data_ptr()), n, nn.value, wn.value, ww.value, _stream()))
+    if with_rows:
+        check(lib().mvk_gemm_f32_tn_grouped_rows(C.c_void_p(slot["dev"].data_ptr()), counts.ctypes.data_as(C.c_void_p),
+                                                 wgs.ctypes.data_as(C.c_void_p), _stream()))
+    else:
+        check(lib().mvk_gemm_f32_tn_grouped(C.c_void_p(slot["dev"].data_ptr()), n, nn.value, wn.value, ww.value, _stream()))
     if not torch.cuda.is_current_stream_capturing():
         ev = torch.cuda.Event()
         ev.record()
@@ -552,6 +573,60 @@
             _DEFER["leaves"].add(id(leaf))
         return out
     return gemm(A, B, transA=True, transB=transB)
+
+
+class _DwItem(tuple):
+    rows = None
+
+
+def _dw_gemm_cat(g, x, inds2d, i64, stride, skip, target=None):
+    L = lib()
+    M, Cout = g.shape
+    Ns, C1 = x.shape
+    C2 = skip.shape[1]
+    halves = ((x, 0, C1, (inds2d, i64, stride, Ns)), (skip, C1, C2, (None, 0, 1, 0)))
+    leaf = target if (target is not None and target.is_leaf) else None
+    defer = _DEFER["on"] and _HAS_USE_COUNT and g.is_cuda and len(_DEFER["items"]) + 2 <= _DW_MAX
+    if _DEFER["on"] and leaf is not None:
+        if id(leaf) in _DEFER["leaves"]:
+            raise RuntimeError("defer_weight_grads: the same parameter receives two weight gradients inside one scope "
+                               "(shared weights): run this backward without the scope (MVK_DEFER_DW=0)")
+        defer = defer and leaf.grad is None
+    split_arena_prepare(g.device)
+    ordered = bool(L.mvk_gemm_split_ordered())
+    plan, ok = [], M > 0 and Ns > 0
+    for (_, _, n, _) in halves if ok else ():
+        if defer and n > 16 and L.mvk_gemm_f32_tn_grouped_rows_ok(n):
+            plan.append((True, L.mvk_gemm_f32_tn_grouped_split(Cout, n, M)))
+        else:
+            sp = C.c_int(0)
+            check(L.mvk_gemm_f32_tn_rows_plan(Cout, n, M, C.byref(sp)))
+            plan.append((False, sp.value))
+            ok = ok and sp.value > 0
+    if not ok:
+        cat = torch.empty((M, C1 + C2), device=g.device, dtype=torch.float32)
+        check(L.mvk_gather_rows_cat_fwd(_p(x), Ns, C1, _p(inds2d), i64, M, stride, _p(skip), C2, _p(cat), _stream()))
+        return _dw_gemm(g, cat, target=target)
+    deferred = any(d for d, _ in plan)
+    zeroed = any(sp > 1 for _, sp in plan) and not ordered
+    if deferred:
+        out = (_zeros((Cout, C1 + C2), g.device) if zeroed
+               else torch.empty((Cout, C1 + C2), device=g.device, dtype=torch.float32))
+    else:
+        out = _split_out((Cout, C1 + C2), g.device, 2 if zeroed else 1)
+    storage = out.untyped_storage()
+    for (B, col0, n, (inds, b64, st, ns)), (d, _) in zip(halves, plan):
+        c_ptr = out.data_ptr() + 4 * col0
+        if d:
+            item = _DwItem((g, B, c_ptr, zeroed, storage))
+            item.rows = (C1 + C2, inds, b64, st, ns)
+            _DEFER["items"].append(item)
+            storage = None
+        else:
+            check(L.mvk_gemm_f32_tn_rows(_p(g), _p(B), C.c_void_p(c_ptr), Cout, n, M, C1 + C2, _p(inds), b64, st, ns, _stream()))
+    if deferred and leaf is not None:
+        _DEFER["leaves"].add(id(leaf))
+    return out
 
 
 
@@ -1214,6 +1289,29 @@
         return dx, None, d_skip
 
 
+DECODER_INPLACE = os.environ.get("MVK_DECODER_INPLACE", "1") == "1"
+
+
+def _upsample_cat_linear_inplace(x, inds2d, i64, stride, skip, W, stats_n_valid):
+    Nq, Ns, C1, C2, N = inds2d.shape[0], x.shape[0], x.shape[1], skip.shape[1], W.shape[0]
+    if not DECODER_INPLACE or min(Nq, Ns, C1, C2, N) == 0:
+        return None
+    if W.shape[1] != C1 + C2:
+        raise RuntimeError("upsample_cat_linear: W has %d input columns, the inputs %d + %d" % (W.shape[1], C1, C2))
+    W = _f32c(W)
+    split_arena_prepare(x.device)
+    stats_ok = stats_n_valid is not None and Nq <= _STATS_EPILOGUE_ROWS and Nq > bn_single_launch_rows(N)
+    sp, rows = C.c_int(0), C.c_int(0)
+    check(lib().mvk_gemm_f32_rows_dual_plan(Nq, N, C1, C2, int(stats_ok), C.byref(sp), C.byref(rows)))
+    if sp.value == 0:
+        return None
+    y = _split_out((Nq, N), x.device, sp.value)
+    part = torch.empty(((Nq + rows.value - 1) // rows.value, 2, N), device=x.device, dtype=torch.float32) if rows.value > 0 else None
+    check(lib().mvk_gemm_f32_rows_dual(_p(x), _p(inds2d), i64, stride, Ns, _p(skip), _p(W), _p(y), Nq, N, C1, C2, sp.value,
+                                       _p(part), _p(stats_n_valid) if part is not None else None, _stream()))
+    return y, (BnStats(part, rows.value, None) if part is not None else None)
+
+
 class _UpsampleCatLinearFn(torch.autograd.Function):
 
     @staticmethod
@@ -1227,30 +1325,45 @@
             raise RuntimeError("upsample_cat_linear: the skip features and the upsampling indices differ in length")
         stride = inds2d.shape[1] if inds2d.dim() == 2 else 1
         C1, C2 = x.shape[1], skip.shape[1]
-        cat = torch.empty((Nq, C1 + C2), device=x.device, dtype=torch.float32)
-        check(lib().mvk_gather_rows_cat_fwd(_p(x), x.shape[0], C1, _p(inds2d), i64, Nq, stride, _p(skip), C2, _p(cat),
-                                            _stream()))
         ctx.set_materialize_grads(False)
-        ctx.save_for_backward(cat, W, inds2d)
         ctx.dims = (x.shape[0], C1, C2, stride, i64)
-        y, st = _product(cat, W, transB=True, stats_n_valid=stats_n_valid, finish=finish)
+        y = _upsample_cat_linear_inplace(x, inds2d, i64, stride, skip, W, stats_n_valid) if finish is None else None
+        ctx.inplace = y is not None
+        if ctx.inplace:
+            y, st = y
+            ctx.save_for_backward(x, skip, W, inds2d)
+        else:
+            cat = torch.empty((Nq, C1 + C2), device=x.device, dtype=torch.float32)
+            check(lib().mvk_gather_rows_cat_fwd(_p(x), x.shape[0], C1, _p(inds2d), i64, Nq, stride, _p(skip), C2, _p(cat),
+                                                _stream()))
+            ctx.save_for_backward(cat, W, inds2d)
+            y, st = _product(cat, W, transB=True, stats_n_valid=stats_n_valid, finish=finish)
         if st is not None:
             ctx.mark_non_differentiable(st.partials)
         return y, st
 
     @staticmethod
     def backward(ctx, g, g_st=None):
-        cat, W, inds2d = ctx.saved_tensors
         ns, C1, C2, stride, i64 = ctx.dims
         g = _f32c(g)
-        M, N, Kd = cat.shape[0], C1 + C2, W.shape[0]
+        if ctx.inplace:
+            x, skip, W, inds2d = ctx.saved_tensors
+
+            def weight_grad():
+                return _dw_gemm_cat(g, x, inds2d, i64, stride, skip, target=W)
+        else:
+            cat, W, inds2d = ctx.saved_tensors
+
+            def weight_grad():
+                return _dw_gemm(g, cat, target=W)
+        M, N, Kd = inds2d.shape[0], C1 + C2, W.shape[0]
         split_arena_prepare(g.device)
         if is_deterministic() and M > 0:
             rev = ctx.rev
             if rev is not None and rev.shape[0] >= ns:
                 dx = gemm_ldb(gather_sum_rows(g, rev[:ns]), W, 0, C1, N) if ctx.needs_input_grad[0] else None
                 d_skip = gemm_ldb(g, W, C1, C2, N) if ctx.needs_input_grad[2] else None
-                dW = _dw_gemm(g, cat, target=W) if ctx.needs_input_grad[3] else None
+                dW = weight_grad() if ctx.needs_input_grad[3] else None
                 return dx, None, d_skip, dW, None, None
             _no_reverse_list("a closest_pool / upsampling matrix")
         dx = _zeros((ns, C1), g.device)
@@ -1259,7 +1372,7 @@
         if M > 0:
             check(lib().mvk_gemm_f32_scatter_cat(_p(g), _p(W), M, N, Kd, _p(inds2d), i64, stride, ns, C1, _p(dx),
                                                  _p(d_skip), _stream()))
-        dW = _dw_gemm(g, cat, target=W) if ctx.needs_input_grad[3] else None
+        dW = weight_grad() if ctx.needs_input_grad[3] else None
         return (dx if ctx.needs_input_grad[0] else None), None, (d_skip if ctx.needs_input_grad[2] else None), dW, None, None
 
 
diff --git a/include/mvkpconv_decoder.h b/include/mvkpconv_decoder.h
--- /dev/null
+++ b/include/mvkpconv_decoder.h
@@ -0,0 +1,32 @@
+#ifndef MVKPCONV_DECODER_H
+#define MVKPCONV_DECODER_H
+
+#include <stdint.h>
+
+#ifdef __cplusplus
+extern "C" {
+#endif
+
+int mvk_gemm_f32_rows_dual_plan(int64_t M, int64_t N, int64_t C1, int64_t C2, int want_stats, int* out_split,
+                                int* out_stat_rows);
+
+int mvk_gemm_f32_rows_dual(const float* x, const void* idx, int idx64, int64_t idx_stride, int64_t Ns, const float* skip,
+                           const float* W, float* C, int64_t M, int64_t N, int64_t C1, int64_t C2, int split_k,
+                           float* bn_part, const int32_t* n_valid, void* stream);
+
+int mvk_gemm_f32_tn_rows_plan(int64_t M, int64_t N, int64_t Kd, int* out_split);
+
+int mvk_gemm_f32_tn_rows(const float* A, const float* B, float* C, int64_t M, int64_t N, int64_t Kd, int64_t ldc,
+                         const void* idx, int idx64, int64_t idx_stride, int64_t Ns, void* stream);
+
+int mvk_gemm_f32_tn_grouped_rows_ok(int64_t N);
+
+int mvk_gemm_f32_tn_grouped_plan_rows(const void* problems_host, int n, void* table_host, int* counts_host,
+                                      int64_t* wgs_host, int32_t* splits_host, void* stream);
+
+int mvk_gemm_f32_tn_grouped_rows(const void* table_dev, const int* counts_host, const int64_t* wgs_host, void* stream);
+
+#ifdef __cplusplus
+}
+#endif
+#endif
```

Result: no change. 5.502 million points/s (-0.7%).
